# Minys233/GCN-BMP

Measured on NVIDIA B200. Metric: drug pairs/sec (fwd+bwd, GGNN+co-attention), higher is better.
Workload: dtype bf16

## Files before the change

gcn-bmp_b200/csrc/coattn_tc.cu:

```cuda
#include "tc_common.cuh"

namespace bmp {
namespace ctc {
using namespace tc;

constexpr int EPW = 16, NE = 32 * EPW, NT = NE + 64;
constexpr int CLD = 68;
constexpr int PLD = 65;
constexpr int MAXHD = 15;
constexpr int STAGES = 2;

#define EPI_SYNC() asm volatile("bar.sync 1, %0;" ::"n"(NE) : "memory")
#define CTS(i) do { if (a.dbg && blockIdx.x == 0 && tid == 0 && it == 1) a.dbg[i] = clock64(); } while (0)

struct Args {
    int mb, n1, n2, O, head, act, pool;
    const float *atoms_1, *atoms_2, *b, *wa_1, *wa_2, *W_j, *b_j, *lt_2, *V2;
    const uint8_t *img1, *img2, *img1x;
    float *c1, *c2;
    const float *dc1, *dc2;
    float *R, *P1, *P2, *DL1, *DL2, *d_a1, *d_a2;
    float *d_W, *d_lt_1, *d_lt_2, *d_V1, *d_V2, *d_b, *d_wa_1, *d_wa_2;
    long long *dbg;
};

template <int H, bool BWD>
struct Cfg {
    static constexpr int KP = H / 64;
    static constexpr int W1_TILE = (H + 32) * 128;
    static constexpr int WH_TILE = H * 128;
    static constexpr int OFF_XP = 0;
    static constexpr int OFF_QP = OFF_XP + KP * PANEL_BYTES;
    static constexpr int OFF_W = OFF_QP + PANEL_BYTES;
    static constexpr int OFF_SP = OFF_W + STAGES * W1_TILE;
    static constexpr int OFF_DP = OFF_SP + (BWD ? KP * PANEL_BYTES : 0);
    static constexpr int OFF_F = OFF_DP + (BWD ? 2 * PANEL_BYTES : 0);
    static constexpr int TMEM_COLS = BWD ? 512 : 256;
    static constexpr uint32_t COL_D1 = 0, COL_D2 = 192, COL_R = 0, COL_A1 = 0, COL_S = 256, COL_A2 = 256, COL_X1 = 160, COL_X2 = 176, COL_DW = 384;
};

__host__ __device__ inline int f32_floats(int H, int hd, bool bwd) {
    hd = hd <= 8 ? 8 : 16;
    int n = AT * CLD + 2 * AT * PLD + 4;
    n += 4 * hd * AT;
    n += 4 * AT + 2 * H;
    n += 4 * AT + 16 * AT;
    if (bwd) n += 2 * H + 2 * hd * AT + 2 * 16 + 4;
    return (n + 3) & ~3;
}
template <int H, bool BWD>
__host__ __device__ inline size_t smem_bytes(int hd) {
    return (size_t)Cfg<H, BWD>::OFF_F + (size_t)f32_floats(H, hd, BWD) * 4 + 256 + 1024;
}

__device__ __forceinline__ float warp_sum(float v) {
    for (int o = 16; o; o >>= 1) v += __shfl_xor_sync(0xffffffffu, v, o);
    return v;
}
__device__ __forceinline__ float warp_max(float v) {
    for (int o = 16; o; o >>= 1) v = fmaxf(v, __shfl_xor_sync(0xffffffffu, v, o));
    return v;
}
__device__ __forceinline__ float bf16_at(const uint8_t *panels, int row, int col) {
    return __bfloat162float(*reinterpret_cast<const __nv_bfloat16 *>(panels + (col >> 6) * PANEL_BYTES + sw128(row, col & 63)));
}
__device__ __forceinline__ uint4 pack8(const float *v) {
    return make_uint4(pack_bf16(v[0], v[1]), pack_bf16(v[2], v[3]), pack_bf16(v[4], v[5]), pack_bf16(v[6], v[7]));
}

template <int H, bool BWD, int HP>
__global__ void __launch_bounds__(NT, 1) coattn_tc_kernel(const Args a) {
    using C = Cfg<H, BWD>;
    constexpr int HS = HP, HQ = HP / 4;
    constexpr int KP = C::KP;
    extern __shared__ uint8_t smem_raw[];
    uint8_t *smem = (uint8_t *)(((uintptr_t)smem_raw + 1023) & ~(uintptr_t)1023);
    const uint32_t sbase = s32(smem);
    const uint32_t s_xp = sbase + C::OFF_XP, s_qp = sbase + C::OFF_QP, s_w = sbase + C::OFF_W, s_sp = sbase + C::OFF_SP,
                   s_dp = sbase + C::OFF_DP;
    uint8_t *XP = smem + C::OFF_XP, *QP = smem + C::OFF_QP, *SP = smem + C::OFF_SP, *DP = smem + C::OFF_DP;
    const int hd = a.head, N1 = a.n1, N2 = a.n2, O = a.O;
    const bool pool = a.pool != 0;
    float *fp = reinterpret_cast<float *>(smem + C::OFF_F);
    float *Cs = fp; fp += AT * CLD;
    float *L1t = fp; fp += AT * PLD;
    float *L2p = fp; fp += AT * PLD + 4;
    float *lt1 = fp; fp += HS * AT;
    float *lt2 = fp; fp += HS * AT;
    float *H1 = fp; fp += HS * AT;
    float *H2 = fp; fp += HS * AT;
    float *attn1 = fp; fp += AT;
    float *attn2 = fp; fp += AT;
    float *v1 = fp; fp += AT;
    float *v2 = fp; fp += AT;
    float *p1 = fp; fp += H;
    float *p2 = fp; fp += H;
    float *st4 = fp; fp += 4 * AT;
    float *part = fp; fp += 16 * AT;
    float *dp1 = fp, *dp2 = fp + H, *dpre1 = fp + 2 * H, *dpre2 = dpre1 + HS * AT;
    float *gwa1 = dpre2 + HS * AT, *gwa2 = gwa1 + 16, *gb = gwa2 + 16;
    const int f32n = f32_floats(H, hd, BWD);
    const uint32_t s_bar = sbase + C::OFF_F + f32n * 4;
    auto BAR = [&](int i) { return s_bar + 8u * i; };
    constexpr int B_FULL = 0, B_EMPTY = 2, B_XRDY = 4, B_G1 = 5, B_S = 6, B_QRDY = 7, B_G2 = 8, B_DRDY = 9, B_R = 10,
                  B_A2 = 11, B_RRDY = 12, B_A1 = 13, NBAR = 14;
    uint32_t *tmem_slot = reinterpret_cast<uint32_t *>(smem + C::OFF_F + f32n * 4 + 8 * NBAR + 8);

    const int tid = threadIdx.x, warp = tid >> 5, lane = tid & 31;
    if (tid == 0) {
        for (int s = 0; s < STAGES; ++s) { mbar_init(BAR(B_FULL + s), 1); mbar_init(BAR(B_EMPTY + s), 1); }
        mbar_init(BAR(B_XRDY), EPW);
        mbar_init(BAR(B_G1), 1);
        mbar_init(BAR(B_S), 1);
        mbar_init(BAR(B_QRDY), EPW);
        mbar_init(BAR(B_G2), 1);
        mbar_init(BAR(B_DRDY), EPW);
        mbar_init(BAR(B_R), 1);
        mbar_init(BAR(B_A2), 1);
        mbar_init(BAR(B_RRDY), EPW);
        mbar_init(BAR(B_A1), 1);
        fence_mbar_init();
    }
    if (warp == EPW + 1) {
        asm volatile("tcgen05.alloc.cta_group::1.sync.aligned.shared::cta.b32 [%0], %1;" ::"r"(s32(tmem_slot)), "r"(C::TMEM_COLS));
        asm volatile("tcgen05.relinquish_alloc_permit.cta_group::1.sync.aligned;");
    }
    tc_fence_before();
    __syncthreads();
    tc_fence_after();
    const uint32_t tmem = *tmem_slot;

    if (warp == EPW) {
        if (lane == 0) {
            uint32_t stage = 0, phase = 0;
            auto put = [&](const uint8_t *src, uint32_t bytes) {
                mbar_wait(BAR(B_EMPTY + stage), phase ^ 1);
                mbar_expect_tx(BAR(B_FULL + stage), bytes);
                tma_bulk_g2s(s_w + stage * C::W1_TILE, src, bytes, BAR(B_FULL + stage));
                if (++stage == STAGES) { stage = 0; phase ^= 1; }
            };
            for (int pair = blockIdx.x; pair < a.mb; pair += gridDim.x) {
                for (int kt = 0; kt < KP; ++kt) put(a.img1 + (size_t)kt * C::W1_TILE, C::W1_TILE);
                if (BWD) {
                    for (int kt = 0; kt < KP; ++kt) put(a.img2 + (size_t)kt * C::WH_TILE, C::WH_TILE);
                    for (int kt = 0; kt < KP; ++kt) put(a.img1 + (size_t)kt * C::W1_TILE, C::WH_TILE);
                    put(a.img1x, C::WH_TILE);
                }
            }
        }
    } else if (warp == EPW + 1) {
        if (lane == 0) {
            constexpr uint32_t ID_G1 = idesc2(H + 32, 0, 0), ID_H = idesc2(H, 0, 0), ID_64 = idesc2(64, 0, 0), ID_HMN = idesc2(H, 0, 1),
                               ID_WMN = idesc2(H, 1, 1), ID_X = idesc2(16, 1, 1);
            uint32_t stage = 0, phase = 0, it = 0;
            auto mma_wtile = [&](uint32_t a_addr, uint32_t dcol, uint32_t id, bool first, int ksteps) {
                mbar_wait(BAR(B_FULL + stage), phase);
                tc_fence_after();
                const uint32_t b_addr = s_w + stage * C::W1_TILE;
                for (int k = 0; k < ksteps; ++k)
                    tc_mma(tmem + dcol, desc_kmajor(a_addr + k * 32), desc_kmajor(b_addr + k * 32), id, (first && k == 0) ? 0u : 1u);
                tc_commit(BAR(B_EMPTY + stage));
                if (++stage == STAGES) { stage = 0; phase ^= 1; }
            };
            for (int pair = blockIdx.x; pair < a.mb; pair += gridDim.x, ++it) {
                const uint32_t par = it & 1;
                mbar_wait(BAR(B_XRDY), par);
                tc_fence_after();
                for (int kp = 0; kp < KP; ++kp) mma_wtile(s_xp + kp * PANEL_BYTES, C::COL_D1, ID_G1, kp == 0, 4);
                tc_commit(BAR(B_G1));
                if (BWD) {
                    for (int kp = 0; kp < KP; ++kp) mma_wtile(s_xp + kp * PANEL_BYTES, C::COL_S, ID_H, kp == 0, 4);
                    tc_commit(BAR(B_S));
                }
                mbar_wait(BAR(B_QRDY), par);
                tc_fence_after();
                for (int kp = 0; kp < KP; ++kp)
#pragma unroll
                    for (int k = 0; k < 4; ++k)
                        tc_mma(tmem + C::COL_D2, desc_kmajor(s_xp + kp * PANEL_BYTES + k * 32), desc_kmajor(s_qp + kp * 8192 + k * 32), ID_64,
                               (kp == 0 && k == 0) ? 0u : 1u);
                tc_commit(BAR(B_G2));
                if (BWD) {
                    const uint32_t acc = it ? 1u : 0u;
                    mbar_wait(BAR(B_DRDY), par);
                    tc_fence_after();
#pragma unroll
                    for (int k = 0; k < 4; ++k)
                        tc_mma(tmem + C::COL_R, desc_kmajor(s_dp + k * 32), desc_mnmajor(s_xp + 64 * 128 + k * 16 * 128), ID_HMN, k ? 1u : 0u);
                    tc_commit(BAR(B_R));
#pragma unroll
                    for (int k = 0; k < 5; ++k)
                        tc_mma(tmem + C::COL_A2, desc_kmajor(k < 4 ? s_dp + k * 32 : s_dp + PANEL_BYTES), desc_mnmajor(s_sp + k * 16 * 128), ID_HMN,
                               k ? 1u : 0u);
#pragma unroll
                    for (int k = 0; k < 4; ++k)
                        tc_mma(tmem + C::COL_X2, desc_mnmajor(s_xp + 64 * 128 + k * 16 * 128), desc_mnmajor(s_dp + PANEL_BYTES + 64 * 128 + k * 16 * 128),
                               ID_X, (acc || k) ? 1u : 0u);
                    tc_commit(BAR(B_A2));
                    mbar_wait(BAR(B_RRDY), par);
                    tc_fence_after();
                    for (int kp = 0; kp < KP; ++kp) mma_wtile(s_sp + kp * PANEL_BYTES, C::COL_A1, ID_H, kp == 0, 4);
                    mma_wtile(s_qp, C::COL_A1, ID_H, false, 1);
#pragma unroll
                    for (int k = 0; k < 4; ++k) {
                        tc_mma(tmem + C::COL_DW, desc_mnmajor(s_xp + k * 16 * 128), desc_mnmajor(s_sp + k * 16 * 128), ID_WMN, (acc || k) ? 1u : 0u);
                        tc_mma(tmem + C::COL_X1, desc_mnmajor(s_xp + k * 16 * 128), desc_mnmajor(s_qp + k * 16 * 128), ID_X, (acc || k) ? 1u : 0u);
                    }
                    tc_commit(BAR(B_A1));
                }
            }
        }
    } else {
        const int q = warp & 3, cg = warp >> 2;
        const int row = 32 * q + lane;
        const uint32_t t_lane = tmem + ((uint32_t)(32 * q) << 16);
        uint32_t it = 0;
        if (BWD) {
            for (int i = tid; i < 36; i += NE) gwa1[i] = 0.f;
            for (int idx = tid; idx < 16 * (H / 8); idx += NE) {
                const int e = idx / (H / 8), c8 = idx % (H / 8);
                float v[8];
#pragma unroll
                for (int x = 0; x < 8; ++x) {
                    const int k = c8 * 8 + x;
                    v[x] = e < hd ? a.lt_2[(long)e * H + k] : (e == 15 ? a.V2[k] : 0.f);
                }
                *reinterpret_cast<uint4 *>(SP + (c8 >> 3) * PANEL_BYTES + sw128(64 + e, (c8 & 7) * 8)) = pack8(v);
            }
            for (int idx = tid; idx < 128 * 8; idx += NE)
                *reinterpret_cast<uint4 *>(DP + PANEL_BYTES + idx * 16) = make_uint4(0, 0, 0, 0);
        }
        for (int pair = blockIdx.x; pair < a.mb; pair += gridDim.x, ++it) {
            const uint32_t par = it & 1;
            const long r1 = (long)pair * N1, r2 = (long)pair * N2;
            EPI_SYNC();
            CTS(0);
            {
                constexpr int PER = 128 * (H / 8) / NE;
                float4 x0[PER], x1[PER];
#pragma unroll
                for (int u = 0; u < PER; ++u) {
                    const int idx = tid + u * NE, r = idx / (H / 8), c8 = idx % (H / 8), n = r & 63;
                    const bool live = r < 64 ? n < N1 : n < N2;
                    x0[u] = x1[u] = make_float4(0.f, 0.f, 0.f, 0.f);
                    if (live) {
                        const float4 *src = reinterpret_cast<const float4 *>((r < 64 ? a.atoms_1 + (r1 + n) * H : a.atoms_2 + (r2 + n) * H) + c8 * 8);
                        x0[u] = __ldg(src);
                        x1[u] = __ldg(src + 1);
                    }
                }
#pragma unroll
                for (int u = 0; u < PER; ++u) {
                    const int idx = tid + u * NE, r = idx / (H / 8), c8 = idx % (H / 8);
                    *reinterpret_cast<uint4 *>(XP + (c8 >> 3) * PANEL_BYTES + sw128(r, (c8 & 7) * 8)) =
                        make_uint4(pack_bf16(x0[u].x, x0[u].y), pack_bf16(x0[u].z, x0[u].w), pack_bf16(x1[u].x, x1[u].y), pack_bf16(x1[u].z, x1[u].w));
                }
            }
            warp_arrive(BAR(B_XRDY), lane);
            CTS(1);
            if (pair + (int)gridDim.x < a.mb) {
                const long np = pair + gridDim.x;
                const char *b1 = reinterpret_cast<const char *>(a.atoms_1 + np * N1 * H), *b2 = reinterpret_cast<const char *>(a.atoms_2 + np * N2 * H);
                for (int off = tid * 128; off < N1 * H * 4; off += NE * 128) asm volatile("prefetch.global.L2 [%0];" ::"l"(b1 + off));
                for (int off = tid * 128; off < N2 * H * 4; off += NE * 128) asm volatile("prefetch.global.L2 [%0];" ::"l"(b2 + off));
            }
            mbar_wait(BAR(B_G1), par);
            tc_fence_after();
            CTS(2);
            if (q >= 2 && cg * 32 < H) {
                uint32_t v[32];
                tc_ld32(t_lane + C::COL_D1 + cg * 32, v);
                tc_wait_ld();
                const int i = row - 64;
#pragma unroll
                for (int g = 0; g < 4; ++g) {
                    const int kk = cg * 32 + 8 * g;
                    float f[8];
#pragma unroll
                    for (int x = 0; x < 8; ++x) f[x] = __uint_as_float(v[8 * g + x]);
                    *reinterpret_cast<uint4 *>(QP + (kk >> 6) * 8192 + sw128(i, kk & 63)) = pack8(f);
                }
            }
            if (cg == (H == 128 ? 0 : 3)) {
                uint32_t w[16];
                tc_ld16(t_lane + C::COL_D1 + H + (q >= 2 ? 16 : 0), w);
                tc_wait_ld();
                const int n = row & 63;
                float *lt = (q >= 2 ? lt2 : lt1) + n * HS;
#pragma unroll
                for (int d4 = 0; d4 < HQ; ++d4)
                    *reinterpret_cast<float4 *>(lt + 4 * d4) = make_float4(__uint_as_float(w[4 * d4]), __uint_as_float(w[4 * d4 + 1]), __uint_as_float(w[4 * d4 + 2]),
                                                                           4 * d4 + 3 == 15 ? 0.f : __uint_as_float(w[4 * d4 + 3]));
                (q >= 2 ? v2 : v1)[n] = __uint_as_float(w[15]);
            }
            if (BWD) {
                mbar_wait(BAR(B_S), par);
                tc_fence_after();
                if (q < 2 && cg * 32 < H) {
                    uint32_t v[32];
                    tc_ld32(t_lane + C::COL_S + cg * 32, v);
                    tc_wait_ld();
#pragma unroll
                    for (int g = 0; g < 4; ++g) {
                        const int kk = cg * 32 + 8 * g;
                        float f[8];
#pragma unroll
                        for (int x = 0; x < 8; ++x) f[x] = __uint_as_float(v[8 * g + x]);
                        *reinterpret_cast<uint4 *>(SP + (kk >> 6) * PANEL_BYTES + sw128(row, kk & 63)) = pack8(f);
                    }
                }
            }
            warp_arrive(BAR(B_QRDY), lane);
            EPI_SYNC();
            CTS(3);
            mbar_wait(BAR(B_G2), par);
            tc_fence_after();
            CTS(4);
            if (q < 2) {
                uint32_t w[16];
                tc_ld16(t_lane + C::COL_D2 + cg * 16, w);
                tc_wait_ld();
                const float base = v1[row] + a.b[0];
#pragma unroll
                for (int x = 0; x < 16; x += 4) {
                    const float4 vv = *reinterpret_cast<const float4 *>(v2 + cg * 16 + x);
                    float4 o;
                    o.x = act_fast(a.act, __uint_as_float(w[x]) + base + vv.x);
                    o.y = act_fast(a.act, __uint_as_float(w[x + 1]) + base + vv.y);
                    o.z = act_fast(a.act, __uint_as_float(w[x + 2]) + base + vv.z);
                    o.w = act_fast(a.act, __uint_as_float(w[x + 3]) + base + vv.w);
                    *reinterpret_cast<float4 *>(Cs + row * CLD + cg * 16 + x) = o;
                }
            }
            tc_fence_before();
            EPI_SYNC();
            CTS(5);
            if (pool) {
                if (tid < AT) {
                    float sm = 0.f;
                    for (int j = 0; j < N1; ++j) sm += Cs[j * CLD + tid];
                    attn2[tid] = sm / (float)N1;
                }
                for (int j = warp; j < AT; j += EPW) {
                    const float sm = warp_sum((lane < N2 ? Cs[j * CLD + lane] : 0.f) + (lane + 32 < N2 ? Cs[j * CLD + lane + 32] : 0.f));
                    if (lane == 0) attn1[j] = sm / (float)N2;
                }
            } else {
            float *m2 = st4, *is2 = st4 + AT, *m1 = st4 + 2 * AT, *is1 = st4 + 3 * AT;
            {
                const int i = tid & 63, pt = tid >> 6;
                float m = -INFINITY, s = 0.f;
                if (i < N2) {
                    float c[8];
#pragma unroll
                    for (int x = 0; x < 8; ++x) c[x] = (8 * pt + x < N1) ? Cs[(8 * pt + x) * CLD + i] : -INFINITY;
#pragma unroll
                    for (int x = 0; x < 8; ++x) m = fmaxf(m, c[x]);
#pragma unroll
                    for (int x = 0; x < 8; ++x) s += c[x] > -INFINITY ? __expf(c[x] - m) : 0.f;
                }
                part[pt * AT + i] = m;
                part[8 * AT + pt * AT + i] = s;
                {
                    float x0[4], x1[4], mx[4], sm[4];
#pragma unroll
                    for (int k = 0; k < 4; ++k) {
                        const int j = warp + EPW * k;
                        x0[k] = (j < N1 && lane < N2) ? Cs[j * CLD + lane] : -INFINITY;
                        x1[k] = (j < N1 && lane + 32 < N2) ? Cs[j * CLD + lane + 32] : -INFINITY;
                        mx[k] = fmaxf(x0[k], x1[k]);
                    }
#pragma unroll
                    for (int o = 16; o; o >>= 1)
#pragma unroll
                        for (int k = 0; k < 4; ++k) mx[k] = fmaxf(mx[k], __shfl_xor_sync(0xffffffffu, mx[k], o));
#pragma unroll
                    for (int k = 0; k < 4; ++k)
                        sm[k] = (x0[k] > -INFINITY ? __expf(x0[k] - mx[k]) : 0.f) + (x1[k] > -INFINITY ? __expf(x1[k] - mx[k]) : 0.f);
#pragma unroll
                    for (int o = 16; o; o >>= 1)
#pragma unroll
                        for (int k = 0; k < 4; ++k) sm[k] += __shfl_xor_sync(0xffffffffu, sm[k], o);
                    if (lane < 4) {
                        const float mm = lane == 0 ? mx[0] : (lane == 1 ? mx[1] : (lane == 2 ? mx[2] : mx[3]));
                        const float ss = lane == 0 ? sm[0] : (lane == 1 ? sm[1] : (lane == 2 ? sm[2] : sm[3]));
                        m2[warp + EPW * lane] = mm;
                        is2[warp + EPW * lane] = ss > 0.f ? 1.f / ss : 0.f;
                    }
                }
            }
            EPI_SYNC();
            if (tid < AT) {
                float m = -INFINITY, s = 0.f;
#pragma unroll
                for (int pt = 0; pt < 8; ++pt) m = fmaxf(m, part[pt * AT + tid]);
#pragma unroll
                for (int pt = 0; pt < 8; ++pt) {
                    const float pm = part[pt * AT + tid];
                    s += pm > -INFINITY ? part[8 * AT + pt * AT + tid] * __expf(pm - m) : 0.f;
                }
                m1[tid] = m;
                is1[tid] = s > 0.f ? 1.f / s : 0.f;
            }
            EPI_SYNC();
            for (int idx = tid; idx < AT * AT; idx += NE) {
                const int j = idx >> 6, i = idx & 63;
                const bool live = j < N1 && i < N2;
                const float c = Cs[j * CLD + i];
                L2p[j * PLD + i] = live ? __expf(c - m2[j]) * is2[j] : 0.f;
                L1t[i * PLD + j] = live ? __expf(c - m1[i]) * is1[i] : 0.f;
            }
            EPI_SYNC();
            CTS(6);
            {
                const int which = tid >> 8, n = (tid >> 2) & 63, pt = tid & 3;
                const float *Lw = which ? L2p : L1t, *other = which ? lt1 : lt2;
                float acc[HP];
#pragma unroll
                for (int d = 0; d < HP; ++d) acc[d] = 0.f;
#pragma unroll 4
                for (int mm = 0; mm < 16; ++mm) {
                    const int m = 4 * mm + pt;
                    const float l = Lw[m * PLD + n];
#pragma unroll
                    for (int d4 = 0; d4 < HQ; ++d4) {
                        const float4 r4 = *reinterpret_cast<const float4 *>(other + m * HS + 4 * d4);
                        acc[4 * d4] = fmaf(l, r4.x, acc[4 * d4]); acc[4 * d4 + 1] = fmaf(l, r4.y, acc[4 * d4 + 1]);
                        acc[4 * d4 + 2] = fmaf(l, r4.z, acc[4 * d4 + 2]); acc[4 * d4 + 3] = fmaf(l, r4.w, acc[4 * d4 + 3]);
                    }
                }
#pragma unroll
                for (int d = 0; d < HP; ++d) {
                    acc[d] += __shfl_xor_sync(0xffffffffu, acc[d], 1);
                    acc[d] += __shfl_xor_sync(0xffffffffu, acc[d], 2);
                }
                const float *self = (which ? lt2 : lt1) + n * HS;
                float *Hk = (which ? H2 : H1) + n * HS;
#pragma unroll
                for (int d4 = 0; d4 < HQ; ++d4) {
                    const float v = pt == 0 ? acc[4 * d4] : (pt == 1 ? acc[4 * d4 + 1] : (pt == 2 ? acc[4 * d4 + 2] : acc[4 * d4 + 3]));
                    Hk[4 * d4 + pt] = tanh_fast(self[4 * d4 + pt] + v);
                }
            }
            EPI_SYNC();
            CTS(7);
            if (tid < 2 * AT) {
                const int n = tid & 63;
                const float *Hk = (tid < AT ? H1 : H2) + n * HS, *wa = tid < AT ? a.wa_1 : a.wa_2;
                float sc = 0.f;
#pragma unroll
                for (int d = 0; d < HP; ++d) sc += d < hd ? __ldg(wa + d) * Hk[d] : 0.f;
                (tid < AT ? attn1 : attn2)[n] = sc;
            }
            }
            EPI_SYNC();
            if (warp < 2) {
                float *x = warp ? attn2 : attn1;
                const int n = warp ? N2 : N1;
                const float x0 = lane < n ? x[lane] : -INFINITY, x1 = lane + 32 < n ? x[lane + 32] : -INFINITY;
                const float m = warp_max(fmaxf(x0, x1));
                const float e0 = lane < n ? __expf(x0 - m) : 0.f, e1 = lane + 32 < n ? __expf(x1 - m) : 0.f;
                const float s = warp_sum(e0 + e1);
                x[lane] = e0 / s;
                x[lane + 32] = e1 / s;
            }
            EPI_SYNC();
            CTS(8);
            if (tid < 2 * H) {
                const int which = tid >= H, h = which ? tid - H : tid;
                const float *at = which ? attn2 : attn1;
                const int n = which ? N2 : N1;
                float s = 0.f;
                for (int r = 0; r < n; ++r) s += at[r] * bf16_at(XP, 64 * which + r, h);
                (which ? p2 : p1)[h] = s;
            }
            EPI_SYNC();
            CTS(9);
            if (!BWD) {
                for (int r = tid >> 2; r < 2 * O; r += NE / 4) {
                    const int which = r >= O, o = which ? r - O : r, pt = tid & 3;
                    const float *p = which ? p2 : p1;
                    const float4 *w = reinterpret_cast<const float4 *>(a.W_j + (long)o * H);
                    float4 ww[H / 16];
#pragma unroll
                    for (int u = 0; u < H / 16; ++u) ww[u] = __ldg(w + 4 * u + pt);
                    float s0 = 0.f, s1 = 0.f;
#pragma unroll
                    for (int u = 0; u < H / 16; ++u) {
                        const float4 pp = *reinterpret_cast<const float4 *>(p + 4 * (4 * u + pt));
                        s0 = fmaf(ww[u].x, pp.x, fmaf(ww[u].y, pp.y, s0));
                        s1 = fmaf(ww[u].z, pp.z, fmaf(ww[u].w, pp.w, s1));
                    }
                    float sum = s0 + s1;
                    sum += __shfl_xor_sync(0xffffffffu, sum, 1);
                    sum += __shfl_xor_sync(0xffffffffu, sum, 2);
                    if (pt == 0) (which ? a.c2 : a.c1)[(long)pair * O + o] = sum + a.b_j[o];
                }
                CTS(10);
                continue;
            }
            float *t1 = st4, *t2 = st4 + AT, *cs = st4 + 2 * AT, *rsum = st4 + 3 * AT;
            {
                const int oh = tid >> 8, e = tid & 255;
                const int which = e >= H, h = which ? e - H : e;
                float s0 = 0.f, s1 = 0.f, s2 = 0.f, s3 = 0.f;
                if (e < 2 * H) {
                    if (oh == 0) (which ? a.P2 : a.P1)[(long)pair * H + h] = (which ? p2 : p1)[h];
                    const float *dc = (which ? a.dc2 : a.dc1) + (long)pair * O;
                    const int ob = ((O + 1) / 2 + 7) & ~7, o_end = oh ? O : (ob < O ? ob : O);
                    int o = oh ? (ob < O ? ob : O) : 0;
                    for (; o + 8 <= o_end; o += 8) {
                        float w[8];
#pragma unroll
                        for (int x = 0; x < 8; ++x) w[x] = __ldg(a.W_j + (long)(o + x) * H + h);
                        const float4 d0 = __ldg(reinterpret_cast<const float4 *>(dc + o)), d1 = __ldg(reinterpret_cast<const float4 *>(dc + o) + 1);
                        s0 = fmaf(w[0], d0.x, s0); s1 = fmaf(w[1], d0.y, s1); s2 = fmaf(w[2], d0.z, s2); s3 = fmaf(w[3], d0.w, s3);
                        s0 = fmaf(w[4], d1.x, s0); s1 = fmaf(w[5], d1.y, s1); s2 = fmaf(w[6], d1.z, s2); s3 = fmaf(w[7], d1.w, s3);
                    }
                    for (; o < o_end; ++o) s0 = fmaf(__ldg(a.W_j + (long)o * H + h), __ldg(dc + o), s0);
                }
                if (oh == 1 && e < 2 * H) part[e] = (s0 + s1) + (s2 + s3);
                EPI_SYNC();
                if (oh == 0 && e < 2 * H) (which ? dp2 : dp1)[h] = (s0 + s1) + (s2 + s3) + part[e];
            }
            EPI_SYNC();
            CTS(10);
            {
                const int which = tid >> 8, n = (tid >> 2) & 63, hp = tid & 3;
                const float *dp = which ? dp2 : dp1;
                float s = 0.f;
                for (int c8 = hp; c8 < H / 8; c8 += 4) {
                    const uint4 u = *reinterpret_cast<const uint4 *>(XP + (c8 >> 3) * PANEL_BYTES + sw128(64 * which + n, (c8 & 7) * 8));
                    const __nv_bfloat162 *b2 = reinterpret_cast<const __nv_bfloat162 *>(&u);
#pragma unroll
                    for (int x = 0; x < 4; ++x) {
                        const float2 f = __bfloat1622float2(b2[x]);
                        s += f.x * dp[c8 * 8 + 2 * x] + f.y * dp[c8 * 8 + 2 * x + 1];
                    }
                }
                s += __shfl_xor_sync(0xffffffffu, s, 1);
                s += __shfl_xor_sync(0xffffffffu, s, 2);
                if (hp == 0) (which ? t2 : t1)[n] = s;
            }
            EPI_SYNC();
            if (warp < 2) {
                const float *at = warp ? attn2 : attn1;
                float *da = warp ? t2 : t1;
                const int n = warp ? N2 : N1;
                const float x0 = lane < n ? at[lane] * da[lane] : 0.f, x1 = lane + 32 < n ? at[lane + 32] * da[lane + 32] : 0.f;
                const float dot = warp_sum(x0 + x1);
                da[lane] = lane < n ? at[lane] * (da[lane] - dot) : 0.f;
                da[lane + 32] = lane + 32 < n ? at[lane + 32] * (da[lane + 32] - dot) : 0.f;
            }
            EPI_SYNC();
            CTS(11);
            if (pool) {
                for (int idx = tid; idx < 2 * AT * HP; idx += NE) (idx < AT * HP ? H1 : H2 - AT * HP)[idx] = 0.f;
                for (int idx = tid; idx < AT * AT; idx += NE) {
                    const int j = idx >> 6, i = idx & 63;
                    const float c = Cs[j * CLD + i];
                    const float g = (j < N1 && i < N2) ? t1[j] / (float)N2 + t2[i] / (float)N1 : 0.f;
                    Cs[j * CLD + i] = g * act_bwd(a.act, c, c);
                }
                EPI_SYNC();
            } else {
            for (int idx = tid; idx < 2 * AT * HQ; idx += NE) {
                const int which = idx / (AT * HQ), r = idx % (AT * HQ), n = r / HQ, d4 = r % HQ;
                const float4 hv = *reinterpret_cast<const float4 *>((which ? H2 : H1) + n * HS + 4 * d4);
                const float *wa = which ? a.wa_2 : a.wa_1;
                const float ds = (which ? t2 : t1)[n];
                float4 o;
                o.x = 4 * d4 + 0 < hd ? ds * __ldg(wa + 4 * d4 + 0) * (1.f - hv.x * hv.x) : 0.f;
                o.y = 4 * d4 + 1 < hd ? ds * __ldg(wa + 4 * d4 + 1) * (1.f - hv.y * hv.y) : 0.f;
                o.z = 4 * d4 + 2 < hd ? ds * __ldg(wa + 4 * d4 + 2) * (1.f - hv.z * hv.z) : 0.f;
                o.w = 4 * d4 + 3 < hd ? ds * __ldg(wa + 4 * d4 + 3) * (1.f - hv.w * hv.w) : 0.f;
                *reinterpret_cast<float4 *>((which ? dpre2 : dpre1) + n * HS + 4 * d4) = o;
            }
            for (int r = warp; r < 2 * hd; r += EPW) {
                const int which = r >= hd, d = which ? r - hd : r;
                const float *Hk = (which ? H2 : H1) + d, *ds = which ? t2 : t1;
                const float sw = warp_sum(ds[lane] * Hk[lane * HS] + ds[lane + 32] * Hk[(lane + 32) * HS]);
                if (lane == 0) (which ? gwa2 : gwa1)[d] += sw;
            }
            EPI_SYNC();
            CTS(12);
            {
                const int out = tid >> 2, pt = tid & 3, which = out >= AT, n = out & 63;
                const float *Lw = which ? L2p : L1t;
                const float *other = which ? dpre2 : dpre1;
                float own[HP];
#pragma unroll
                for (int d4 = 0; d4 < HQ; ++d4) {
                    const float4 r4 = *reinterpret_cast<const float4 *>((which ? lt1 : lt2) + n * HS + 4 * d4);
                    own[4 * d4] = r4.x; own[4 * d4 + 1] = r4.y; own[4 * d4 + 2] = r4.z; own[4 * d4 + 3] = r4.w;
                }
                float u = 0.f;
#pragma unroll 4
                for (int mm = 0; mm < 16; ++mm) {
                    const int m = 4 * mm + pt;
                    float dl = 0.f;
#pragma unroll
                    for (int d4 = 0; d4 < HQ; ++d4) {
                        const float4 r4 = *reinterpret_cast<const float4 *>(other + m * HS + 4 * d4);
                        dl = fmaf(r4.x, own[4 * d4], fmaf(r4.y, own[4 * d4 + 1], fmaf(r4.z, own[4 * d4 + 2], fmaf(r4.w, own[4 * d4 + 3], dl))));
                    }
                    u = fmaf(Lw[n * PLD + m], dl, u);
                }
                u += __shfl_xor_sync(0xffffffffu, u, 1);
                u += __shfl_xor_sync(0xffffffffu, u, 2);
                if (pt == 0) part[out] = u;
            }
            {
                const int which = tid >> 8, n = (tid >> 2) & 63, pt = tid & 3;
                const float *Lw = which ? L1t : L2p, *other = which ? dpre1 : dpre2;
                float acc[HP];
#pragma unroll
                for (int d = 0; d < HP; ++d) acc[d] = 0.f;
#pragma unroll 4
                for (int mm = 0; mm < 16; ++mm) {
                    const int m = 4 * mm + pt;
                    const float l = Lw[n * PLD + m];
#pragma unroll
                    for (int d4 = 0; d4 < HQ; ++d4) {
                        const float4 r4 = *reinterpret_cast<const float4 *>(other + m * HS + 4 * d4);
                        acc[4 * d4] = fmaf(l, r4.x, acc[4 * d4]); acc[4 * d4 + 1] = fmaf(l, r4.y, acc[4 * d4 + 1]);
                        acc[4 * d4 + 2] = fmaf(l, r4.z, acc[4 * d4 + 2]); acc[4 * d4 + 3] = fmaf(l, r4.w, acc[4 * d4 + 3]);
                    }
                }
#pragma unroll
                for (int d = 0; d < HP; ++d) {
                    acc[d] += __shfl_xor_sync(0xffffffffu, acc[d], 1);
                    acc[d] += __shfl_xor_sync(0xffffffffu, acc[d], 2);
                }
                const float *self = (which ? dpre2 : dpre1) + n * HS;
                float *dst = (which ? H2 : H1) + n * HS;
#pragma unroll
                for (int d4 = 0; d4 < HQ; ++d4) {
                    const float v = pt == 0 ? acc[4 * d4] : (pt == 1 ? acc[4 * d4 + 1] : (pt == 2 ? acc[4 * d4 + 2] : acc[4 * d4 + 3]));
                    dst[4 * d4 + pt] = self[4 * d4 + pt] + v;
                }
            }
            EPI_SYNC();
            CTS(13);
            {
                const int i = tid & 63;
                float l2[HP], p2[HP];
#pragma unroll
                for (int d4 = 0; d4 < HQ; ++d4) {
                    const float4 x4 = *reinterpret_cast<const float4 *>(lt2 + i * HS + 4 * d4), y4 = *reinterpret_cast<const float4 *>(dpre2 + i * HS + 4 * d4);
                    l2[4 * d4] = x4.x; l2[4 * d4 + 1] = x4.y; l2[4 * d4 + 2] = x4.z; l2[4 * d4 + 3] = x4.w;
                    p2[4 * d4] = y4.x; p2[4 * d4 + 1] = y4.y; p2[4 * d4 + 2] = y4.z; p2[4 * d4 + 3] = y4.w;
                }
                const float u1i = part[i];
#pragma unroll 2
                for (int u8 = 0; u8 < AT * AT / NE; ++u8) {
                    const int j = (tid >> 6) + u8 * (NE / 64);
                    float dl1 = 0.f, dl2 = 0.f;
#pragma unroll
                    for (int d4 = 0; d4 < HQ; ++d4) {
                        const float4 x4 = *reinterpret_cast<const float4 *>(dpre1 + j * HS + 4 * d4), y4 = *reinterpret_cast<const float4 *>(lt1 + j * HS + 4 * d4);
                        dl1 = fmaf(x4.x, l2[4 * d4], fmaf(x4.y, l2[4 * d4 + 1], fmaf(x4.z, l2[4 * d4 + 2], fmaf(x4.w, l2[4 * d4 + 3], dl1))));
                        dl2 = fmaf(y4.x, p2[4 * d4], fmaf(y4.y, p2[4 * d4 + 1], fmaf(y4.z, p2[4 * d4 + 2], fmaf(y4.w, p2[4 * d4 + 3], dl2))));
                    }
                    const float c = Cs[j * CLD + i];
                    const float g = L1t[i * PLD + j] * (dl1 - u1i) + L2p[j * PLD + i] * (dl2 - part[AT + j]);
                    Cs[j * CLD + i] = g * act_bwd(a.act, c, c);
                }
            }
            EPI_SYNC();
            CTS(14);
            }
            if (tid < AT) {
                float s = 0.f;
                for (int j = 0; j < AT; ++j) s += Cs[j * CLD + tid];
                rsum[tid] = s;
            }
            for (int j = warp; j < AT; j += EPW) {
                const float s = warp_sum(Cs[j * CLD + lane] + Cs[j * CLD + lane + 32]);
                if (lane == 0) cs[j] = s;
            }
            EPI_SYNC();
            CTS(15);
            if (warp == EPW - 1) {
                const float s = warp_sum(rsum[lane] + rsum[lane + 32]);
                if (lane == 0) gb[0] += s;
            }
            for (int idx = tid; idx < 2 * AT * 8; idx += NE) {
                float v[8];
                if (idx < AT * 8) {
                    const int j = idx >> 3, c8 = idx & 7;
                    const float4 x0 = *reinterpret_cast<const float4 *>(Cs + j * CLD + c8 * 8), x1 = *reinterpret_cast<const float4 *>(Cs + j * CLD + c8 * 8 + 4);
                    v[0] = x0.x; v[1] = x0.y; v[2] = x0.z; v[3] = x0.w; v[4] = x1.x; v[5] = x1.y; v[6] = x1.z; v[7] = x1.w;
                    *reinterpret_cast<uint4 *>(DP + sw128(j, c8 * 8)) = pack8(v);
                } else {
                    const int i = idx & 63, c8 = (idx - AT * 8) >> 6;
#pragma unroll
                    for (int x = 0; x < 8; ++x) v[x] = Cs[(c8 * 8 + x) * CLD + i];
                    *reinterpret_cast<uint4 *>(DP + sw128(64 + i, c8 * 8)) = pack8(v);
                }
            }
            if (tid < 2 * AT) {
                const int which = tid < AT, n = tid & 63;
                const float *dl = (which ? H2 : H1) + n * HS;
                float v[16];
#pragma unroll
                for (int d = 0; d < 16; ++d) v[d] = d < HP ? dl[d] : 0.f;
                v[15] = which ? rsum[n] : cs[n];
                uint8_t *dst = which ? DP + PANEL_BYTES : QP;
                const int r = which ? 64 + n : n;
                *reinterpret_cast<uint4 *>(dst + sw128(r, 0)) = pack8(v);
                *reinterpret_cast<uint4 *>(dst + sw128(r, 8)) = pack8(v + 8);
            }
            warp_arrive(BAR(B_DRDY), lane);
            CTS(16);
            mbar_wait(BAR(B_R), par);
            mbar_wait(BAR(B_A2), par);
            tc_fence_after();
            CTS(17);
            float *stg = reinterpret_cast<float *>(DP + warp * 2048);
            if (cg * 32 < H) {
                uint32_t v[32];
                if (q < 2) {
                    tc_ld32(t_lane + C::COL_R + cg * 32, v);
                    tc_wait_ld();
#pragma unroll
                    for (int g = 0; g < 4; ++g) {
                        const int kk = cg * 32 + 8 * g;
                        float f[8];
#pragma unroll
                        for (int x = 0; x < 8; ++x) f[x] = __uint_as_float(v[8 * g + x]);
                        *reinterpret_cast<uint4 *>(SP + (kk >> 6) * PANEL_BYTES + sw128(row, kk & 63)) = pack8(f);
                    }
                } else {
                    tc_ld32(t_lane + C::COL_A2 + cg * 32, v);
                    tc_wait_ld();
                    const float at = attn2[row - 64];
                    float f[32];
#pragma unroll
                    for (int x = 0; x < 32; x += 4) {
                        const float4 d4 = *reinterpret_cast<const float4 *>(dp2 + cg * 32 + x);
                        f[x] = fmaf(at, d4.x, __uint_as_float(v[x])); f[x + 1] = fmaf(at, d4.y, __uint_as_float(v[x + 1]));
                        f[x + 2] = fmaf(at, d4.z, __uint_as_float(v[x + 2])); f[x + 3] = fmaf(at, d4.w, __uint_as_float(v[x + 3]));
                    }
#pragma unroll
                    for (int h2 = 0; h2 < 2; ++h2)
                        warp_store_rows<16>(stg, f + 16 * h2, lane, [&](int r) -> float * {
                            const int i = 32 * (q - 2) + r;
                            return i < N2 ? a.d_a2 + (r2 + i) * H + cg * 32 + 16 * h2 : nullptr;
                        });
                }
            }
            warp_arrive(BAR(B_RRDY), lane);
            CTS(18);
            mbar_wait(BAR(B_A1), par);
            tc_fence_after();
            CTS(19);
            if (q < 2 && cg * 32 < H) {
                uint32_t v[32];
                tc_ld32(t_lane + C::COL_A1 + cg * 32, v);
                tc_wait_ld();
                const float at = attn1[row];
                float f[32];
#pragma unroll
                for (int x = 0; x < 32; x += 4) {
                    const float4 d4 = *reinterpret_cast<const float4 *>(dp1 + cg * 32 + x);
                    f[x] = fmaf(at, d4.x, __uint_as_float(v[x])); f[x + 1] = fmaf(at, d4.y, __uint_as_float(v[x + 1]));
                    f[x + 2] = fmaf(at, d4.z, __uint_as_float(v[x + 2])); f[x + 3] = fmaf(at, d4.w, __uint_as_float(v[x + 3]));
                }
#pragma unroll
                for (int h2 = 0; h2 < 2; ++h2)
                    warp_store_rows<16>(stg, f + 16 * h2, lane, [&](int r) -> float * {
                        const int j = 32 * q + r;
                        return j < N1 ? a.d_a1 + (r1 + j) * H + cg * 32 + 16 * h2 : nullptr;
                    });
            }
            CTS(20);
            CTS(21);
            tc_fence_before();
        }
        if (BWD && it > 0) {
            tc_fence_after();
            if (row < H && cg * 32 < H && a.d_W) {
                uint32_t v[32];
                tc_ld32(t_lane + C::COL_DW + cg * 32, v);
                tc_wait_ld();
                float *dst = a.d_W + (long)row * H + cg * 32;
#pragma unroll
                for (int x = 0; x < 32; x += 4)
                    atomicAdd(reinterpret_cast<float4 *>(dst + x),
                              make_float4(__uint_as_float(v[x]), __uint_as_float(v[x + 1]), __uint_as_float(v[x + 2]), __uint_as_float(v[x + 3])));
            }
            if (row < H && cg >= 2) {
                const int k2 = cg - 2;
                uint32_t w[16];
                tc_ld16(t_lane + (k2 ? C::COL_X2 : C::COL_X1), w);
                tc_wait_ld();
                float *dlt = k2 ? a.d_lt_2 : a.d_lt_1, *dV = k2 ? a.d_V2 : a.d_V1;
#pragma unroll
                for (int d = 0; d < MAXHD; ++d)
                    if (d < hd && dlt) atomicAdd(dlt + (long)d * H + row, __uint_as_float(w[d]));
                if (dV) atomicAdd(dV + row, __uint_as_float(w[15]));
            }
            tc_fence_before();
            EPI_SYNC();
            if (tid < hd) {
                if (a.d_wa_1) atomicAdd(a.d_wa_1 + tid, gwa1[tid]);
                if (a.d_wa_2) atomicAdd(a.d_wa_2 + tid, gwa2[tid]);
            }
            if (tid == 0 && a.d_b) atomicAdd(a.d_b, gb[0]);
        }
    }
    tc_fence_before();
    __syncthreads();
    if (warp == EPW + 1) {
        tc_fence_after();
        asm volatile("tcgen05.dealloc.cta_group::1.sync.aligned.b32 %0, %1;" ::"r"(tmem), "r"(C::TMEM_COLS));
    }
}

struct PackArgs {
    int H, head;
    const float *W, *V1, *V2, *lt_1, *lt_2;
    uint8_t *img1, *img2, *img1x;
};
__global__ void pack_coattn_kernel(const PackArgs p) {
    const int H = p.H, KP = H / 64, hd = p.head;
    const long n1 = (long)KP * (H + 32) * 64, n2 = (long)KP * H * 64, n3 = (long)H * 64;
    for (long idx = (long)blockIdx.x * blockDim.x + threadIdx.x; idx < n1 + n2 + n3; idx += (long)gridDim.x * blockDim.x) {
        float w = 0.f;
        uint8_t *dst;
        int n, kk;
        if (idx < n1) {
            kk = idx & 63; n = (idx >> 6) % (H + 32);
            const int kt = (int)(idx / (64L * (H + 32))), K = kt * 64 + kk;
            if (n < H) w = p.W[(long)n * H + K];
            else {
                const int e = n - H, which = e >> 4, d = e & 15;
                if (d < hd) w = (which ? p.lt_2 : p.lt_1)[(long)d * H + K];
                else if (d == 15) w = (which ? p.V2 : p.V1)[K];
            }
            dst = p.img1 + (size_t)kt * (H + 32) * 128;
        } else if (idx < n1 + n2) {
            const long r = idx - n1;
            kk = r & 63; n = (r >> 6) % H;
            const int kt = (int)(r / (64L * H));
            w = p.W[(long)(kt * 64 + kk) * H + n];
            dst = p.img2 + (size_t)kt * H * 128;
        } else {
            const long r = idx - n1 - n2;
            kk = r & 63; n = (int)(r >> 6);
            if (kk < hd) w = p.lt_1[(long)kk * H + n];
            else if (kk == 15) w = p.V1[n];
            dst = p.img1x;
        }
        const uint32_t off = (uint32_t)n * 128u + ((((uint32_t)(kk >> 3) ^ ((uint32_t)n & 7u)) << 4) | (((uint32_t)kk & 7u) << 1));
        *reinterpret_cast<__nv_bfloat16 *>(dst + off) = __float2bfloat16_rn(w);
    }
}

static size_t img_bytes(int H) { return (size_t)(H / 64) * (H + 32) * 128 + (size_t)(H / 64) * H * 128 + (size_t)H * 128; }

}
}

using namespace bmp;

static long long *g_ctc_dbg = nullptr;
extern "C" void bmp_debug_set_buffer_ctc(void *p) { g_ctc_dbg = (long long *)p; }

extern "C" size_t bmp_coattn_tc_workspace_bytes(int hidden) {
    if (hidden != 64 && hidden != 128) return 0;
    return ctc::img_bytes(hidden) + 1024;
}

bool bmp_coattn_tc_supported(int H, int head, int variant, bool bwd) {
    if (H != 64 && H != 128) return false;
    if (variant == BMP_COATTN_FINE ? (head < 1 || head > ctc::MAXHD) : variant != BMP_COATTN_POOL) return false;
    if (variant == BMP_COATTN_POOL) head = 0;
    const size_t need = H == 64 ? (bwd ? ctc::smem_bytes<64, true>(head) : ctc::smem_bytes<64, false>(head))
                                : (bwd ? ctc::smem_bytes<128, true>(head) : ctc::smem_bytes<128, false>(head));
    return need <= 227 * 1024;
}

template <int H, bool BWD, int HP>
static int launch_ctc_hp(const ctc::Args &k, int head, cudaStream_t st) {
    int dev = 0, sms = 148;
    cudaGetDevice(&dev);
    cudaDeviceGetAttribute(&sms, cudaDevAttrMultiProcessorCount, dev);
    const int grid = k.mb < sms ? k.mb : sms;
    const size_t smem = ctc::smem_bytes<H, BWD>(head);
    cudaFuncSetAttribute(ctc::coattn_tc_kernel<H, BWD, HP>, cudaFuncAttributeMaxDynamicSharedMemorySize, (int)smem);
    ProfScope prof(BWD ? BMP_PROF_COATTN_BWD : BMP_PROF_COATTN_FWD, st);
    ctc::coattn_tc_kernel<H, BWD, HP><<<grid, ctc::NT, smem, st>>>(k);
    count_launch();
    return check_launch("coattn_tc_kernel");
}

template <int H, bool BWD>
static int launch_ctc(const ctc::Args &k, int head, cudaStream_t st) {
    return head <= 8 ? launch_ctc_hp<H, BWD, 8>(k, head, st) : launch_ctc_hp<H, BWD, 16>(k, head, st);
}

static int ctc_prepare(ctc::Args &k, int mb, int n1, int n2, int H, int O, int head, int act, const float *a1, const float *a2,
                       const float *W, const float *V1, const float *V2, const float *b, const float *lt1, const float *lt2,
                       const float *wa1, const float *wa2, const float *Wj, const float *bj, void *ws, size_t ws_bytes, bool images_ready,
                       cudaStream_t st) {
    if (!ws || ws_bytes < bmp_coattn_tc_workspace_bytes(H)) {
        set_error("BMP_MODE_BF16 co-attention: tc_workspace of >= %zu bytes required", bmp_coattn_tc_workspace_bytes(H));
        return BMP_EINVAL;
    }
    uint8_t *base = (uint8_t *)(((uintptr_t)ws + 255) & ~(uintptr_t)255);
    ctc::PackArgs p;
    p.H = H; p.head = head; p.W = W; p.V1 = V1; p.V2 = V2; p.lt_1 = lt1; p.lt_2 = lt2;
    p.img1 = base;
    p.img2 = p.img1 + (size_t)(H / 64) * (H + 32) * 128;
    p.img1x = p.img2 + (size_t)(H / 64) * H * 128;
    if (!images_ready) {
        ctc::pack_coattn_kernel<<<32, 256, 0, st>>>(p);
        count_launch();
        int rc = check_launch("pack_coattn_kernel");
        if (rc) return rc;
    }
    k = ctc::Args{};
    k.mb = mb; k.n1 = n1; k.n2 = n2; k.O = O; k.head = head; k.act = act;
    k.atoms_1 = a1; k.atoms_2 = a2; k.b = b; k.wa_1 = wa1; k.wa_2 = wa2; k.W_j = Wj; k.b_j = bj; k.lt_2 = lt2; k.V2 = V2;
    k.img1 = p.img1; k.img2 = p.img2; k.img1x = p.img1x;
    k.dbg = g_ctc_dbg;
    return BMP_OK;
}

int bmp_coattn_forward_tc(const bmp_coattn_fwd_t *a, void *stream) {
    cudaStream_t st = (cudaStream_t)stream;
    ctc::Args k;
    const int head = a->variant == BMP_COATTN_POOL ? 0 : a->head;
    int rc = ctc_prepare(k, a->mb, a->n1, a->n2, a->hidden, a->out_dim, head, a->act, a->atoms_1, a->atoms_2, a->W, a->V1, a->V2, a->b,
                         a->lt_1, a->lt_2, a->wa_1, a->wa_2, a->W_j, a->b_j, a->tc_workspace, a->tc_workspace_bytes, a->tc_images_ready != 0, st);
    if (rc) return rc;
    k.c1 = a->compact_1; k.c2 = a->compact_2;
    k.pool = a->variant == BMP_COATTN_POOL;
    return a->hidden == 64 ? launch_ctc<64, false>(k, head, st) : launch_ctc<128, false>(k, head, st);
}

int bmp_coattn_backward_tc(const bmp_coattn_bwd_t *a, void *stream) {
    cudaStream_t st = (cudaStream_t)stream;
    ctc::Args k;
    const int head = a->variant == BMP_COATTN_POOL ? 0 : a->head;
    int rc = ctc_prepare(k, a->mb, a->n1, a->n2, a->hidden, a->out_dim, head, a->act, a->atoms_1, a->atoms_2, a->W, a->V1, a->V2, a->b,
                         a->lt_1, a->lt_2, a->wa_1, a->wa_2, a->W_j, a->b_j, a->tc_workspace, a->tc_workspace_bytes, a->tc_images_ready != 0, st);
    if (rc) return rc;
    k.dc1 = a->d_compact_1; k.dc2 = a->d_compact_2; k.R = a->R; k.P1 = a->P1; k.P2 = a->P2; k.DL1 = a->DL1; k.DL2 = a->DL2;
    k.d_a1 = a->d_atoms_1; k.d_a2 = a->d_atoms_2;
    k.d_W = a->d_W; k.d_lt_1 = a->d_lt_1; k.d_lt_2 = a->d_lt_2;
    k.d_V1 = a->d_V1; k.d_V2 = a->d_V2; k.d_b = a->d_b; k.d_wa_1 = a->d_wa_1; k.d_wa_2 = a->d_wa_2;
    k.pool = a->variant == BMP_COATTN_POOL;
    return a->hidden == 64 ? launch_ctc<64, true>(k, head, st) : launch_ctc<128, true>(k, head, st);
}
```

gcn-bmp_b200/csrc/common.cuh:

```cuda
#pragma once
#include <cuda_runtime.h>
#include <stdint.h>
#include <initializer_list>
#include "../../include/gcnbmp.h"

namespace bmp {

constexpr int AT = 64;
constexpr int NTHREADS = 256;
constexpr int KT = 32;
constexpr int XLD = KT + 4;
constexpr int XLDT = 64 + 4;
constexpr int STAGE_FLOATS = 2 * 64 * XLD;

void set_error(const char *fmt, ...);
void count_launch(int n = 1);
int check_launch(const char *what);
bool aligned16(std::initializer_list<const void *> ps);
struct ProfScope {
    int kind;
    cudaStream_t st;
    void *slot;
    ProfScope(int kind, cudaStream_t st);
    ~ProfScope();
};
inline bool same_gru(const bmp_gru_t &x, const bmp_gru_t &y) {
    return x.W_r == y.W_r && x.b_Wr == y.b_Wr && x.U_r == y.U_r && x.b_Ur == y.b_Ur && x.W_z == y.W_z && x.b_Wz == y.b_Wz &&
           x.U_z == y.U_z && x.b_Uz == y.b_Uz && x.W == y.W && x.b_W == y.b_W && x.U == y.U && x.b_U == y.b_U;
}

__device__ __forceinline__ void cp_async16(void *smem, const void *gmem) {
    unsigned s = (unsigned)__cvta_generic_to_shared(smem);
    asm volatile("cp.async.cg.shared.global [%0], [%1], 16;\n" ::"r"(s), "l"(gmem));
}
__device__ __forceinline__ void cp_async_commit() { asm volatile("cp.async.commit_group;\n" ::); }
template <int N>
__device__ __forceinline__ void cp_async_wait() { asm volatile("cp.async.wait_group %0;\n" ::"n"(N)); }

__device__ __forceinline__ float sigmoidf_(float x) { return 1.f / (1.f + expf(-x)); }

__device__ __forceinline__ float act_fwd(int act, float x) {
    switch (act) {
        case BMP_ACT_TANH: return tanhf(x);
        case BMP_ACT_RELU: return x > 0.f ? x : 0.f;
        case BMP_ACT_SIGMOID: return sigmoidf_(x);
        default: return x;
    }
}
__device__ __forceinline__ float act_bwd(int act, float x, float y) {
    switch (act) {
        case BMP_ACT_TANH: return 1.f - y * y;
        case BMP_ACT_RELU: return x > 0.f ? 1.f : 0.f;
        case BMP_ACT_SIGMOID: return y * (1.f - y);
        default: return 1.f;
    }
}

__device__ __forceinline__ void zero_acc(float (&acc)[4][4]) {
#pragma unroll
    for (int a = 0; a < 4; ++a)
#pragma unroll
        for (int b = 0; b < 4; ++b) acc[a][b] = 0.f;
}

template <bool TRANS>
__device__ __forceinline__ void stage_tile(float *buf, const float *__restrict__ Xg, long ldx,
                                           int o_base, int o_lim, int k0, int K) {
    const int tid = threadIdx.x;
#pragma unroll
    for (int it = 0; it < 2; ++it) {
        int idx = tid + it * NTHREADS;
        if (!TRANS) {
            int row = idx >> 3, kq = (idx & 7) * 4;
            float *dst = buf + row * XLD + kq;
            if (o_base + row < o_lim && k0 + kq < K)
                cp_async16(dst, Xg + (long)(o_base + row) * ldx + k0 + kq);
            else
                *reinterpret_cast<float4 *>(dst) = make_float4(0.f, 0.f, 0.f, 0.f);
        } else {
            int krow = idx >> 4, oq = (idx & 15) * 4;
            float *dst = buf + krow * XLDT + oq;
            if (k0 + krow < K && o_base + oq < o_lim)
                cp_async16(dst, Xg + (long)(k0 + krow) * ldx + o_base + oq);
            else
                *reinterpret_cast<float4 *>(dst) = make_float4(0.f, 0.f, 0.f, 0.f);
        }
    }
}

template <bool TRANS>
__device__ __forceinline__ void gemm64_g(float (&acc)[4][4], const float *__restrict__ Xg, long ldx,
                                         int o_base, int o_lim, int K, const float *Ys, float *stage) {
    const int tx = threadIdx.x & 15, ty = threadIdx.x >> 4;
    const int o0 = ty * 4, i0 = tx * 4;
    const int nchunks = (K + KT - 1) / KT;
    constexpr int BUF = 64 * XLD;
    stage_tile<TRANS>(stage, Xg, ldx, o_base, o_lim, 0, K);
    cp_async_commit();
    for (int c = 0; c < nchunks; ++c) {
        float *cur = stage + (c & 1) * BUF;
        if (c + 1 < nchunks) {
            stage_tile<TRANS>(stage + ((c + 1) & 1) * BUF, Xg, ldx, o_base, o_lim, (c + 1) * KT, K);
            cp_async_commit();
            cp_async_wait<1>();
        } else {
            cp_async_wait<0>();
        }
        __syncthreads();
        const int k0 = c * KT;
        const int kmax = min(KT, K - k0);
        const float *Yk = Ys + (long)k0 * AT + i0;
        if (!TRANS) {
            for (int kk = 0; kk < kmax; kk += 4) {
                float4 x[4], y[4];
#pragma unroll
                for (int a = 0; a < 4; ++a) x[a] = *reinterpret_cast<const float4 *>(cur + (o0 + a) * XLD + kk);
#pragma unroll
                for (int q = 0; q < 4; ++q) y[q] = *reinterpret_cast<const float4 *>(Yk + (kk + q) * AT);
#pragma unroll
                for (int a = 0; a < 4; ++a) {
                    acc[a][0] += x[a].x * y[0].x + x[a].y * y[1].x + x[a].z * y[2].x + x[a].w * y[3].x;
                    acc[a][1] += x[a].x * y[0].y + x[a].y * y[1].y + x[a].z * y[2].y + x[a].w * y[3].y;
                    acc[a][2] += x[a].x * y[0].z + x[a].y * y[1].z + x[a].z * y[2].z + x[a].w * y[3].z;
                    acc[a][3] += x[a].x * y[0].w + x[a].y * y[1].w + x[a].z * y[2].w + x[a].w * y[3].w;
                }
            }
        } else {
#pragma unroll 4
            for (int kk = 0; kk < kmax; ++kk) {
                float4 x = *reinterpret_cast<const float4 *>(cur + kk * XLDT + o0);
                float4 y = *reinterpret_cast<const float4 *>(Yk + kk * AT);
                acc[0][0] += x.x * y.x; acc[0][1] += x.x * y.y; acc[0][2] += x.x * y.z; acc[0][3] += x.x * y.w;
                acc[1][0] += x.y * y.x; acc[1][1] += x.y * y.y; acc[1][2] += x.y * y.z; acc[1][3] += x.y * y.w;
                acc[2][0] += x.z * y.x; acc[2][1] += x.z * y.y; acc[2][2] += x.z * y.z; acc[2][3] += x.z * y.w;
                acc[3][0] += x.w * y.x; acc[3][1] += x.w * y.y; acc[3][2] += x.w * y.z; acc[3][3] += x.w * y.w;
            }
        }
        __syncthreads();
    }
}

__device__ __forceinline__ void gemm64_s(float (&acc)[4][4], const float *Xs, int ldx, int o_base, int K,
                                         const float *Ys) {
    const int tx = threadIdx.x & 15, ty = threadIdx.x >> 4;
    const int o0 = o_base + ty * 4, i0 = tx * 4;
    for (int kk = 0; kk < K; kk += 4) {
        float4 x[4], y[4];
#pragma unroll
        for (int a = 0; a < 4; ++a) x[a] = *reinterpret_cast<const float4 *>(Xs + (o0 + a) * ldx + kk);
#pragma unroll
        for (int q = 0; q < 4; ++q) y[q] = *reinterpret_cast<const float4 *>(Ys + (kk + q) * AT + i0);
#pragma unroll
        for (int a = 0; a < 4; ++a) {
            acc[a][0] += x[a].x * y[0].x + x[a].y * y[1].x + x[a].z * y[2].x + x[a].w * y[3].x;
            acc[a][1] += x[a].x * y[0].y + x[a].y * y[1].y + x[a].z * y[2].y + x[a].w * y[3].y;
            acc[a][2] += x[a].x * y[0].z + x[a].y * y[1].z + x[a].z * y[2].z + x[a].w * y[3].z;
            acc[a][3] += x[a].x * y[0].w + x[a].y * y[1].w + x[a].z * y[2].w + x[a].w * y[3].w;
        }
    }
}

__device__ __forceinline__ void load_cm(float *dst, const float *__restrict__ src, int n, int C) {
    const int nq = C >> 2;
    for (int idx = threadIdx.x; idx < nq * AT; idx += NTHREADS) {
        int i = idx & (AT - 1), cq = idx >> 6;
        float4 v = make_float4(0.f, 0.f, 0.f, 0.f);
        if (i < n) v = *reinterpret_cast<const float4 *>(src + (long)i * C + cq * 4);
        float *d = dst + (cq * 4) * AT + i;
        d[0] = v.x; d[AT] = v.y; d[2 * AT] = v.z; d[3 * AT] = v.w;
    }
}
__device__ __forceinline__ void load_embed_cm(float *dst, const int32_t *__restrict__ ids,
                                              const float *__restrict__ W, int n, int C, int n_types) {
    const int nq = C >> 2;
    for (int idx = threadIdx.x; idx < nq * AT; idx += NTHREADS) {
        int i = idx & (AT - 1), cq = idx >> 6;
        float4 v = make_float4(0.f, 0.f, 0.f, 0.f);
        if (i < n) {
            int id = ids[i];
            id = id < 0 ? 0 : (id >= n_types ? n_types - 1 : id);
            v = *reinterpret_cast<const float4 *>(W + (long)id * C + cq * 4);
        }
        float *d = dst + (cq * 4) * AT + i;
        d[0] = v.x; d[AT] = v.y; d[2 * AT] = v.z; d[3 * AT] = v.w;
    }
}
__device__ __forceinline__ void store_cm(float *__restrict__ dst, long ld, const float *src, int n, int C) {
    const int nq = C >> 2;
    for (int idx = threadIdx.x; idx < nq * AT; idx += NTHREADS) {
        int i = idx & (AT - 1), cq = idx >> 6;
        if (i < n) {
            const float *s = src + (cq * 4) * AT + i;
            *reinterpret_cast<float4 *>(dst + (long)i * ld + cq * 4) = make_float4(s[0], s[AT], s[2 * AT], s[3 * AT]);
        }
    }
}
__device__ __forceinline__ void tile_store_g(float *__restrict__ g, long ld, int o_base, int o_lim, int n,
                                             const float (&v)[4][4]) {
    const int tx = threadIdx.x & 15, ty = threadIdx.x >> 4;
    const int o0 = o_base + ty * 4, i0 = tx * 4;
    if (o0 >= o_lim) return;
#pragma unroll
    for (int b = 0; b < 4; ++b)
        if (i0 + b < n)
            *reinterpret_cast<float4 *>(g + (long)(i0 + b) * ld + o0) = make_float4(v[0][b], v[1][b], v[2][b], v[3][b]);
}
__device__ __forceinline__ void tile_load_g(const float *__restrict__ g, long ld, int o_base, int o_lim, int n,
                                            float (&v)[4][4]) {
    const int tx = threadIdx.x & 15, ty = threadIdx.x >> 4;
    const int o0 = o_base + ty * 4, i0 = tx * 4;
#pragma unroll
    for (int b = 0; b < 4; ++b) {
        float4 t = make_float4(0.f, 0.f, 0.f, 0.f);
        if (o0 < o_lim && i0 + b < n) t = *reinterpret_cast<const float4 *>(g + (long)(i0 + b) * ld + o0);
        v[0][b] = t.x; v[1][b] = t.y; v[2][b] = t.z; v[3][b] = t.w;
    }
}
__device__ __forceinline__ void tile_store_s(float *s, int o_base, const float (&v)[4][4]) {
    const int tx = threadIdx.x & 15, ty = threadIdx.x >> 4;
    const int o0 = o_base + ty * 4, i0 = tx * 4;
#pragma unroll
    for (int a = 0; a < 4; ++a)
        *reinterpret_cast<float4 *>(s + (o0 + a) * AT + i0) = make_float4(v[a][0], v[a][1], v[a][2], v[a][3]);
}
__device__ __forceinline__ void tile_load_s(const float *s, int o_base, float (&v)[4][4]) {
    const int tx = threadIdx.x & 15, ty = threadIdx.x >> 4;
    const int o0 = o_base + ty * 4, i0 = tx * 4;
#pragma unroll
    for (int a = 0; a < 4; ++a) {
        float4 t = *reinterpret_cast<const float4 *>(s + (o0 + a) * AT + i0);
        v[a][0] = t.x; v[a][1] = t.y; v[a][2] = t.z; v[a][3] = t.w;
    }
}

template <bool TRANSPOSE>
__device__ __forceinline__ void load_adj(float *dst, const float *__restrict__ adj, int n,
                                         const float *colscale = nullptr) {
    if (TRANSPOSE) {
        for (int idx = threadIdx.x; idx < 16 * AT; idx += NTHREADS) {
            int i = idx & (AT - 1), jq = (idx >> 6) * 4;
            float v[4] = {0.f, 0.f, 0.f, 0.f};
            if (i < n) {
#pragma unroll
                for (int q = 0; q < 4; ++q)
                    if (jq + q < n) {
                        v[q] = adj[(long)i * n + jq + q];
                        if (colscale) v[q] *= colscale[jq + q];
                    }
            }
#pragma unroll
            for (int q = 0; q < 4; ++q) dst[(jq + q) * AT + i] = v[q];
        }
    } else {
        for (int idx = threadIdx.x; idx < AT * AT; idx += NTHREADS) {
            int i = idx >> 6, j = idx & (AT - 1);
            float v = 0.f;
            if (i < n && j < n) {
                v = adj[(long)i * n + j];
                if (colscale) v *= colscale[j];
            }
            dst[i * AT + j] = v;
        }
    }
}

}
```

gcn-bmp_b200/csrc/gemm.cu:

```cuda
#include "common.cuh"

namespace bmp {

constexpr int RT = 32;
constexpr int WLD = 64 + 4;

__global__ void __launch_bounds__(NTHREADS) wgrad_kernel(const float *__restrict__ A, int lda,
                                                         const float *__restrict__ B, int ldb,
                                                         float *__restrict__ C, int ldc,
                                                         long rows, int M, int N, int tilesN, long rows_per_cta,
                                                         int vec) {
    __shared__ __align__(16) float As[2][RT][WLD];
    __shared__ __align__(16) float Bs[2][RT][WLD];
    const int tid = threadIdx.x;
    const int tm = (blockIdx.x / tilesN) * 64, tn = (blockIdx.x % tilesN) * 64;
    const long r_begin = (long)blockIdx.y * rows_per_cta;
    const long r_end = min(rows, r_begin + rows_per_cta);
    if (r_begin >= r_end) return;
    const int tx = tid & 15, ty = tid >> 4;
    const int m0 = ty * 4, n0 = tx * 4;
    float acc[4][4];
    zero_acc(acc);

    auto stage = [&](int buf, long r0) {
#pragma unroll
        for (int it = 0; it < 2; ++it) {
            int idx = tid + it * NTHREADS;
            int rr = idx >> 4, cq = (idx & 15) * 4;
            long r = r0 + rr;
            float *da = &As[buf][rr][cq], *db = &Bs[buf][rr][cq];
            if (vec) {
                if (r < r_end && tm + cq < M) cp_async16(da, A + r * lda + tm + cq);
                else *reinterpret_cast<float4 *>(da) = make_float4(0.f, 0.f, 0.f, 0.f);
                if (r < r_end && tn + cq < N) cp_async16(db, B + r * ldb + tn + cq);
                else *reinterpret_cast<float4 *>(db) = make_float4(0.f, 0.f, 0.f, 0.f);
            } else {
#pragma unroll
                for (int q = 0; q < 4; ++q) {
                    da[q] = (r < r_end && tm + cq + q < M) ? A[r * lda + tm + cq + q] : 0.f;
                    db[q] = (r < r_end && tn + cq + q < N) ? B[r * ldb + tn + cq + q] : 0.f;
                }
            }
        }
    };
    const long nchunks = (r_end - r_begin + RT - 1) / RT;
    stage(0, r_begin);
    cp_async_commit();
    for (long c = 0; c < nchunks; ++c) {
        const int cur = c & 1;
        if (c + 1 < nchunks) {
            stage(cur ^ 1, r_begin + (c + 1) * RT);
            cp_async_commit();
            cp_async_wait<1>();
        } else {
            cp_async_wait<0>();
        }
        __syncthreads();
#pragma unroll 8
        for (int kk = 0; kk < RT; ++kk) {
            float4 x = *reinterpret_cast<const float4 *>(&As[cur][kk][m0]);
            float4 y = *reinterpret_cast<const float4 *>(&Bs[cur][kk][n0]);
            acc[0][0] += x.x * y.x; acc[0][1] += x.x * y.y; acc[0][2] += x.x * y.z; acc[0][3] += x.x * y.w;
            acc[1][0] += x.y * y.x; acc[1][1] += x.y * y.y; acc[1][2] += x.y * y.z; acc[1][3] += x.y * y.w;
            acc[2][0] += x.z * y.x; acc[2][1] += x.z * y.y; acc[2][2] += x.z * y.z; acc[2][3] += x.z * y.w;
            acc[3][0] += x.w * y.x; acc[3][1] += x.w * y.y; acc[3][2] += x.w * y.z; acc[3][3] += x.w * y.w;
        }
        __syncthreads();
    }
#pragma unroll
    for (int a = 0; a < 4; ++a)
#pragma unroll
        for (int b = 0; b < 4; ++b)
            if (tm + m0 + a < M && tn + n0 + b < N) atomicAdd(C + (long)(tm + m0 + a) * ldc + tn + n0 + b, acc[a][b]);
}

__global__ void __launch_bounds__(NTHREADS) colsum_kernel(const float *__restrict__ B, int ldb,
                                                          float *__restrict__ out, int ostride, long rows, int N,
                                                          long rows_per_cta) {
    __shared__ float red[4][64];
    const int col = blockIdx.x * 64 + (threadIdx.x & 63), rg = threadIdx.x >> 6;
    const long r_begin = (long)blockIdx.y * rows_per_cta;
    const long r_end = min(rows, r_begin + rows_per_cta);
    float s = 0.f;
    if (col < N)
        for (long r = r_begin + rg; r < r_end; r += 4) s += B[r * ldb + col];
    red[rg][threadIdx.x & 63] = s;
    __syncthreads();
    if (rg == 0 && col < N) {
        s = red[0][threadIdx.x] + red[1][threadIdx.x] + red[2][threadIdx.x] + red[3][threadIdx.x];
        atomicAdd(out + (long)col * ostride, s);
    }
}

template <int MODE>
__global__ void __launch_bounds__(NTHREADS) linear_kernel(const float *__restrict__ X, const float *__restrict__ W,
                                                          const float *__restrict__ bias, float *__restrict__ Y,
                                                          long rows, int in_dim, int out_dim, int act) {
    __shared__ __align__(16) float Xs[64][XLD];
    __shared__ __align__(16) float Ws[64 * XLD];
    const int tid = threadIdx.x, tx = tid & 15, ty = tid >> 4;
    const long r0 = (long)blockIdx.x * 64;
    const int c0 = blockIdx.y * 64;
    const int Kred = MODE == 0 ? in_dim : out_dim;
    const int Nout = MODE == 0 ? out_dim : in_dim;
    const int ldx = Kred, ldw = in_dim;
    float acc[4][4];
    zero_acc(acc);
    for (int k0 = 0; k0 < Kred; k0 += KT) {
        for (int idx = tid; idx < 64 * KT; idx += NTHREADS) {
            int rr = idx / KT, kk = idx % KT;
            long r = r0 + rr;
            Xs[rr][kk] = (r < rows && k0 + kk < Kred) ? X[r * ldx + k0 + kk] : 0.f;
        }
        if (MODE == 0) {
            for (int idx = tid; idx < 64 * KT; idx += NTHREADS) {
                int oo = idx / KT, kk = idx % KT;
                Ws[oo * XLD + kk] = (c0 + oo < out_dim && k0 + kk < in_dim) ? W[(long)(c0 + oo) * ldw + k0 + kk] : 0.f;
            }
        } else {
            for (int idx = tid; idx < KT * 64; idx += NTHREADS) {
                int oo = idx / 64, kk = idx % 64;
                Ws[oo * WLD + kk] = (k0 + oo < out_dim && c0 + kk < in_dim) ? W[(long)(k0 + oo) * ldw + c0 + kk] : 0.f;
            }
        }
        __syncthreads();
        if (MODE == 0) {
#pragma unroll
            for (int kk = 0; kk < KT; kk += 4) {
                float4 x[4], w[4];
#pragma unroll
                for (int a = 0; a < 4; ++a) x[a] = *reinterpret_cast<const float4 *>(&Xs[tx + 16 * a][kk]);
#pragma unroll
                for (int b = 0; b < 4; ++b) w[b] = *reinterpret_cast<const float4 *>(&Ws[(ty * 4 + b) * XLD + kk]);
#pragma unroll
                for (int a = 0; a < 4; ++a)
#pragma unroll
                    for (int b = 0; b < 4; ++b)
                        acc[a][b] += x[a].x * w[b].x + x[a].y * w[b].y + x[a].z * w[b].z + x[a].w * w[b].w;
            }
        } else {
#pragma unroll
            for (int kk = 0; kk < KT; kk += 4) {
                float4 x[4], w[4];
#pragma unroll
                for (int a = 0; a < 4; ++a) x[a] = *reinterpret_cast<const float4 *>(&Xs[tx + 16 * a][kk]);
#pragma unroll
                for (int q = 0; q < 4; ++q) w[q] = *reinterpret_cast<const float4 *>(&Ws[(kk + q) * WLD + ty * 4]);
#pragma unroll
                for (int a = 0; a < 4; ++a) {
                    acc[a][0] += x[a].x * w[0].x + x[a].y * w[1].x + x[a].z * w[2].x + x[a].w * w[3].x;
                    acc[a][1] += x[a].x * w[0].y + x[a].y * w[1].y + x[a].z * w[2].y + x[a].w * w[3].y;
                    acc[a][2] += x[a].x * w[0].z + x[a].y * w[1].z + x[a].z * w[2].z + x[a].w * w[3].z;
                    acc[a][3] += x[a].x * w[0].w + x[a].y * w[1].w + x[a].z * w[2].w + x[a].w * w[3].w;
                }
            }
        }
        __syncthreads();
    }
#pragma unroll
    for (int a = 0; a < 4; ++a) {
        long r = r0 + tx + 16 * a;
        if (r >= rows) continue;
#pragma unroll
        for (int b = 0; b < 4; ++b) {
            int c = c0 + ty * 4 + b;
            if (c >= Nout) continue;
            float v = acc[a][b];
            if (MODE == 0) {
                if (bias) v += bias[c];
                v = act_fwd(act, v);
            }
            Y[r * Nout + c] = v;
        }
    }
}

__global__ void act_bwd_kernel(float *__restrict__ dy, const float *__restrict__ y, long n, int act) {
    long i = (long)blockIdx.x * blockDim.x + threadIdx.x;
    if (i >= n) return;
    float yy = y[i], d = 1.f;
    if (act == BMP_ACT_TANH) d = 1.f - yy * yy;
    else if (act == BMP_ACT_RELU) d = yy > 0.f ? 1.f : 0.f;
    else if (act == BMP_ACT_SIGMOID) d = yy * (1.f - yy);
    dy[i] *= d;
}

static int sm_count() {
    static int sms = 0;
    if (!sms) {
        int dev = 0;
        cudaGetDevice(&dev);
        cudaDeviceGetAttribute(&sms, cudaDevAttrMultiProcessorCount, dev);
        if (sms <= 0) sms = 148;
    }
    return sms;
}

}

using namespace bmp;

extern "C" int bmp_wgrad(const float *A, int lda, const float *B, int ldb, float *C, int ldc,
                         int64_t rows, int M, int N, void *stream) {
    if (!A || !B || !C) { set_error("bmp_wgrad: null pointer"); return BMP_EINVAL; }
    if (rows <= 0 || M <= 0 || N <= 0) return BMP_OK;
    const int vec = !((lda & 3) || (ldb & 3) || (M & 3) || (N & 3) || ((uintptr_t)A & 15) || ((uintptr_t)B & 15));
    const int tilesM = (M + 63) / 64, tilesN = (N + 63) / 64;
    const int tiles = tilesM * tilesN;
    long split = (4L * sm_count() + tiles - 1) / tiles;
    long max_split = (rows + 4 * RT - 1) / (4 * RT);
    if (split > max_split) split = max_split;
    if (split < 1) split = 1;
    if (split > 65535) split = 65535;
    long rpc = (rows + split - 1) / split;
    rpc = (rpc + RT - 1) / RT * RT;
    split = (rows + rpc - 1) / rpc;
    dim3 grid(tiles, (unsigned)split);
    wgrad_kernel<<<grid, NTHREADS, 0, (cudaStream_t)stream>>>(A, lda, B, ldb, C, ldc, rows, M, N, tilesN, rpc, vec);
    count_launch();
    return check_launch("wgrad_kernel");
}

extern "C" int bmp_colsum(const float *B, int ldb, float *out, int out_stride, int64_t rows, int N, void *stream) {
    if (!B || !out) { set_error("bmp_colsum: null pointer"); return BMP_EINVAL; }
    if (rows <= 0 || N <= 0) return BMP_OK;
    const int tiles = (N + 63) / 64;
    long split = (2L * sm_count() + tiles - 1) / tiles;
    long max_split = (rows + 255) / 256;
    if (split > max_split) split = max_split;
    if (split < 1) split = 1;
    if (split > 65535) split = 65535;
    long rpc = (rows + split - 1) / split;
    split = (rows + rpc - 1) / rpc;
    dim3 grid(tiles, (unsigned)split);
    colsum_kernel<<<grid, NTHREADS, 0, (cudaStream_t)stream>>>(B, ldb, out, out_stride, rows, N, rpc);
    count_launch();
    return check_launch("colsum_kernel");
}

extern "C" int bmp_linear_forward(const float *x, const float *W, const float *b, float *y,
                                  int rows, int in_dim, int out_dim, int act, void *stream) {
    if (!x || !W || !y) { set_error("bmp_linear_forward: null pointer"); return BMP_EINVAL; }
    if (rows <= 0) return BMP_OK;
    if (in_dim <= 0 || out_dim <= 0) { set_error("bmp_linear_forward: bad dims"); return BMP_ESHAPE; }
    dim3 grid((rows + 63) / 64, (out_dim + 63) / 64);
    linear_kernel<0><<<grid, NTHREADS, 0, (cudaStream_t)stream>>>(x, W, b, y, rows, in_dim, out_dim, act);
    count_launch();
    return check_launch("linear_kernel<0>");
}

extern "C" int bmp_linear_backward(const float *x, const float *W, const float *y, float *dy,
                                   float *dx, float *dW, float *db,
                                   int rows, int in_dim, int out_dim, int act, void *stream) {
    if (!x || !W || !dy) { set_error("bmp_linear_backward: null pointer"); return BMP_EINVAL; }
    if (rows <= 0) return BMP_OK;
    cudaStream_t st = (cudaStream_t)stream;
    int rc;
    if (act != BMP_ACT_IDENTITY) {
        if (!y) { set_error("bmp_linear_backward: y needed for a non-identity activation"); return BMP_EINVAL; }
        long n = (long)rows * out_dim;
        act_bwd_kernel<<<(unsigned)((n + 255) / 256), 256, 0, st>>>(dy, y, n, act);
        count_launch();
        if ((rc = check_launch("act_bwd_kernel"))) return rc;
    }
    if (dx) {
        dim3 grid((rows + 63) / 64, (in_dim + 63) / 64);
        linear_kernel<1><<<grid, NTHREADS, 0, st>>>(dy, W, nullptr, dx, rows, in_dim, out_dim, 0);
        count_launch();
        if ((rc = check_launch("linear_kernel<1>"))) return rc;
    }
    if (dW) {
        if ((rc = bmp_wgrad(dy, out_dim, x, in_dim, dW, in_dim, rows, out_dim, in_dim, stream))) return rc;
    }
    if (db && (rc = bmp_colsum(dy, out_dim, db, 1, rows, out_dim, stream))) return rc;
    return BMP_OK;
}
```

gcn-bmp_b200/csrc/pair.cu:

```cuda
#include <cstring>
#include "common.cuh"

using namespace bmp;

namespace {

struct Carve {
    uint8_t *p;
    size_t used;
    explicit Carve(void *base) : p((uint8_t *)(((uintptr_t)base + 1023) & ~(uintptr_t)1023)), used(1024) {}
    template <class T>
    T *take(size_t n) {
        const size_t bytes = (n * sizeof(T) + 1023) & ~(size_t)1023;
        T *r = p ? reinterpret_cast<T *>(p) : nullptr;
        if (p) p += bytes;
        used += bytes;
        return r;
    }
};

struct Enc {
    float *Hs, *Ms, *Gs, *RSs, *Ps, *dHs;
    float *out2, *dout2;
    uint8_t *stash2;
    float *R, *DL;
};

struct Plan {
    Enc e[2];
    void *x3_ws, *tc_fwd, *tc_bwd, *co_ws;
    size_t x3_bytes, tc_bytes, co_bytes;
    float *c1, *c2, *dc1, *dc2, *P1, *P2, *corr, *dcorr, *dlogits;
    size_t total;
};

Plan make_plan(void *base, int mb, int n1, int n2, int H, int O, int head, int K, int T, int mode) {
    Plan pl;
    memset(&pl, 0, sizeof(pl));
    Carve c(base);
    const int N[2] = {n1, n2};
    const bool bf16 = mode == BMP_MODE_BF16;
    for (int s = 0; s < 2; ++s) {
        const size_t R = (size_t)mb * N[s], RH = R * H;
        Enc &e = pl.e[s];
        if (bf16) {
            e.out2 = c.take<float>(2 * RH);
            e.dout2 = c.take<float>(2 * RH);
            e.stash2 = c.take<uint8_t>(bmp_ggnn_stash2_bytes(mb, H, T));
        } else {
            e.Hs = c.take<float>((size_t)(T + 1) * RH);
            e.Ms = c.take<float>((size_t)T * RH);
            e.Gs = c.take<float>((size_t)T * 3 * RH);
            e.RSs = c.take<float>((size_t)T * RH);
            e.Ps = c.take<float>((size_t)T * 4 * RH);
            e.dHs = c.take<float>((size_t)(T + 1) * RH);
        }
        e.R = c.take<float>(RH);
        e.DL = c.take<float>(R * (size_t)(head > 0 ? head : 1));
    }
    if (bf16) {
        pl.tc_bytes = bmp_ggnn_tc_workspace_bytes(H, T);
        pl.tc_fwd = c.take<uint8_t>(pl.tc_bytes);
        pl.tc_bwd = c.take<uint8_t>(pl.tc_bytes);
        pl.co_bytes = bmp_coattn_tc_workspace_bytes(H);
        pl.co_ws = c.take<uint8_t>(pl.co_bytes ? pl.co_bytes : 16);
    } else {
        const size_t b1 = bmp_ggnn_x3_workspace_bytes(mb, n1, H, 4, T, 0), b2 = bmp_ggnn_x3_workspace_bytes(mb, n2, H, 4, T, 0);
        pl.x3_bytes = (b1 && b2) ? (b1 > b2 ? b1 : b2) : 0;
        pl.x3_ws = pl.x3_bytes ? c.take<uint8_t>(pl.x3_bytes) : nullptr;
    }
    pl.c1 = c.take<float>((size_t)mb * O); pl.c2 = c.take<float>((size_t)mb * O);
    pl.dc1 = c.take<float>((size_t)mb * O); pl.dc2 = c.take<float>((size_t)mb * O);
    pl.P1 = c.take<float>((size_t)mb * H); pl.P2 = c.take<float>((size_t)mb * H);
    pl.corr = c.take<float>((size_t)mb * O); pl.dcorr = c.take<float>((size_t)mb * O);
    pl.dlogits = c.take<float>((size_t)mb * K);
    pl.total = c.used;
    return pl;
}

bool shape_bad(int mb, int n1, int n2, int H, int O, int head, int K, int T) {
    return mb <= 0 || n1 <= 0 || n2 <= 0 || H <= 0 || O <= 0 || head < 0 || K <= 0 || T <= 0 || T > BMP_MAX_STEPS;
}

}

extern "C" size_t bmp_pair_workspace_bytes(int mb, int n1, int n2, int hidden, int out_dim, int head, int n_classes, int n_steps, int mode) {
    if (shape_bad(mb, n1, n2, hidden, out_dim, head, n_classes, n_steps)) return 0;
    if (mode == BMP_MODE_BF16 && bmp_ggnn_stash2_bytes(mb, hidden, n_steps) == 0) return 0;
    return make_plan(nullptr, mb, n1, n2, hidden, out_dim, head, n_classes, n_steps, mode).total;
}

extern "C" int bmp_pair_forward_backward(const bmp_pair_t *a, void *stream) {
    if (!a || !a->atoms_1 || !a->atoms_2 || !a->adj_1 || !a->adj_2 || !a->labels || !a->embed_W || !a->out_W || !a->logits || !a->loss ||
        !a->workspace) {
        set_error("bmp_pair_forward_backward: null argument");
        return BMP_EINVAL;
    }
    const int mb = a->mb, H = a->hidden, O = a->out_dim, K = a->n_classes, T = a->n_steps, head = a->head;
    if (shape_bad(mb, a->n1, a->n2, H, O, head, K, T)) { set_error("bmp_pair_forward_backward: bad shape"); return BMP_ESHAPE; }
    const size_t need = bmp_pair_workspace_bytes(mb, a->n1, a->n2, H, O, head, K, T, a->mode);
    if (need == 0 || a->workspace_bytes < need) {
        set_error("bmp_pair_forward_backward: workspace of %zu bytes, %zu needed", a->workspace_bytes, need);
        return BMP_EINVAL;
    }
    if (!(a->count > 0.f)) { set_error("bmp_pair_forward_backward: count must be positive"); return BMP_EINVAL; }
    const bool bf16 = a->mode == BMP_MODE_BF16;
    cudaStream_t st = (cudaStream_t)stream;
    Plan pl = make_plan(a->workspace, mb, a->n1, a->n2, H, O, head, K, T, a->mode);
    const int N[2] = {a->n1, a->n2};
    const int32_t *atoms[2] = {a->atoms_1, a->atoms_2};
    const void *adj[2] = {a->adj_1, a->adj_2};
    if (a->adj_u8 && !bf16) { set_error("bmp_pair_forward_backward: a byte / bit-packed adjacency needs BMP_MODE_BF16"); return BMP_EINVAL; }
    const float *hT[2];
    float *d_hT[2];
    int rc;

    for (int s = 0; s < 2; ++s) {
        const size_t RH = (size_t)mb * N[s] * H;
        Enc &e = pl.e[s];
        bmp_ggnn_fwd_t f;
        memset(&f, 0, sizeof(f));
        f.mb = mb; f.n_atoms = N[s]; f.hidden = H; f.n_edge = 4; f.n_steps = T; f.n_atom_types = a->n_atom_types; f.mode = a->mode;
        f.atoms = atoms[s]; f.embed_W = a->embed_W; f.adj = reinterpret_cast<const float *>(adj[s]); f.adj_u8 = a->adj_u8;
        for (int t = 0; t < T; ++t) { f.msg_W[t] = a->msg_W[t]; f.msg_b[t] = a->msg_b[t]; f.gru[t] = a->gru[t]; f.stateful[t] = a->stateful[t]; }
        if (bf16) {
            f.h0_out = e.out2; f.h_out = e.out2 + RH; f.stash2 = e.stash2;
            f.tc_workspace = pl.tc_fwd; f.tc_workspace_bytes = pl.tc_bytes; f.tc_images_ready = s;
            hT[s] = e.out2 + RH; d_hT[s] = e.dout2 + RH;
        } else {
            f.Hs = e.Hs; f.Ms = e.Ms; f.Gs = e.Gs; f.RSs = e.RSs;
            f.tc_workspace = pl.x3_ws; f.tc_workspace_bytes = pl.x3_bytes; f.tc_images_ready = s;
            hT[s] = e.Hs + (size_t)T * RH; d_hT[s] = e.dHs + (size_t)T * RH;
        }
        if ((rc = bmp_ggnn_forward(&f, stream))) return rc;
    }
    bmp_coattn_fwd_t cf;
    memset(&cf, 0, sizeof(cf));
    cf.mb = mb; cf.n1 = a->n1; cf.n2 = a->n2; cf.hidden = H; cf.out_dim = O; cf.head = head; cf.variant = a->coattn_variant; cf.act = a->coattn_act;
    cf.atoms_1 = hT[0]; cf.atoms_2 = hT[1];
    cf.W = a->W; cf.V1 = a->V1; cf.V2 = a->V2; cf.b = a->b; cf.lt_1 = a->lt_1; cf.lt_2 = a->lt_2; cf.wa_1 = a->wa_1; cf.wa_2 = a->wa_2;
    cf.W_j = a->W_j; cf.b_j = a->b_j;
    cf.compact_1 = pl.c1; cf.compact_2 = pl.c2;
    cf.mode = a->mode; cf.tc_workspace = pl.co_ws; cf.tc_workspace_bytes = pl.co_bytes;
    if ((rc = bmp_coattn_forward(&cf, stream))) return rc;
    if ((rc = bmp_hole_corr_forward(pl.c1, pl.c2, pl.corr, mb, O, stream))) return rc;
    if ((rc = bmp_linear_forward(pl.corr, a->out_W, a->out_b, a->logits, mb, O, K, BMP_ACT_IDENTITY, stream))) return rc;
    if ((rc = bmp_sigmoid_ce(a->logits, a->labels, a->loss, pl.dlogits, mb * K, a->count, stream))) return rc;
    if ((rc = bmp_linear_backward(pl.corr, a->out_W, a->logits, pl.dlogits, pl.dcorr, a->d_out_W, a->d_out_b, mb, O, K, BMP_ACT_IDENTITY, stream)))
        return rc;
    if ((rc = bmp_hole_corr_backward(pl.c1, pl.c2, pl.dcorr, pl.dc1, pl.dc2, mb, O, stream))) return rc;
    for (int s = 0; s < 2; ++s) {
        const size_t RH = (size_t)mb * N[s] * H;
        if (bf16) cudaMemsetAsync(pl.e[s].dout2, 0, RH * sizeof(float), st);
        else cudaMemsetAsync(pl.e[s].dHs, 0, (size_t)T * RH * sizeof(float), st);
    }
    bmp_coattn_bwd_t cb;
    memset(&cb, 0, sizeof(cb));
    cb.mb = mb; cb.n1 = a->n1; cb.n2 = a->n2; cb.hidden = H; cb.out_dim = O; cb.head = head; cb.variant = a->coattn_variant; cb.act = a->coattn_act;
    cb.atoms_1 = hT[0]; cb.atoms_2 = hT[1];
    cb.W = a->W; cb.V1 = a->V1; cb.V2 = a->V2; cb.b = a->b; cb.lt_1 = a->lt_1; cb.lt_2 = a->lt_2; cb.wa_1 = a->wa_1; cb.wa_2 = a->wa_2;
    cb.W_j = a->W_j; cb.b_j = a->b_j;
    cb.d_compact_1 = pl.dc1; cb.d_compact_2 = pl.dc2;
    cb.R = pl.e[0].R; cb.P1 = pl.P1; cb.P2 = pl.P2; cb.DL1 = pl.e[0].DL; cb.DL2 = pl.e[1].DL;
    cb.d_atoms_1 = d_hT[0]; cb.d_atoms_2 = d_hT[1];
    cb.d_W = a->d_W; cb.d_V1 = a->d_V1; cb.d_V2 = a->d_V2; cb.d_b = a->d_b; cb.d_lt_1 = a->d_lt_1; cb.d_lt_2 = a->d_lt_2;
    cb.d_wa_1 = a->d_wa_1; cb.d_wa_2 = a->d_wa_2; cb.d_W_j = a->d_W_j; cb.d_b_j = a->d_b_j;
    cb.mode = a->mode; cb.tc_workspace = pl.co_ws; cb.tc_workspace_bytes = pl.co_bytes; cb.tc_images_ready = 1;
    if ((rc = bmp_coattn_backward(&cb, stream))) return rc;
    for (int s = 0; s < 2; ++s) {
        Enc &e = pl.e[s];
        bmp_ggnn_bwd_t g;
        memset(&g, 0, sizeof(g));
        g.mb = mb; g.n_atoms = N[s]; g.hidden = H; g.n_edge = 4; g.n_steps = T; g.mode = a->mode;
        g.adj = reinterpret_cast<const float *>(adj[s]); g.adj_u8 = a->adj_u8;
        for (int t = 0; t < T; ++t) {
            g.msg_W[t] = a->msg_W[t]; g.gru[t] = a->gru[t]; g.stateful[t] = a->stateful[t];
            g.d_msg_W[t] = a->d_msg_W[t]; g.d_msg_b[t] = a->d_msg_b[t]; g.d_gru[t] = a->d_gru[t];
        }
        if (bf16) {
            g.stash2 = e.stash2; g.dHs = e.dout2;
            g.tc_workspace = pl.tc_bwd; g.tc_workspace_bytes = pl.tc_bytes; g.tc_images_ready = s;
        } else {
            g.Hs = e.Hs; g.Ms = e.Ms; g.RSs = e.RSs; g.Gs = e.Gs; g.Ps = e.Ps; g.dHs = e.dHs;
            g.tc_workspace = pl.x3_ws; g.tc_workspace_bytes = pl.x3_bytes; g.tc_images_ready = 1;
        }
        if ((rc = bmp_ggnn_backward(&g, stream))) return rc;
        if (a->d_embed_W &&
            (rc = bmp_embed_backward(atoms[s], bf16 ? e.dout2 : e.dHs, a->d_embed_W, mb * N[s], H, a->n_atom_types, stream)))
            return rc;
    }
    return BMP_OK;
}
```

gcn-bmp_b200/gcnbmp/_capi.py:

```python
import ctypes as C
import os

_HERE = os.path.dirname(os.path.abspath(__file__))
LIB_PATH = os.path.join(_HERE, "libgcnbmp.so")

MAX_STEPS = 16
OK, EINVAL, ESHAPE, EARCH, ECUDA = 0, -1, -2, -3, -4
ACT = {"identity": 0, "tanh": 1, "relu": 2, "sigmoid": 3}
READOUT_R1, READOUT_R2, READOUT_SUM = 1, 2, 3
COATTN_FINE, COATTN_POOL = 0, 1
PAIR_SYM, PAIR_PROD, PAIR_CONCAT = 0, 1, 2
MODE_F32, MODE_BF16 = 0, 1

fp = C.c_void_p
_A = lambda: fp * MAX_STEPS


class GRU(C.Structure):
    _fields_ = [(n, fp) for n in ("W_r", "b_Wr", "U_r", "b_Ur", "W_z", "b_Wz", "U_z", "b_Uz", "W", "b_W", "U", "b_U")]


class GgnnFwd(C.Structure):
    _fields_ = [(n, C.c_int) for n in ("mb", "n_atoms", "hidden", "n_edge", "n_steps", "n_atom_types", "mode")] + [
        ("atoms", fp), ("h_in", fp), ("embed_W", fp), ("adj", fp), ("state_in", fp),
        ("msg_W", _A()), ("msg_b", _A()), ("gru", GRU * MAX_STEPS), ("stateful", C.c_int * MAX_STEPS),
        ("h_out", fp), ("h0_out", fp), ("Hs", fp), ("Ms", fp), ("Gs", fp), ("RSs", fp),
        ("tc_workspace", fp), ("tc_workspace_bytes", C.c_size_t), ("stash2", fp), ("tc_images_ready", C.c_int), ("adj_u8", C.c_int),
        ("mol_index", fp)]


class GgnnBwd(C.Structure):
    _fields_ = [(n, C.c_int) for n in ("mb", "n_atoms", "hidden", "n_edge", "n_steps", "mode")] + [
        ("adj", fp), ("state_in", fp), ("msg_W", _A()), ("gru", GRU * MAX_STEPS),
        ("stateful", C.c_int * MAX_STEPS), ("Hs", fp), ("Ms", fp), ("RSs", fp), ("Gs", fp), ("Ps", fp), ("dHs", fp),
        ("d_msg_W", _A()), ("d_msg_b", _A()), ("d_gru", GRU * MAX_STEPS), ("d_state_in", fp),
        ("tc_workspace", fp), ("tc_workspace_bytes", C.c_size_t), ("stash2", fp), ("tc_images_ready", C.c_int), ("adj_u8", C.c_int),
        ("mol_index", fp)]


class Pair(C.Structure):
    _fields_ = [(n, C.c_int) for n in ("mb", "n1", "n2", "hidden", "out_dim", "head", "n_classes", "n_steps", "n_atom_types", "mode",
                                       "coattn_variant", "coattn_act")] + [
        ("atoms_1", fp), ("atoms_2", fp), ("adj_1", fp), ("adj_2", fp), ("labels", fp), ("count", C.c_float), ("embed_W", fp),
        ("msg_W", _A()), ("msg_b", _A()), ("gru", GRU * MAX_STEPS), ("stateful", C.c_int * MAX_STEPS)] + [
        (n, fp) for n in ("W", "V1", "V2", "b", "lt_1", "lt_2", "wa_1", "wa_2", "W_j", "b_j", "out_W", "out_b", "d_embed_W")] + [
        ("d_msg_W", _A()), ("d_msg_b", _A()), ("d_gru", GRU * MAX_STEPS)] + [
        (n, fp) for n in ("d_W", "d_V1", "d_V2", "d_b", "d_lt_1", "d_lt_2", "d_wa_1", "d_wa_2", "d_W_j", "d_b_j", "d_out_W", "d_out_b",
                          "logits", "loss", "workspace")] + [("workspace_bytes", C.c_size_t), ("adj_u8", C.c_int)]


class Bimpm(C.Structure):
    _fields_ = [(n, C.c_int) for n in ("mb", "n1", "n2", "hidden", "head")] + [
        ("atoms_1", fp), ("atoms_2", fp), ("max_pooling_W", fp), ("att_mean_W", fp), ("att_max_W", fp),
        ("out_1", fp), ("out_2", fp), ("d_out_1", fp), ("d_out_2", fp), ("d_atoms_1", fp), ("d_atoms_2", fp),
        ("d_max_pooling_W", fp), ("d_att_mean_W", fp), ("d_att_max_W", fp), ("workspace", fp), ("workspace_bytes", C.c_size_t)]


class RelgcnFwd(C.Structure):
    _fields_ = [(n, C.c_int) for n in ("mb", "n_atoms", "n_edge", "n_layers", "n_atom_types", "scale_adj", "act")] + [
        ("ch", C.c_int * (MAX_STEPS + 1)), ("atoms", fp), ("h_in", fp), ("embed_W", fp), ("adj", fp),
        ("self_W", _A()), ("self_b", _A()), ("edge_W", _A()), ("edge_b", _A()), ("h_out", fp), ("Hs", fp),
        ("mode", C.c_int), ("tc_workspace", fp), ("tc_workspace_bytes", C.c_size_t), ("stash2", fp), ("tc_images_ready", C.c_int), ("adj_u8", C.c_int)]


class RelgcnBwd(C.Structure):
    _fields_ = [(n, C.c_int) for n in ("mb", "n_atoms", "n_edge", "n_layers", "scale_adj", "act")] + [
        ("ch", C.c_int * (MAX_STEPS + 1)), ("adj", fp), ("self_W", _A()), ("edge_W", _A()), ("Hs", fp),
        ("d_h_out", fp), ("Ds", fp), ("Ps", fp), ("d_h0", fp),
        ("d_self_W", _A()), ("d_self_b", _A()), ("d_edge_W", _A()), ("d_edge_b", _A()),
        ("mode", C.c_int), ("tc_workspace", fp), ("tc_workspace_bytes", C.c_size_t), ("stash2", fp), ("tc_images_ready", C.c_int), ("adj_u8", C.c_int)]


class ReadoutFwd(C.Structure):
    _fields_ = [(n, C.c_int) for n in ("mb", "n_atoms", "hidden", "out_dim", "variant", "act", "act_agg")] + [
        (n, fp) for n in ("h", "h0", "is_real_node", "W_i", "b_i", "W_j", "b_j", "g")] + [
        ("mode", C.c_int), ("tc_workspace", fp), ("tc_workspace_bytes", C.c_size_t), ("tc_images_ready", C.c_int)]


class ReadoutBwd(C.Structure):
    _fields_ = [(n, C.c_int) for n in ("mb", "n_atoms", "hidden", "out_dim", "variant", "act", "act_agg")] + [
        (n, fp) for n in ("h", "h0", "is_real_node", "W_i", "b_i", "W_j", "b_j", "g", "dg",
                          "DU", "DV", "dh", "dh0", "d_W_i", "d_b_i", "d_W_j", "d_b_j")] + [
        ("mode", C.c_int), ("tc_workspace", fp), ("tc_workspace_bytes", C.c_size_t), ("tc_images_ready", C.c_int)]


_CO_PARAMS = ("W", "V1", "V2", "b", "lt_1", "lt_2", "wa_1", "wa_2", "W_j", "b_j")


class CoattnFwd(C.Structure):
    _fields_ = [(n, C.c_int) for n in ("mb", "n1", "n2", "hidden", "out_dim", "head", "variant", "act")] + [
        (n, fp) for n in ("atoms_1", "atoms_2") + _CO_PARAMS + ("compact_1", "compact_2")] + [
        ("mode", C.c_int), ("tc_workspace", fp), ("tc_workspace_bytes", C.c_size_t), ("tc_images_ready", C.c_int)]


class CoattnBwd(C.Structure):
    _fields_ = [(n, C.c_int) for n in ("mb", "n1", "n2", "hidden", "out_dim", "head", "variant", "act")] + [
        (n, fp) for n in ("atoms_1", "atoms_2") + _CO_PARAMS + ("d_compact_1", "d_compact_2", "R", "P1", "P2",
                                                             "DL1", "DL2", "d_atoms_1", "d_atoms_2")
        + tuple("d_" + p for p in _CO_PARAMS)] + [
        ("mode", C.c_int), ("tc_workspace", fp), ("tc_workspace_bytes", C.c_size_t), ("tc_images_ready", C.c_int)]


def _load():
    if not os.path.exists(LIB_PATH):
        raise ImportError(
            "gcnbmp: %s is missing -- build it with `python gcn-bmp_b200/build.py` "
            "(there is no CPU fallback)" % LIB_PATH)
    lib = C.CDLL(LIB_PATH)
    i, i64, f, vp = C.c_int, C.c_int64, C.c_float, C.c_void_p
    sig = {
        "bmp_ggnn_forward": [C.POINTER(GgnnFwd), vp],
        "bmp_ggnn_backward": [C.POINTER(GgnnBwd), vp],
        "bmp_embed_backward": [fp, fp, fp, i, i, i, vp],
        "bmp_relgcn_forward": [C.POINTER(RelgcnFwd), vp],
        "bmp_relgcn_backward": [C.POINTER(RelgcnBwd), vp],
        "bmp_rescale_adj": [fp, fp, i, i, i, vp],
        "bmp_readout_forward": [C.POINTER(ReadoutFwd), vp],
        "bmp_readout_backward": [C.POINTER(ReadoutBwd), vp],
        "bmp_coattn_forward": [C.POINTER(CoattnFwd), vp],
        "bmp_coattn_backward": [C.POINTER(CoattnBwd), vp],
        "bmp_hole_corr_forward": [fp, fp, fp, i, i, vp],
        "bmp_hole_corr_backward": [fp, fp, fp, fp, fp, i, i, vp],
        "bmp_linear_forward": [fp, fp, fp, fp, i, i, i, i, vp],
        "bmp_linear_backward": [fp, fp, fp, fp, fp, fp, fp, i, i, i, i, vp],
        "bmp_wgrad": [fp, i, fp, i, fp, i, i64, i, i, vp],
        "bmp_wgrad_tc": [fp, i, fp, i, fp, i, i64, i, i, fp, i, vp],
        "bmp_wgrad_tc3": [fp, i, fp, i, fp, i, i64, i, i, fp, i, vp],
        "bmp_colsum": [fp, i, fp, i, i64, i, vp],
        "bmp_sigmoid_ce": [fp, fp, fp, fp, i, f, vp],
        "bmp_adam_step": [fp, fp, fp, fp, i, f, f, f, f, f, i, vp],
        "bmp_pair_features_forward": [fp, fp, fp, i, i, i, vp],
        "bmp_pair_features_backward": [fp, fp, fp, fp, fp, i, i, i, vp],
        "bmp_bilinear_forward": [fp, fp, fp, fp, fp, fp, fp, fp, i, i, i, i, vp],
        "bmp_bilinear_backward": [fp] * 14 + [i, i, i, i, vp],
        "bmp_grad_hooks": [fp, fp, i, f, f, f, fp, vp],
        "bmp_atoms_bcast_add_act_forward": [fp, fp, fp, i, i, i, i, vp],
        "bmp_atoms_bcast_add_act_backward": [fp, fp, fp, fp, i, i, i, i, vp],
        "bmp_atoms_softmax_forward": [fp, fp, i, i, i, vp],
        "bmp_atoms_softmax_backward": [fp, fp, fp, i, i, i, vp],
        "bmp_atoms_pool_forward": [fp, i, fp, fp, i, i, i, vp],
        "bmp_atoms_pool_backward": [fp, i, fp, fp, fp, fp, i, i, i, vp],
        "bmp_gin_aggregate": [fp, fp, fp, i, i, i, i, i, vp],
        "bmp_nfp_gather": [fp, fp, fp, i, i, i, i, i, vp],
        "bmp_bimpm_forward": [C.POINTER(Bimpm), vp],
        "bmp_bimpm_backward": [C.POINTER(Bimpm), vp],
        "bmp_embed_forward": [fp, fp, fp, i, i, i, vp],
    }
    for name, args in sig.items():
        fn = getattr(lib, name)
        fn.argtypes, fn.restype = args, C.c_int
    lib.bmp_ggnn_tc_workspace_bytes.argtypes, lib.bmp_ggnn_tc_workspace_bytes.restype = [i, i], C.c_size_t
    lib.bmp_ggnn_stash2_bytes.argtypes, lib.bmp_ggnn_stash2_bytes.restype = [i, i, i], C.c_size_t
    lib.bmp_ggnn_x3_workspace_bytes.argtypes, lib.bmp_ggnn_x3_workspace_bytes.restype = [i, i, i, i, i, i], C.c_size_t
    lib.bmp_pair_workspace_bytes.argtypes, lib.bmp_pair_workspace_bytes.restype = [i] * 9, C.c_size_t
    lib.bmp_pair_forward_backward.argtypes, lib.bmp_pair_forward_backward.restype = [C.c_void_p, vp], C.c_int
    lib.bmp_readout_tc_workspace_bytes.argtypes, lib.bmp_readout_tc_workspace_bytes.restype = [i, i], C.c_size_t
    lib.bmp_readout_x3_workspace_bytes.argtypes, lib.bmp_readout_x3_workspace_bytes.restype = [i] * 6, C.c_size_t
    lib.bmp_coattn_tc_workspace_bytes.argtypes, lib.bmp_coattn_tc_workspace_bytes.restype = [i], C.c_size_t
    lib.bmp_relgcn_tc_workspace_bytes.argtypes, lib.bmp_relgcn_tc_workspace_bytes.restype = [i, i], C.c_size_t
    lib.bmp_bimpm_workspace_bytes.argtypes, lib.bmp_bimpm_workspace_bytes.restype = [i, i, i, i, i], C.c_size_t
    lib.bmp_last_error.restype = C.c_char_p
    lib.bmp_version.restype = C.c_int
    lib.bmp_device_check.restype = C.c_int
    lib.bmp_launch_count.restype = C.c_uint64
    lib.bmp_reset_launch_count.restype = None
    lib.bmp_profile_enable.argtypes, lib.bmp_profile_enable.restype = [i], None
    lib.bmp_profile_read.argtypes, lib.bmp_profile_read.restype = [C.POINTER(C.c_double), C.POINTER(C.c_longlong), i], C.c_int
    return lib


lib = _load()
EXPORTS = ["bmp_ggnn_forward", "bmp_ggnn_backward", "bmp_embed_backward", "bmp_relgcn_forward",
           "bmp_relgcn_backward", "bmp_relgcn_tc_workspace_bytes", "bmp_rescale_adj", "bmp_readout_forward", "bmp_readout_backward", "bmp_readout_tc_workspace_bytes", "bmp_coattn_forward",
           "bmp_coattn_backward", "bmp_coattn_tc_workspace_bytes", "bmp_hole_corr_forward", "bmp_hole_corr_backward", "bmp_linear_forward",
           "bmp_linear_backward", "bmp_ggnn_tc_workspace_bytes", "bmp_ggnn_stash2_bytes", "bmp_ggnn_x3_workspace_bytes", "bmp_pair_workspace_bytes", "bmp_pair_forward_backward", "bmp_readout_x3_workspace_bytes", "bmp_wgrad", "bmp_wgrad_tc", "bmp_wgrad_tc3", "bmp_colsum", "bmp_sigmoid_ce", "bmp_adam_step",
           "bmp_pair_features_forward", "bmp_pair_features_backward", "bmp_bilinear_forward", "bmp_bilinear_backward", "bmp_grad_hooks",
           "bmp_atoms_bcast_add_act_forward", "bmp_atoms_bcast_add_act_backward", "bmp_atoms_softmax_forward", "bmp_atoms_softmax_backward",
           "bmp_atoms_pool_forward", "bmp_atoms_pool_backward", "bmp_gin_aggregate", "bmp_nfp_gather", "bmp_embed_forward", "bmp_bimpm_forward", "bmp_bimpm_backward", "bmp_bimpm_workspace_bytes",
           "bmp_last_error", "bmp_version", "bmp_device_check", "bmp_launch_count", "bmp_reset_launch_count",
           "bmp_profile_enable", "bmp_profile_read"]


class BmpError(RuntimeError):
    def __init__(self, code, msg):
        RuntimeError.__init__(self, "gcnbmp error %d: %s" % (code, msg))
        self.code = code


def check(rc):
    if rc != 0:
        msg = lib.bmp_last_error().decode("utf-8", "replace")
        if rc == ESHAPE:
            raise ValueError("gcnbmp: %s" % msg)
        raise BmpError(rc, msg)


def launch_count():
    return int(lib.bmp_launch_count())


def reset_launch_count():
    lib.bmp_reset_launch_count()


PROF_KINDS = ("ggnn_fwd", "ggnn_bwd", "wgrad", "coattn_fwd", "coattn_bwd", "readout")


def profile_enable(on=True):
    lib.bmp_profile_enable(1 if on else 0)


def profile_read():
    n = len(PROF_KINDS)
    ms, cnt = (C.c_double * n)(), (C.c_longlong * n)()
    check(lib.bmp_profile_read(ms, cnt, n))
    return {k: (float(ms[j]), int(cnt[j])) for j, k in enumerate(PROF_KINDS)}
```

gcn-bmp_b200/gcnbmp/functional.py:

```python
import ctypes as C

import torch

from . import _capi as K


def _p(t):
    return None if t is None else C.c_void_p(t.data_ptr())


def _stream():
    return C.c_void_p(torch.cuda.current_stream().cuda_stream)


def adj_format(t):
    if t.dtype in (torch.uint8, torch.bool):
        n, w = t.shape[-2], t.shape[-1]
        return 2 if (t.dtype == torch.uint8 and w == (n + 7) // 8 and w != n) else 1
    return 0


def pack_adjacency(adj):
    if isinstance(adj, torch.Tensor):
        n = adj.shape[-1]
        w = (n + 7) // 8
        b = (adj != 0).to(torch.uint8)
        if w * 8 != n:
            b = torch.nn.functional.pad(b, (0, w * 8 - n))
        b = b.reshape(b.shape[:-1] + (w, 8))
        weights = (1 << torch.arange(8, device=b.device, dtype=torch.int32))
        return (b.to(torch.int32) * weights).sum(dim=-1).to(torch.uint8)
    import numpy as np
    return np.packbits(np.asarray(adj) != 0, axis=-1, bitorder="little")


def unpack_adjacency(bits, n_atoms=None):
    n = bits.shape[-2] if n_atoms is None else n_atoms
    sh = torch.arange(8, device=bits.device, dtype=torch.int32)
    x = ((bits.to(torch.int32).unsqueeze(-1) >> sh) & 1).reshape(bits.shape[:-1] + (bits.shape[-1] * 8,))
    return x[..., :n].to(torch.float32).contiguous()


def _adj(t, mode):
    fmt = adj_format(t)
    if fmt == 2 and mode != K.MODE_BF16:
        return unpack_adjacency(t), 0
    if mode == K.MODE_BF16 and fmt:
        t = t.contiguous()
        return (t.view(torch.uint8) if t.dtype == torch.bool else t), fmt
    return _f32(t), 0


def _f32(t):
    if t is None:
        return None
    if t.dtype != torch.float32 or not t.is_contiguous():
        t = t.contiguous().float()
    return t


def _need_cuda(*ts):
    for t in ts:
        if t is not None and not t.is_cuda:
            raise RuntimeError("gcnbmp: tensors must live on a CUDA device (no CPU fallback)")


def act_code(a):
    if a is None:
        return K.ACT["identity"]
    name = a if isinstance(a, str) else getattr(a, "__name__", str(a))
    if name not in K.ACT:
        raise ValueError("gcnbmp: unsupported activation %r" % (a,))
    return K.ACT[name]


GRU_FIELDS = ("W_r", "b_Wr", "U_r", "b_Ur", "W_z", "b_Wz", "U_z", "b_Uz", "W", "b_W", "U", "b_U")


def _fill_gru(dst, tensors):
    for name, t in zip(GRU_FIELDS, tensors):
        setattr(dst, name, _p(t))


_WEIGHT_CACHE = False
_PARAM_EPOCH = 0
_IMAGES = {}


def set_weight_cache(flag):
    global _WEIGHT_CACHE
    _WEIGHT_CACHE = bool(flag)
    if not flag:
        _IMAGES.clear()


def params_changed():
    global _PARAM_EPOCH
    _PARAM_EPOCH += 1
    _IMAGES.clear()


def _tc_images(kind, nbytes, dev, params):
    if not _WEIGHT_CACHE:
        return torch.empty((nbytes,), device=dev, dtype=torch.uint8), 0
    key = (kind, nbytes, str(dev)) + tuple(p.data_ptr() if p is not None else 0 for p in params)
    ent = _IMAGES.get(key)
    if ent is not None and ent[1] == _PARAM_EPOCH:
        return ent[0], 1
    ws = torch.empty((nbytes,), device=dev, dtype=torch.uint8)
    _IMAGES[key] = (ws, _PARAM_EPOCH, tuple(params))
    return ws, 0


F32_TENSOR_CORES = True


def _x3_workspace(a, mb, N, H, E, T, dev, params, inference):
    if not F32_TENSOR_CORES:
        return None
    nbytes = int(K.lib.bmp_ggnn_x3_workspace_bytes(mb, N, H, E, T, int(inference)))
    if nbytes == 0:
        return None
    ws, a.tc_images_ready = _tc_images("ggnn_x3", nbytes, dev, params)
    a.tc_workspace, a.tc_workspace_bytes = _p(ws), nbytes
    return ws


_GRAD_SINK = False


def set_grad_sink(flag):
    global _GRAD_SINK
    _GRAD_SINK = bool(flag)


def _grad_targets(params):
    bufs, rets = [], []
    for p in params:
        if p is None:
            bufs.append(None)
            rets.append(None)
        elif (_GRAD_SINK and p.is_leaf and p.requires_grad and p.grad is not None and p.grad.dtype == torch.float32
              and p.grad.is_contiguous() and p.grad.shape == p.shape):
            bufs.append(p.grad)
            rets.append(None)
        else:
            z = torch.zeros_like(p)
            bufs.append(z)
            rets.append(z)
    return bufs, rets


class GGNNEncode(torch.autograd.Function):

    @staticmethod
    def forward(ctx, x, adj, state_in, plan, n_msg, n_gru, mode, want_stash, keep_steps, mol_index, *params):
        _need_cuda(x, adj)
        if mol_index is not None and (mode != K.MODE_BF16 or x.dtype not in (torch.int32, torch.int64)):
            x, adj, mol_index = x.index_select(0, mol_index.long()), adj.index_select(0, mol_index.long()), None
        adj, adj_u8 = _adj(adj, mode)
        mb, E, N, _ = adj.shape
        if mol_index is not None:
            mol_index = mol_index.to(torch.int32).contiguous()
            mb = mol_index.shape[0]
        embed_W = params[0]
        msg = [(params[1 + 2 * i], params[2 + 2 * i]) for i in range(n_msg)]
        base = 1 + 2 * n_msg
        gru = [params[base + 12 * i: base + 12 * (i + 1)] for i in range(n_gru)]
        H = msg[0][0].shape[1]
        T = len(plan)
        a = K.GgnnFwd()
        a.mb, a.n_atoms, a.hidden, a.n_edge, a.n_steps, a.mode = mb, N, H, E, T, mode
        is_ids = x.dtype in (torch.int32, torch.int64)
        if is_ids:
            x = x.to(torch.int32).contiguous()
            a.atoms, a.embed_W, a.n_atom_types = _p(x), _p(embed_W), embed_W.shape[0]
        else:
            x = _f32(x)
            a.h_in = _p(x)
        state_in = _f32(state_in)
        a.adj, a.state_in, a.adj_u8, a.mol_index = _p(adj), _p(state_in), adj_u8, _p(mol_index)
        for t, (mi, gi, st) in enumerate(plan):
            a.msg_W[t], a.msg_b[t] = _p(msg[mi][0]), _p(msg[mi][1])
            _fill_gru(a.gru[t], gru[gi])
            a.stateful[t] = int(st)
        dev = adj.device
        rows = mb * N
        if mode == K.MODE_BF16:
            nbytes = int(K.lib.bmp_ggnn_tc_workspace_bytes(H, T))
            if nbytes == 0:
                raise ValueError("gcnbmp: BMP_MODE_BF16 supports hidden 64, 128 or (forward only) 256 (got %d)" % H)
            if want_stash and H == 256:
                raise ValueError("gcnbmp: BMP_MODE_BF16 at hidden 256 is forward-only (call under torch.no_grad(), "
                                 "or train in MODE_F32)")
            ws, a.tc_images_ready = _tc_images("ggnn_fwd", nbytes, dev, params)
            a.tc_workspace, a.tc_workspace_bytes = _p(ws), nbytes
        if want_stash and mode == K.MODE_BF16 and not keep_steps:
            out = torch.empty((2, mb, N, H), device=dev, dtype=torch.float32)
            stash2 = torch.empty((int(K.lib.bmp_ggnn_stash2_bytes(mb, H, T)),), device=dev, dtype=torch.uint8)
            a.h0_out, a.h_out, a.stash2 = _p(out[0]), _p(out[1]), _p(stash2)
            K.check(K.lib.bmp_ggnn_forward(C.byref(a), _stream()))
            ctx.save_for_backward(x, adj, state_in, stash2, None, None, None, *params)
            ctx.mol_index = mol_index
            ctx.meta = (plan, n_msg, n_gru, mode, is_ids, (mb, N, H))
            return out
        x3ws = None
        if mode == K.MODE_F32 and state_in is None and mol_index is None and not adj_u8:
            x3ws = _x3_workspace(a, mb, N, H, E, T, dev, params, not want_stash)
        if want_stash:
            Hs = torch.empty((T + 1, mb, N, H), device=dev, dtype=torch.float32)
            Ms = torch.empty((T, rows, H), device=dev, dtype=torch.float32)
            Gs = torch.empty((T, rows, 3 * H), device=dev, dtype=torch.float32)
            RSs = torch.empty((T, rows, H), device=dev, dtype=torch.float32)
            a.Hs, a.Ms, a.Gs, a.RSs = _p(Hs), _p(Ms), _p(Gs), _p(RSs)
            K.check(K.lib.bmp_ggnn_forward(C.byref(a), _stream()))
            ctx.save_for_backward(x, adj, state_in, Hs, Ms, Gs, RSs, *params)
            ctx.mol_index = mol_index
            ctx.meta = (plan, n_msg, n_gru, mode, is_ids, None)
            ctx.x3 = x3ws is not None
            return Hs
        out = torch.empty((2, mb, N, H), device=dev, dtype=torch.float32)
        a.h0_out, a.h_out = _p(out[0]), _p(out[1])
        K.check(K.lib.bmp_ggnn_forward(C.byref(a), _stream()))
        return out

    @staticmethod
    def backward(ctx, dHs):
        x, adj, state_in, Hs, Ms, Gs, RSs = ctx.saved_tensors[:7]
        params = ctx.saved_tensors[7:]
        plan, n_msg, n_gru, mode, is_ids, v2shape = ctx.meta
        T = len(plan)
        E = adj.shape[1]
        stash2 = None
        if v2shape is not None:
            stash2, Hs = Hs, None
            mb, N, H = v2shape
        else:
            _, mb, N, H = Hs.shape
        rows = mb * N
        dHs = dHs.contiguous().clone()
        grads, rets = _grad_targets(params)
        Ps = torch.empty((T, rows, E * H), device=adj.device, dtype=torch.float32) if stash2 is None else None
        a = K.GgnnBwd()
        a.mb, a.n_atoms, a.hidden, a.n_edge, a.n_steps, a.mode = mb, N, H, E, T, mode
        mol_index = ctx.mol_index
        a.adj, a.state_in, a.adj_u8, a.mol_index = _p(adj), _p(state_in), adj_format(adj), _p(mol_index)
        base = 1 + 2 * n_msg
        for t, (mi, gi, st) in enumerate(plan):
            a.msg_W[t] = _p(params[1 + 2 * mi])
            _fill_gru(a.gru[t], params[base + 12 * gi: base + 12 * (gi + 1)])
            a.stateful[t] = int(st)
            a.d_msg_W[t], a.d_msg_b[t] = _p(grads[1 + 2 * mi]), _p(grads[2 + 2 * mi])
            _fill_gru(a.d_gru[t], grads[base + 12 * gi: base + 12 * (gi + 1)])
        a.Hs, a.Ms, a.RSs, a.Gs, a.Ps, a.dHs = _p(Hs), _p(Ms), _p(RSs), _p(Gs), _p(Ps), _p(dHs)
        a.stash2 = _p(stash2)
        d_state = torch.zeros_like(state_in) if state_in is not None else None
        a.d_state_in = _p(d_state)
        if mode == K.MODE_BF16:
            nbytes = int(K.lib.bmp_ggnn_tc_workspace_bytes(H, T))
            ws, a.tc_images_ready = _tc_images("ggnn_bwd", nbytes, adj.device, params)
            a.tc_workspace, a.tc_workspace_bytes = _p(ws), nbytes
        if mode == K.MODE_F32 and getattr(ctx, "x3", False):
            _x3_workspace(a, mb, N, H, E, T, adj.device, params, False)
        K.check(K.lib.bmp_ggnn_backward(C.byref(a), _stream()))
        dx = None
        if is_ids:
            ids = x if mol_index is None else x.index_select(0, mol_index.long()).contiguous()
            K.check(K.lib.bmp_embed_backward(_p(ids), _p(dHs[0]), _p(grads[0]), rows, H, grads[0].shape[0], _stream()))
        else:
            dx = dHs[0]
            rets[0] = None
        return (dx, None, d_state, None, None, None, None, None, None, None) + tuple(rets)


class RelGCNEncode(torch.autograd.Function):

    @staticmethod
    def forward(ctx, x, adj, ch, scale_adj, act, want_stash, mode, *params):
        _need_cuda(x, adj)
        adj, adj_u8 = _adj(adj, mode)
        mb, E, N, _ = adj.shape
        L = len(ch) - 1
        tc = mode == K.MODE_BF16 and int(K.lib.bmp_relgcn_tc_workspace_bytes(ch[0], L)) > 0 and len(set(ch)) == 1 and E == 4
        if mode == K.MODE_BF16 and not tc:
            raise ValueError("gcnbmp: BMP_MODE_BF16 RelGCN needs one channel count in {64,128} for all layers and 4 bond types "
                             "(got %r, %d bond types)" % (tuple(ch), E))
        a = K.RelgcnFwd()
        a.mb, a.n_atoms, a.n_edge, a.n_layers, a.scale_adj, a.act = mb, N, E, L, int(bool(scale_adj)), act
        for l, c in enumerate(ch):
            a.ch[l] = c
        is_ids = x.dtype in (torch.int32, torch.int64)
        if is_ids:
            x = x.to(torch.int32).contiguous()
            a.atoms, a.embed_W, a.n_atom_types = _p(x), _p(params[0]), params[0].shape[0]
        else:
            x = _f32(x)
            a.h_in = _p(x)
        a.adj, a.adj_u8 = _p(adj), adj_u8
        for l in range(L):
            Ws, bs, We, be = params[1 + 4 * l: 5 + 4 * l]
            a.self_W[l], a.self_b[l], a.edge_W[l], a.edge_b[l] = _p(Ws), _p(bs), _p(We), _p(be)
        rows = mb * N
        h_out = torch.empty((mb, N, ch[-1]), device=adj.device, dtype=torch.float32)
        a.h_out = _p(h_out)
        Hs = None
        if tc:
            nbytes = int(K.lib.bmp_relgcn_tc_workspace_bytes(ch[0], L))
            ws, a.tc_images_ready = _tc_images("relgcn_fwd", nbytes, adj.device, params)
            a.mode, a.tc_workspace, a.tc_workspace_bytes = K.MODE_BF16, _p(ws), nbytes
            if want_stash:
                Hs = torch.empty((int(K.lib.bmp_ggnn_stash2_bytes(mb, ch[0], L)),), device=adj.device, dtype=torch.uint8)
                a.stash2 = _p(Hs)
        elif want_stash:
            Hs = torch.empty((rows * sum(ch),), device=adj.device, dtype=torch.float32)
            a.Hs = _p(Hs)
        K.check(K.lib.bmp_relgcn_forward(C.byref(a), _stream()))
        if want_stash:
            ctx.save_for_backward(x, adj, Hs, *params)
            ctx.meta = (tuple(ch), int(bool(scale_adj)), act, is_ids, tc)
        return h_out

    @staticmethod
    def backward(ctx, d_out):
        x, adj, Hs = ctx.saved_tensors[:3]
        params = ctx.saved_tensors[3:]
        ch, scale_adj, act, is_ids, tc = ctx.meta
        mb, E, N, _ = adj.shape
        L = len(ch) - 1
        rows = mb * N
        dev = adj.device
        d_out = _f32(d_out)
        grads, rets = _grad_targets(params)
        Ds = Ps = None
        if not tc:
            Ds = torch.empty((rows * sum(ch[1:]),), device=dev, dtype=torch.float32)
            Ps = torch.empty((rows * E * sum(ch[1:]),), device=dev, dtype=torch.float32)
        d_h0 = torch.empty((mb, N, ch[0]), device=dev, dtype=torch.float32)
        a = K.RelgcnBwd()
        if tc:
            nbytes = int(K.lib.bmp_relgcn_tc_workspace_bytes(ch[0], L))
            ws, a.tc_images_ready = _tc_images("relgcn_bwd", nbytes, dev, params)
            a.mode, a.tc_workspace, a.tc_workspace_bytes, a.stash2 = K.MODE_BF16, _p(ws), nbytes, _p(Hs)
            Hs = None
        a.mb, a.n_atoms, a.n_edge, a.n_layers, a.scale_adj, a.act = mb, N, E, L, scale_adj, act
        for l, c in enumerate(ch):
            a.ch[l] = c
        a.adj, a.Hs, a.d_h_out, a.Ds, a.Ps, a.d_h0 = _p(adj), _p(Hs), _p(d_out), _p(Ds), _p(Ps), _p(d_h0)
        a.adj_u8 = adj_format(adj)
        for l in range(L):
            Ws, bs, We, be = params[1 + 4 * l: 5 + 4 * l]
            a.self_W[l], a.edge_W[l] = _p(Ws), _p(We)
            gWs, gbs, gWe, gbe = grads[1 + 4 * l: 5 + 4 * l]
            a.d_self_W[l], a.d_self_b[l], a.d_edge_W[l], a.d_edge_b[l] = _p(gWs), _p(gbs), _p(gWe), _p(gbe)
        K.check(K.lib.bmp_relgcn_backward(C.byref(a), _stream()))
        dx = None
        if is_ids:
            K.check(K.lib.bmp_embed_backward(_p(x), _p(d_h0), _p(grads[0]), rows, ch[0], grads[0].shape[0], _stream()))
        else:
            dx = d_h0
            rets[0] = None
        return (dx, None, None, None, None, None, None) + tuple(rets)


def _readout_ws(a, mode, H, O, variant, dev, params):
    a.mode = K.MODE_F32
    if mode == K.MODE_BF16 and variant != K.READOUT_SUM:
        nbytes = int(K.lib.bmp_readout_tc_workspace_bytes(H, O))
        if nbytes:
            ws, a.tc_images_ready = _tc_images("readout", nbytes, dev, params)
            a.mode, a.tc_workspace, a.tc_workspace_bytes = K.MODE_BF16, _p(ws), nbytes
            return ws
    if mode == K.MODE_F32 and F32_TENSOR_CORES and variant != K.READOUT_SUM and isinstance(a, K.ReadoutFwd):
        nbytes = int(K.lib.bmp_readout_x3_workspace_bytes(a.mb, a.n_atoms, H, O, variant, int(bool(a.h0))))
        if nbytes:
            ws, a.tc_images_ready = _tc_images("readout_x3", nbytes, dev, params)
            a.tc_workspace, a.tc_workspace_bytes = _p(ws), nbytes
            return ws
    return None


MAX_KERNEL_ATOMS = 64
_TORCH_ACT = {0: (lambda x: x), 1: torch.tanh, 2: torch.relu, 3: torch.sigmoid}


def _readout_large(h, h0, mask, variant, act, act_agg, W_i, b_i, W_j, b_j):
    if variant == K.READOUT_SUM:
        return h.sum(dim=1)
    h1 = torch.cat((h, h0), dim=2) if h0 is not None else h
    gi = torch.sigmoid(torch.nn.functional.linear(h1, W_i, b_i))
    gj = _TORCH_ACT[act](torch.nn.functional.linear(h1 if variant == K.READOUT_R1 else h, W_j, b_j))
    g = gi * gj
    if mask is not None:
        g = g * mask.reshape(mask.shape[0], mask.shape[1], 1)
    return _TORCH_ACT[act_agg](g.sum(dim=1))


def readout(h, h0, mask, variant, act, act_agg, W_i, b_i, W_j, b_j, mode=0):
    kcat = h.shape[2] * (2 if h0 is not None else 1)
    too_wide = variant != K.READOUT_SUM and torch.is_grad_enabled() and kcat + 2 * W_i.shape[0] > 836
    if h.shape[1] > MAX_KERNEL_ATOMS or too_wide:
        return _readout_large(_f32(h), _f32(h0), _f32(mask), variant, act, act_agg, W_i, b_i, W_j, b_j)
    return Readout.apply(h, h0, mask, variant, act, act_agg, W_i, b_i, W_j, b_j, mode)


def _coattention_large(a1, a2, variant, act, W, V1, V2, b, lt_1, lt_2, wa_1, wa_2, W_j, b_j):
    H = a1.shape[2]
    C = torch.matmul(a2, torch.matmul(a1, W.reshape(H, H)).transpose(1, 2))
    C = C + torch.matmul(a1, V1.reshape(H, 1)).transpose(1, 2) + torch.matmul(a2, V2.reshape(H, 1)) + b.reshape(1, 1, 1)
    C = _TORCH_ACT[act](C)
    if variant == K.COATTN_POOL:
        attn_1 = torch.softmax(C.mean(dim=1), dim=1)
        attn_2 = torch.softmax(C.mean(dim=2), dim=1)
    else:
        L_2 = torch.softmax(C, dim=1)
        L_1 = torch.softmax(C.transpose(1, 2), dim=1)
        l1, l2 = torch.matmul(a1, lt_1.t()), torch.matmul(a2, lt_2.t())
        H_1 = torch.tanh(l1 + torch.matmul(L_1, l2))
        H_2 = torch.tanh(l2 + torch.matmul(L_2, l1))
        attn_1 = torch.softmax(torch.matmul(H_1, wa_1.t()), dim=1)[:, :, 0]
        attn_2 = torch.softmax(torch.matmul(H_2, wa_2.t()), dim=1)[:, :, 0]
    j1 = torch.nn.functional.linear(a1, W_j, b_j)
    j2 = torch.nn.functional.linear(a2, W_j, b_j)
    return (attn_1.unsqueeze(2) * j1).sum(dim=1), (attn_2.unsqueeze(2) * j2).sum(dim=1)


def coattention(atoms_1, atoms_2, variant, act, W, V1, V2, b, lt_1, lt_2, wa_1, wa_2, W_j, b_j, mode=0):
    if max(atoms_1.shape[1], atoms_2.shape[1]) > MAX_KERNEL_ATOMS or atoms_1.shape[2] > 192:
        return _coattention_large(_f32(atoms_1), _f32(atoms_2), variant, act, W, V1, V2, b, lt_1, lt_2, wa_1, wa_2, W_j, b_j)
    return Coattention.apply(atoms_1, atoms_2, variant, act, W, V1, V2, b, lt_1, lt_2, wa_1, wa_2, W_j, b_j, mode)


class Readout(torch.autograd.Function):

    @staticmethod
    def forward(ctx, h, h0, mask, variant, act, act_agg, W_i, b_i, W_j, b_j, mode=0):
        _need_cuda(h)
        h, h0, mask = _f32(h), _f32(h0), _f32(mask)
        mb, N, H = h.shape
        O = H if variant == K.READOUT_SUM else W_i.shape[0]
        g = torch.empty((mb, O), device=h.device, dtype=torch.float32)
        a = K.ReadoutFwd()
        a.mb, a.n_atoms, a.hidden, a.out_dim, a.variant, a.act, a.act_agg = mb, N, H, O, variant, act, act_agg
        a.h, a.h0, a.is_real_node = _p(h), _p(h0), _p(mask)
        a.W_i, a.b_i, a.W_j, a.b_j, a.g = _p(W_i), _p(b_i), _p(W_j), _p(b_j), _p(g)
        ws = _readout_ws(a, mode, H, O, variant, h.device, (W_i, W_j))
        K.check(K.lib.bmp_readout_forward(C.byref(a), _stream()))
        ctx.save_for_backward(h, h0, mask, W_i, b_i, W_j, b_j, g)
        ctx.meta = (variant, act, act_agg, mode)
        return g

    @staticmethod
    def backward(ctx, dg):
        h, h0, mask, W_i, b_i, W_j, b_j, g = ctx.saved_tensors
        variant, act, act_agg, mode = ctx.meta
        mb, N, H = h.shape
        O = g.shape[1]
        dev = h.device
        dg = _f32(dg)
        z = lambda t: torch.zeros_like(t) if t is not None else None
        dh, dh0 = torch.zeros_like(h), z(h0)
        (gWi, gbi, gWj, gbj), rets = _grad_targets([W_i, b_i, W_j, b_j])
        a = K.ReadoutBwd()
        a.mb, a.n_atoms, a.hidden, a.out_dim, a.variant, a.act, a.act_agg = mb, N, H, O, variant, act, act_agg
        a.h, a.h0, a.is_real_node = _p(h), _p(h0), _p(mask)
        a.W_i, a.b_i, a.W_j, a.b_j, a.g, a.dg = _p(W_i), _p(b_i), _p(W_j), _p(b_j), _p(g), _p(dg)
        if variant != K.READOUT_SUM:
            DU = torch.empty((mb * N, O), device=dev, dtype=torch.float32)
            DV = torch.empty((mb * N, O), device=dev, dtype=torch.float32)
            a.DU, a.DV = _p(DU), _p(DV)
        a.dh, a.dh0 = _p(dh), _p(dh0)
        a.d_W_i, a.d_b_i, a.d_W_j, a.d_b_j = _p(gWi), _p(gbi), _p(gWj), _p(gbj)
        ws = _readout_ws(a, mode, H, O, variant, dev, (W_i, W_j))
        K.check(K.lib.bmp_readout_backward(C.byref(a), _stream()))
        return (dh, dh0, None, None, None, None) + tuple(rets) + (None,)


def _coattn_workspace(a, mode, H, dev, params):
    if mode != K.MODE_BF16:
        return None
    n = int(K.lib.bmp_coattn_tc_workspace_bytes(H))
    if not n:
        return None
    ws, a.tc_images_ready = _tc_images("coattn", n, dev, params)
    a.tc_workspace, a.tc_workspace_bytes = _p(ws), n
    return ws


class Coattention(torch.autograd.Function):

    @staticmethod
    def forward(ctx, atoms_1, atoms_2, variant, act, W, V1, V2, b, lt_1, lt_2, wa_1, wa_2, W_j, b_j, mode=0):
        _need_cuda(atoms_1, atoms_2)
        atoms_1, atoms_2 = _f32(atoms_1), _f32(atoms_2)
        mb, n1, H = atoms_1.shape
        n2 = atoms_2.shape[1]
        O = W_j.shape[0]
        head = lt_1.shape[0] if lt_1 is not None else 0
        c1 = torch.empty((mb, O), device=atoms_1.device, dtype=torch.float32)
        c2 = torch.empty_like(c1)
        a = K.CoattnFwd()
        a.mb, a.n1, a.n2, a.hidden, a.out_dim, a.head, a.variant, a.act = mb, n1, n2, H, O, head, variant, act
        a.atoms_1, a.atoms_2 = _p(atoms_1), _p(atoms_2)
        ps = (W, V1, V2, b, lt_1, lt_2, wa_1, wa_2, W_j, b_j)
        for n, t in zip(K._CO_PARAMS, ps):
            setattr(a, n, _p(t))
        a.compact_1, a.compact_2 = _p(c1), _p(c2)
        a.mode = mode
        ws = _coattn_workspace(a, mode, H, atoms_1.device, ps)
        K.check(K.lib.bmp_coattn_forward(C.byref(a), _stream()))
        ctx.save_for_backward(atoms_1, atoms_2, *ps)
        ctx.meta = (variant, act, head, mode)
        return c1, c2

    @staticmethod
    def backward(ctx, dc1, dc2):
        atoms_1, atoms_2 = ctx.saved_tensors[:2]
        ps = ctx.saved_tensors[2:]
        variant, act, head, mode = ctx.meta
        mb, n1, H = atoms_1.shape
        n2 = atoms_2.shape[1]
        O = ps[8].shape[0]
        dev = atoms_1.device
        dc1, dc2 = _f32(dc1), _f32(dc2)
        grads, rets = _grad_targets(ps)
        da1, da2 = torch.empty_like(atoms_1), torch.empty_like(atoms_2)
        e = lambda *s: torch.empty(s, device=dev, dtype=torch.float32)
        R, P1, P2 = e(mb * n1, H), e(mb, H), e(mb, H)
        DL1 = e(mb * n1, head) if head else None
        DL2 = e(mb * n2, head) if head else None
        a = K.CoattnBwd()
        a.mb, a.n1, a.n2, a.hidden, a.out_dim, a.head, a.variant, a.act = mb, n1, n2, H, O, head, variant, act
        a.atoms_1, a.atoms_2 = _p(atoms_1), _p(atoms_2)
        for n, t, g in zip(K._CO_PARAMS, ps, grads):
            setattr(a, n, _p(t))
            setattr(a, "d_" + n, _p(g))
        a.d_compact_1, a.d_compact_2 = _p(dc1), _p(dc2)
        a.R, a.P1, a.P2, a.DL1, a.DL2 = _p(R), _p(P1), _p(P2), _p(DL1), _p(DL2)
        a.d_atoms_1, a.d_atoms_2 = _p(da1), _p(da2)
        a.mode = mode
        ws = _coattn_workspace(a, mode, H, dev, ps)
        K.check(K.lib.bmp_coattn_backward(C.byref(a), _stream()))
        return (da1, da2, None, None) + tuple(rets) + (None,)


class HoleCorr(torch.autograd.Function):

    @staticmethod
    def forward(ctx, left, right):
        _need_cuda(left, right)
        left, right = _f32(left), _f32(right)
        mb, D = left.shape
        out = torch.empty_like(left)
        K.check(K.lib.bmp_hole_corr_forward(_p(left), _p(right), _p(out), mb, D, _stream()))
        ctx.save_for_backward(left, right)
        return out

    @staticmethod
    def backward(ctx, d_out):
        left, right = ctx.saved_tensors
        mb, D = left.shape
        d_out = _f32(d_out)
        dl, dr = torch.empty_like(left), torch.empty_like(right)
        K.check(K.lib.bmp_hole_corr_backward(_p(left), _p(right), _p(d_out), _p(dl), _p(dr), mb, D, _stream()))
        return dl, dr


class PairFeatures(torch.autograd.Function):

    @staticmethod
    def forward(ctx, left, right, kind):
        _need_cuda(left, right)
        left, right = _f32(left), _f32(right)
        if left.shape != right.shape or left.dim() != 2:
            raise ValueError("gcnbmp: pair features need two (mb, D) arrays of one shape, got %s and %s" % (tuple(left.shape), tuple(right.shape)))
        mb, D = left.shape
        out = torch.empty((mb, D if kind == K.PAIR_PROD else 2 * D), device=left.device, dtype=torch.float32)
        K.check(K.lib.bmp_pair_features_forward(_p(left), _p(right), _p(out), mb, D, kind, _stream()))
        ctx.save_for_backward(left, right)
        ctx.kind = kind
        return out

    @staticmethod
    def backward(ctx, d_out):
        left, right = ctx.saved_tensors
        mb, D = left.shape
        d_out = _f32(d_out)
        dl, dr = torch.empty_like(left), torch.empty_like(right)
        K.check(K.lib.bmp_pair_features_backward(_p(left), _p(right), _p(d_out), _p(dl), _p(dr), mb, D, ctx.kind, _stream()))
        return dl, dr, None


class Bilinear(torch.autograd.Function):

    @staticmethod
    def forward(ctx, e1, e2, W, V1, V2, b):
        _need_cuda(e1, e2)
        e1, e2 = _f32(e1), _f32(e2)
        mb, L = e1.shape
        R, Ko = W.shape[1], W.shape[2]
        if e2.shape != (mb, R) or W.shape[0] != L:
            raise ValueError("gcnbmp: Bilinear shapes e1 %s e2 %s W %s" % (tuple(e1.shape), tuple(e2.shape), tuple(W.shape)))
        u = torch.empty((mb, R * Ko), device=e1.device, dtype=torch.float32)
        y = torch.empty((mb, Ko), device=e1.device, dtype=torch.float32)
        K.check(K.lib.bmp_bilinear_forward(_p(e1), _p(e2), _p(W), _p(V1), _p(V2), _p(b), _p(u), _p(y), mb, L, R, Ko, _stream()))
        ctx.save_for_backward(e1, e2, W, V1, V2, b, u)
        return y

    @staticmethod
    def backward(ctx, dy):
        e1, e2, W, V1, V2, b, u = ctx.saved_tensors
        mb, L = e1.shape
        R, Ko = W.shape[1], W.shape[2]
        dy = _f32(dy)
        du = torch.empty_like(u)
        de1, de2 = torch.empty_like(e1), torch.empty_like(e2)
        (dW, dV1, dV2, db), rets = _grad_targets([W, V1, V2, b])
        K.check(K.lib.bmp_bilinear_backward(_p(e1), _p(e2), _p(W), _p(V1), _p(V2), _p(u), _p(dy), _p(du), _p(de1), _p(de2),
                                            _p(dW), _p(dV1), _p(dV2), _p(db), mb, L, R, Ko, _stream()))
        return (de1, de2) + tuple(rets)


class AtomsBcastAddAct(torch.autograd.Function):

    @staticmethod
    def forward(ctx, x, v, n_atoms, act):
        t = x if x is not None else v
        _need_cuda(t)
        x, v = _f32(x), _f32(v)
        if x is not None:
            mb, n_atoms, ch = x.shape
        else:
            mb, ch = v.shape
        if v is not None and tuple(v.shape) != (mb, ch):
            raise ValueError("gcnbmp: broadcast vector %s does not match atoms %s" % (tuple(v.shape), (mb, n_atoms, ch)))
        y = torch.empty((mb, n_atoms, ch), device=t.device, dtype=torch.float32)
        K.check(K.lib.bmp_atoms_bcast_add_act_forward(_p(x), _p(v), _p(y), mb, n_atoms, ch, act, _stream()))
        ctx.save_for_backward(y)
        ctx.meta = (x is not None, v is not None, act)
        return y

    @staticmethod
    def backward(ctx, dy):
        (y,) = ctx.saved_tensors
        has_x, has_v, act = ctx.meta
        mb, n, ch = y.shape
        dy = _f32(dy)
        dx = torch.empty_like(y) if has_x else None
        dv = torch.empty((mb, ch), device=y.device, dtype=torch.float32) if has_v else None
        K.check(K.lib.bmp_atoms_bcast_add_act_backward(_p(y), _p(dy), _p(dx), _p(dv), mb, n, ch, act, _stream()))
        return dx, dv, None, None


class AtomsSoftmax(torch.autograd.Function):

    @staticmethod
    def forward(ctx, x):
        _need_cuda(x)
        x = _f32(x)
        mb, n, ch = x.shape
        y = torch.empty_like(x)
        K.check(K.lib.bmp_atoms_softmax_forward(_p(x), _p(y), mb, n, ch, _stream()))
        ctx.save_for_backward(y)
        return y

    @staticmethod
    def backward(ctx, dy):
        (y,) = ctx.saved_tensors
        mb, n, ch = y.shape
        dx = torch.empty_like(y)
        K.check(K.lib.bmp_atoms_softmax_backward(_p(y), _p(_f32(dy)), _p(dx), mb, n, ch, _stream()))
        return dx


class AtomsPool(torch.autograd.Function):

    @staticmethod
    def forward(ctx, attn, z):
        _need_cuda(attn, z)
        attn, z = _f32(attn), _f32(z)
        mb, n, ch = z.shape
        if attn.shape[:2] != z.shape[:2] or attn.shape[2] not in (1, ch):
            raise ValueError("gcnbmp: attention %s does not pool atoms %s" % (tuple(attn.shape), tuple(z.shape)))
        out = torch.empty((mb, ch), device=z.device, dtype=torch.float32)
        K.check(K.lib.bmp_atoms_pool_forward(_p(attn), attn.shape[2], _p(z), _p(out), mb, n, ch, _stream()))
        ctx.save_for_backward(attn, z)
        return out

    @staticmethod
    def backward(ctx, d_out):
        attn, z = ctx.saved_tensors
        mb, n, ch = z.shape
        da, dz = torch.empty_like(attn), torch.empty_like(z)
        K.check(K.lib.bmp_atoms_pool_backward(_p(attn), attn.shape[2], _p(z), _p(_f32(d_out)), _p(da), _p(dz), mb, n, ch, _stream()))
        return da, dz


class GINAggregate(torch.autograd.Function):

    @staticmethod
    def forward(ctx, h, adj):
        _need_cuda(h, adj)
        h, adj = _f32(h), _f32(adj)
        mb, E, N, _ = adj.shape
        H = h.shape[2]
        out = torch.empty_like(h)
        K.check(K.lib.bmp_gin_aggregate(_p(adj), _p(h), _p(out), mb, E, N, H, 0, _stream()))
        ctx.save_for_backward(adj)
        return out

    @staticmethod
    def backward(ctx, d_out):
        (adj,) = ctx.saved_tensors
        mb, E, N, _ = adj.shape
        d_out = _f32(d_out)
        dh = torch.empty_like(d_out)
        K.check(K.lib.bmp_gin_aggregate(_p(adj), _p(d_out), _p(dh), mb, E, N, d_out.shape[2], 1, _stream()))
        return dh, None


class BiMPMMatch(torch.autograd.Function):

    @staticmethod
    def _args(a1, a2, Wm, Wa, Wx):
        mb, N1, H = a1.shape
        a = K.Bimpm()
        a.mb, a.n1, a.n2, a.hidden, a.head = mb, N1, a2.shape[1], H, Wm.shape[0]
        a.atoms_1, a.atoms_2 = _p(a1), _p(a2)
        a.max_pooling_W, a.att_mean_W, a.att_max_W = _p(Wm), _p(Wa), _p(Wx)
        n = int(K.lib.bmp_bimpm_workspace_bytes(mb, N1, a2.shape[1], H, Wm.shape[0]))
        ws = torch.empty((max(n, 4),), device=a1.device, dtype=torch.uint8)
        a.workspace, a.workspace_bytes = _p(ws), n
        return a, ws

    @staticmethod
    def forward(ctx, a1, a2, Wm, Wa, Wx):
        _need_cuda(a1, a2)
        a1, a2, Wm, Wa, Wx = _f32(a1), _f32(a2), _f32(Wm), _f32(Wa), _f32(Wx)
        if a1.shape[0] != a2.shape[0] or a1.shape[2] != a2.shape[2] or tuple(Wm.shape) != tuple(Wa.shape) != tuple(Wx.shape):
            raise ValueError("gcnbmp: BiMPM shapes %s %s %s" % (tuple(a1.shape), tuple(a2.shape), tuple(Wm.shape)))
        a, ws = BiMPMMatch._args(a1, a2, Wm, Wa, Wx)
        o1 = torch.empty((a.mb, 3 * a.head), device=a1.device, dtype=torch.float32)
        o2 = torch.empty_like(o1)
        a.out_1, a.out_2 = _p(o1), _p(o2)
        K.check(K.lib.bmp_bimpm_forward(C.byref(a), _stream()))
        ctx.save_for_backward(a1, a2, Wm, Wa, Wx)
        return o1, o2

    @staticmethod
    def backward(ctx, g1, g2):
        a1, a2, Wm, Wa, Wx = ctx.saved_tensors
        a, ws = BiMPMMatch._args(a1, a2, Wm, Wa, Wx)
        g1 = _f32(g1) if g1 is not None else torch.zeros((a.mb, 3 * a.head), device=a1.device)
        g2 = _f32(g2) if g2 is not None else torch.zeros((a.mb, 3 * a.head), device=a1.device)
        d1, d2 = torch.empty_like(a1), torch.empty_like(a2)
        (gm, ga, gx), rets = _grad_targets([Wm, Wa, Wx])
        a.d_out_1, a.d_out_2, a.d_atoms_1, a.d_atoms_2 = _p(g1), _p(g2), _p(d1), _p(d2)
        a.d_max_pooling_W, a.d_att_mean_W, a.d_att_max_W = _p(gm), _p(ga), _p(gx)
        K.check(K.lib.bmp_bimpm_backward(C.byref(a), _stream()))
        return (d1, d2) + tuple(rets)


class EmbedID(torch.autograd.Function):

    @staticmethod
    def forward(ctx, ids, W):
        _need_cuda(ids, W)
        ids = ids.to(torch.int32).contiguous()
        W = _f32(W)
        out = torch.empty(tuple(ids.shape) + (W.shape[1],), device=W.device, dtype=torch.float32)
        K.check(K.lib.bmp_embed_forward(_p(ids), _p(W), _p(out), ids.numel(), W.shape[1], W.shape[0], _stream()))
        ctx.save_for_backward(ids, W)
        return out

    @staticmethod
    def backward(ctx, d_out):
        ids, W = ctx.saved_tensors
        (gW,), rets = _grad_targets([W])
        K.check(K.lib.bmp_embed_backward(_p(ids), _p(_f32(d_out)), _p(gW), ids.numel(), W.shape[1], W.shape[0], _stream()))
        return None, rets[0]


class NFPGather(torch.autograd.Function):

    @staticmethod
    def forward(ctx, h, adj, n_degree):
        _need_cuda(h, adj)
        h, adj = _f32(h), _f32(adj)
        mb, N, C = h.shape
        if tuple(adj.shape) != (mb, N, N):
            raise ValueError("gcnbmp: NFP takes the (mb, N, N) adjacency of its preprocessor, got %s" % (tuple(adj.shape),))
        X = torch.empty((mb, N, n_degree * C), device=h.device, dtype=torch.float32)
        K.check(K.lib.bmp_nfp_gather(_p(adj), _p(h), _p(X), mb, N, C, n_degree, 0, _stream()))
        ctx.save_for_backward(adj)
        ctx.meta = (C, n_degree)
        return X

    @staticmethod
    def backward(ctx, dX):
        (adj,) = ctx.saved_tensors
        C, D = ctx.meta
        mb, N, _ = adj.shape
        dh = torch.empty((mb, N, C), device=adj.device, dtype=torch.float32)
        K.check(K.lib.bmp_nfp_gather(_p(adj), _p(_f32(dX)), _p(dh), mb, N, C, D, 1, _stream()))
        return dh, None, None


class Linear(torch.autograd.Function):

    @staticmethod
    def forward(ctx, x, W, b, act):
        _need_cuda(x)
        x = _f32(x)
        rows, in_dim = x.shape
        out_dim = W.shape[0]
        y = torch.empty((rows, out_dim), device=x.device, dtype=torch.float32)
        K.check(K.lib.bmp_linear_forward(_p(x), _p(W), _p(b), _p(y), rows, in_dim, out_dim, act, _stream()))
        ctx.save_for_backward(x, W, b, y)
        ctx.act = act
        return y

    @staticmethod
    def backward(ctx, dy):
        x, W, b, y = ctx.saved_tensors
        rows, in_dim = x.shape
        out_dim = W.shape[0]
        dy = dy.contiguous().float().clone()
        dx = torch.empty_like(x)
        (dW, db), rets = _grad_targets([W, b])
        K.check(K.lib.bmp_linear_backward(_p(x), _p(W), _p(y), _p(dy), _p(dx), _p(dW), _p(db),
                                          rows, in_dim, out_dim, ctx.act, _stream()))
        return dx, rets[0], rets[1], None


class SigmoidCrossEntropy(torch.autograd.Function):

    @staticmethod
    def forward(ctx, x, t, count):
        _need_cuda(x)
        x = _f32(x)
        t = t.to(torch.int32).contiguous()
        if count is None:
            count = float(max(int((t != -1).sum().item()), 1))
        loss = torch.zeros((), device=x.device, dtype=torch.float32)
        dx = torch.empty_like(x)
        K.check(K.lib.bmp_sigmoid_ce(_p(x), _p(t), _p(loss), _p(dx), x.numel(), float(count), _stream()))
        ctx.save_for_backward(dx)
        return loss

    @staticmethod
    def backward(ctx, g):
        return ctx.saved_tensors[0] * g, None, None


def sigmoid_cross_entropy(x, t, count=None):
    return SigmoidCrossEntropy.apply(x, t, count)
```

include/gcnbmp.h:

```cpp
#ifndef GCNBMP_H_
#define GCNBMP_H_

#include <stdint.h>
#include <stddef.h>

#ifdef __cplusplus
extern "C" {
#endif

#define BMP_OK       0
#define BMP_EINVAL  -1
#define BMP_ESHAPE  -2
#define BMP_EARCH   -3
#define BMP_ECUDA   -4

#define BMP_MAX_STEPS   16
#define BMP_MAX_ATOMS   64
#define BMP_X3_MAX_ATOMS 256
#define BMP_MAX_HIDDEN 256

enum { BMP_ACT_IDENTITY = 0, BMP_ACT_TANH = 1, BMP_ACT_RELU = 2, BMP_ACT_SIGMOID = 3 };
enum { BMP_READOUT_R1 = 1, BMP_READOUT_R2 = 2, BMP_READOUT_SUM = 3 };
enum { BMP_COATTN_FINE = 0, BMP_COATTN_POOL = 1 };
enum { BMP_MODE_F32 = 0,
       BMP_MODE_BF16 = 1 };

typedef struct {
    const float *W_r, *b_Wr, *U_r, *b_Ur;
    const float *W_z, *b_Wz, *U_z, *b_Uz;
    const float *W,   *b_W,  *U,   *b_U;
} bmp_gru_t;

typedef struct {
    float *W_r, *b_Wr, *U_r, *b_Ur;
    float *W_z, *b_Wz, *U_z, *b_Uz;
    float *W,   *b_W,  *U,   *b_U;
} bmp_gru_grad_t;

typedef struct {
    int mb, n_atoms, hidden, n_edge, n_steps, n_atom_types, mode;
    const int32_t *atoms;
    const float   *h_in;
    const float   *embed_W;
    const float   *adj;
    const float   *state_in;
    const float   *msg_W[BMP_MAX_STEPS];
    const float   *msg_b[BMP_MAX_STEPS];
    bmp_gru_t      gru[BMP_MAX_STEPS];
    int            stateful[BMP_MAX_STEPS];
    float *h_out;
    float *h0_out;
    float *Hs, *Ms, *Gs, *RSs;
    void  *tc_workspace;
    size_t tc_workspace_bytes;
    void  *stash2;
    int    tc_images_ready;
    int    adj_u8;
    const int32_t *mol_index;
} bmp_ggnn_fwd_t;

int bmp_ggnn_forward(const bmp_ggnn_fwd_t *a, void *stream);
size_t bmp_ggnn_tc_workspace_bytes(int hidden, int n_steps);
size_t bmp_ggnn_x3_workspace_bytes(int mb, int n_atoms, int hidden, int n_edge, int n_steps, int inference);
size_t bmp_ggnn_stash2_bytes(int mb, int hidden, int n_steps);

typedef struct {
    int mb, n_atoms, hidden, n_edge, n_steps, mode;
    const float *adj, *state_in;
    const float *msg_W[BMP_MAX_STEPS];
    bmp_gru_t    gru[BMP_MAX_STEPS];
    int          stateful[BMP_MAX_STEPS];
    const float *Hs, *Ms, *RSs;
    float *Gs, *Ps, *dHs;
    float *d_msg_W[BMP_MAX_STEPS], *d_msg_b[BMP_MAX_STEPS];
    bmp_gru_grad_t d_gru[BMP_MAX_STEPS];
    float *d_state_in;
    void  *tc_workspace;
    size_t tc_workspace_bytes;
    void  *stash2;
    int    tc_images_ready;
    int    adj_u8;
    const int32_t *mol_index;
} bmp_ggnn_bwd_t;

int bmp_ggnn_backward(const bmp_ggnn_bwd_t *a, void *stream);

int bmp_embed_backward(const int32_t *atoms, const float *dh, float *d_embed_W,
                       int rows, int hidden, int n_atom_types, void *stream);

typedef struct {
    int mb, n_atoms, n_edge, n_layers, n_atom_types, scale_adj;
    int act;
    int ch[BMP_MAX_STEPS + 1];
    const int32_t *atoms;  const float *h_in;  const float *embed_W;
    const float *adj;
    const float *self_W[BMP_MAX_STEPS], *self_b[BMP_MAX_STEPS];
    const float *edge_W[BMP_MAX_STEPS], *edge_b[BMP_MAX_STEPS];
    float *h_out;
    float *Hs;
    int    mode;
    void  *tc_workspace;
    size_t tc_workspace_bytes;
    void  *stash2;
    int    tc_images_ready;
    int    adj_u8;
} bmp_relgcn_fwd_t;

int bmp_relgcn_forward(const bmp_relgcn_fwd_t *a, void *stream);
size_t bmp_relgcn_tc_workspace_bytes(int channels, int n_layers);
int bmp_rescale_adj(const float *adj, float *adj_out, int mb, int n_edge, int n_atoms, void *stream);

typedef struct {
    int mb, n_atoms, n_edge, n_layers, scale_adj, act;
    int ch[BMP_MAX_STEPS + 1];
    const float *adj;
    const float *self_W[BMP_MAX_STEPS], *edge_W[BMP_MAX_STEPS];
    const float *Hs;
    const float *d_h_out;
    float *Ds, *Ps, *d_h0;
    float *d_self_W[BMP_MAX_STEPS], *d_self_b[BMP_MAX_STEPS];
    float *d_edge_W[BMP_MAX_STEPS], *d_edge_b[BMP_MAX_STEPS];
    int    mode;
    void  *tc_workspace;
    size_t tc_workspace_bytes;
    void  *stash2;
    int    tc_images_ready;
    int    adj_u8;
} bmp_relgcn_bwd_t;

int bmp_relgcn_backward(const bmp_relgcn_bwd_t *a, void *stream);

typedef struct {
    int mb, n_atoms, hidden, out_dim, variant, act, act_agg;
    const float *h, *h0, *is_real_node;
    const float *W_i, *b_i, *W_j, *b_j;
    float *g;
    int    mode;
    void  *tc_workspace;
    size_t tc_workspace_bytes;
    int    tc_images_ready;
} bmp_readout_fwd_t;

int bmp_readout_forward(const bmp_readout_fwd_t *a, void *stream);
size_t bmp_readout_tc_workspace_bytes(int hidden, int out_dim);
size_t bmp_readout_x3_workspace_bytes(int mb, int n_atoms, int hidden, int out_dim, int variant, int has_h0);

typedef struct {
    int mb, n_atoms, hidden, out_dim, variant, act, act_agg;
    const float *h, *h0, *is_real_node;
    const float *W_i, *b_i, *W_j, *b_j;
    const float *g, *dg;
    float *DU, *DV, *dh, *dh0;
    float *d_W_i, *d_b_i, *d_W_j, *d_b_j;
    int    mode;
    void  *tc_workspace;
    size_t tc_workspace_bytes;
    int    tc_images_ready;
} bmp_readout_bwd_t;

int bmp_readout_backward(const bmp_readout_bwd_t *a, void *stream);

typedef struct {
    int mb, n1, n2, hidden, out_dim, head, variant, act;
    const float *atoms_1, *atoms_2;
    const float *W, *V1, *V2, *b, *lt_1, *lt_2, *wa_1, *wa_2, *W_j, *b_j;
    float *compact_1, *compact_2;
    int    mode;
    void  *tc_workspace;
    size_t tc_workspace_bytes;
    int    tc_images_ready;
} bmp_coattn_fwd_t;

int bmp_coattn_forward(const bmp_coattn_fwd_t *a, void *stream);

typedef struct {
    int mb, n1, n2, hidden, out_dim, head, variant, act;
    const float *atoms_1, *atoms_2;
    const float *W, *V1, *V2, *b, *lt_1, *lt_2, *wa_1, *wa_2, *W_j, *b_j;
    const float *d_compact_1, *d_compact_2;
    float *R, *P1, *P2, *DL1, *DL2;
    float *d_atoms_1, *d_atoms_2;
    float *d_W, *d_V1, *d_V2, *d_b, *d_lt_1, *d_lt_2, *d_wa_1, *d_wa_2, *d_W_j, *d_b_j;
    int    mode;
    void  *tc_workspace;
    size_t tc_workspace_bytes;
    int    tc_images_ready;
} bmp_coattn_bwd_t;

int bmp_coattn_backward(const bmp_coattn_bwd_t *a, void *stream);
size_t bmp_coattn_tc_workspace_bytes(int hidden);

int bmp_hole_corr_forward(const float *left, const float *right, float *out,
                          int mb, int dim, void *stream);
int bmp_hole_corr_backward(const float *left, const float *right, const float *d_out,
                           float *d_left, float *d_right, int mb, int dim, void *stream);

int bmp_linear_forward(const float *x, const float *W, const float *b, float *y,
                       int rows, int in_dim, int out_dim, int act, void *stream);
int bmp_linear_backward(const float *x, const float *W, const float *y, float *dy,
                        float *dx, float *dW, float *db,
                        int rows, int in_dim, int out_dim, int act, void *stream);

int bmp_wgrad(const float *A, int lda, const float *B, int ldb, float *C, int ldc,
              int64_t rows, int M, int N, void *stream);
int bmp_wgrad_tc(const float *A, int lda, const float *B, int ldb, float *C, int ldc,
                 int64_t rows, int M, int N, float *dbias, int bias_stride, void *stream);
int bmp_wgrad_tc3(const float *A, int lda, const float *B, int ldb, float *C, int ldc,
                 int64_t rows, int M, int N, float *dbias, int bias_stride, void *stream);
int bmp_colsum(const float *B, int ldb, float *out, int out_stride, int64_t rows, int N, void *stream);

int bmp_sigmoid_ce(const float *logits, const int32_t *labels, float *loss_sum,
                   float *d_logits, int n, float count, void *stream);

int bmp_adam_step(float *param, const float *grad, float *m, float *v, int n,
                  float alpha, float beta1, float beta2, float eps,
                  float weight_decay_rate, int step, void *stream);

typedef struct {
    int mb, n1, n2, hidden, out_dim, head, n_classes, n_steps, n_atom_types, mode;
    int coattn_variant, coattn_act;
    const int32_t *atoms_1, *atoms_2;
    const void    *adj_1, *adj_2;
    const int32_t *labels;
    float count;
    const float *embed_W;
    const float *msg_W[BMP_MAX_STEPS], *msg_b[BMP_MAX_STEPS];
    bmp_gru_t    gru[BMP_MAX_STEPS];
    int          stateful[BMP_MAX_STEPS];
    const float *W, *V1, *V2, *b, *lt_1, *lt_2, *wa_1, *wa_2, *W_j, *b_j;
    const float *out_W, *out_b;
    float *d_embed_W;
    float *d_msg_W[BMP_MAX_STEPS], *d_msg_b[BMP_MAX_STEPS];
    bmp_gru_grad_t d_gru[BMP_MAX_STEPS];
    float *d_W, *d_V1, *d_V2, *d_b, *d_lt_1, *d_lt_2, *d_wa_1, *d_wa_2, *d_W_j, *d_b_j;
    float *d_out_W, *d_out_b;
    float *logits, *loss;
    void  *workspace;
    size_t workspace_bytes;
    int    adj_u8;
} bmp_pair_t;

size_t bmp_pair_workspace_bytes(int mb, int n1, int n2, int hidden, int out_dim, int head, int n_classes, int n_steps, int mode);
int bmp_pair_forward_backward(const bmp_pair_t *a, void *stream);

enum { BMP_PAIR_SYM = 0, BMP_PAIR_PROD = 1, BMP_PAIR_CONCAT = 2 };
int bmp_pair_features_forward(const float *left, const float *right, float *out, int rows, int dim, int kind, void *stream);
int bmp_pair_features_backward(const float *left, const float *right, const float *d_out, float *d_left, float *d_right,
                               int rows, int dim, int kind, void *stream);

int bmp_bilinear_forward(const float *e1, const float *e2, const float *W, const float *V1, const float *V2, const float *b,
                         float *u, float *y, int rows, int left, int right, int out, void *stream);
int bmp_bilinear_backward(const float *e1, const float *e2, const float *W, const float *V1, const float *V2, const float *u,
                          const float *dy, float *du, float *de1, float *de2, float *dW, float *dV1, float *dV2, float *db,
                          int rows, int left, int right, int out, void *stream);

int bmp_atoms_bcast_add_act_forward(const float *x, const float *v, float *y, int mb, int n_atoms, int ch, int act, void *stream);
int bmp_atoms_bcast_add_act_backward(const float *y, const float *dy, float *dx, float *dv, int mb, int n_atoms, int ch, int act, void *stream);
int bmp_atoms_softmax_forward(const float *x, float *y, int mb, int n_atoms, int ch, void *stream);
int bmp_atoms_softmax_backward(const float *y, const float *dy, float *dx, int mb, int n_atoms, int ch, void *stream);
int bmp_atoms_pool_forward(const float *a, int a_ch, const float *z, float *out, int mb, int n_atoms, int ch, void *stream);
int bmp_atoms_pool_backward(const float *a, int a_ch, const float *z, const float *d_out, float *da, float *dz,
                            int mb, int n_atoms, int ch, void *stream);

int bmp_gin_aggregate(const float *adj, const float *h, float *out, int mb, int n_edge, int n_atoms, int hidden,
                      int transpose, void *stream);

int bmp_grad_hooks(float *grad, const float *param, int n, float clip_threshold, float l2_rate, float l1_rate,
                   float *norm_ws, void *stream);

const char *bmp_last_error(void);
int         bmp_version(void);
int         bmp_device_check(void);
uint64_t    bmp_launch_count(void);
void        bmp_reset_launch_count(void);

typedef struct {
    int mb, n1, n2, hidden, head;
    const float *atoms_1, *atoms_2;
    const float *max_pooling_W, *att_mean_W, *att_max_W;
    float *out_1, *out_2;
    const float *d_out_1, *d_out_2;
    float *d_atoms_1, *d_atoms_2;
    float *d_max_pooling_W, *d_att_mean_W, *d_att_max_W;
    void  *workspace;
    size_t workspace_bytes;
} bmp_bimpm_t;
size_t bmp_bimpm_workspace_bytes(int mb, int n1, int n2, int hidden, int head);
int bmp_bimpm_forward(const bmp_bimpm_t *a, void *stream);
int bmp_bimpm_backward(const bmp_bimpm_t *a, void *stream);

int bmp_embed_forward(const int32_t *atoms, const float *embed_W, float *out, int rows, int hidden, int n_atom_types, void *stream);
int bmp_nfp_gather(const float *adj, const float *src, float *dst, int mb, int n_atoms, int ch, int n_degree, int backward,
                   void *stream);

enum { BMP_PROF_GGNN_FWD = 0, BMP_PROF_GGNN_BWD = 1, BMP_PROF_WGRAD = 2, BMP_PROF_COATTN_FWD = 3, BMP_PROF_COATTN_BWD = 4,
       BMP_PROF_READOUT = 5, BMP_PROF_KINDS = 6 };
void bmp_profile_enable(int on);
int  bmp_profile_read(double *ms, long long *launches, int n_kinds);

#ifdef __cplusplus
}
#endif
#endif
```

Measured before the change: 414,500.

## Split W_j projection out of co-attention kernel into batched linear GEMMs

Moves the per-pair W_j projection (forward compact outputs and backward dP from d_compact) out of the persistent tensor-core co-attention kernel into separate batched linear kernels, with pooled vectors passed through new P/DP workspaces. Inside the kernel it also fuses the softmax normalisation into fewer passes, folds the attention score dot product into the tanh epilogue, parallelises the pooling reduction, and merges an extra MMA tile into the last weight tile. This removes per-pair scalar GEMV work and several barriers from the kernel. The cost is extra kernel launches and global round-trips for the pooled vectors.

After: 422,800 (median of 6 runs). +2.0%, better.

```diff
diff --git a/gcn-bmp_b200/csrc/coattn_tc.cu b/gcn-bmp_b200/csrc/coattn_tc.cu
--- a/gcn-bmp_b200/csrc/coattn_tc.cu
+++ b/gcn-bmp_b200/csrc/coattn_tc.cu
@@ -14,12 +14,12 @@
 #define CTS(i) do { if (a.dbg && blockIdx.x == 0 && tid == 0 && it == 1) a.dbg[i] = clock64(); } while (0)
 
 struct Args {
-    int mb, n1, n2, O, head, act, pool;
-    const float *atoms_1, *atoms_2, *b, *wa_1, *wa_2, *W_j, *b_j, *lt_2, *V2;
+    int mb, n1, n2, head, act, pool;
+    const float *atoms_1, *atoms_2, *b, *wa_1, *wa_2, *lt_2, *V2;
     const uint8_t *img1, *img2, *img1x;
-    float *c1, *c2;
-    const float *dc1, *dc2;
-    float *R, *P1, *P2, *DL1, *DL2, *d_a1, *d_a2;
+    float *P1, *P2;
+    const float *DP1, *DP2;
+    float *d_a1, *d_a2;
     float *d_W, *d_lt_1, *d_lt_2, *d_V1, *d_V2, *d_b, *d_wa_1, *d_wa_2;
     long long *dbg;
 };
@@ -43,7 +43,7 @@
     hd = hd <= 8 ? 8 : 16;
     int n = AT * CLD + 2 * AT * PLD + 4;
     n += 4 * hd * AT;
-    n += 4 * AT + 2 * H;
+    n += 4 * AT;
     n += 4 * AT + 16 * AT;
     if (bwd) n += 2 * H + 2 * hd * AT + 2 * 16 + 4;
     return (n + 3) & ~3;
@@ -63,6 +63,9 @@
 }
 __device__ __forceinline__ float bf16_at(const uint8_t *panels, int row, int col) {
     return __bfloat162float(*reinterpret_cast<const __nv_bfloat16 *>(panels + (col >> 6) * PANEL_BYTES + sw128(row, col & 63)));
+}
+__device__ __forceinline__ uint64_t desc_mn16(uint32_t saddr) {
+    return (uint64_t)((saddr >> 4) & 0x3FFF) | ((uint64_t)(2048 >> 4) << 16) | (64ull << 32) | (1ull << 46) | (2ull << 61);
 }
 __device__ __forceinline__ uint4 pack8(const float *v) {
     return make_uint4(pack_bf16(v[0], v[1]), pack_bf16(v[2], v[3]), pack_bf16(v[4], v[5]), pack_bf16(v[6], v[7]));
@@ -79,7 +82,7 @@
     const uint32_t s_xp = sbase + C::OFF_XP, s_qp = sbase + C::OFF_QP, s_w = sbase + C::OFF_W, s_sp = sbase + C::OFF_SP,
                    s_dp = sbase + C::OFF_DP;
     uint8_t *XP = smem + C::OFF_XP, *QP = smem + C::OFF_QP, *SP = smem + C::OFF_SP, *DP = smem + C::OFF_DP;
-    const int hd = a.head, N1 = a.n1, N2 = a.n2, O = a.O;
+    const int hd = a.head, N1 = a.n1, N2 = a.n2;
     const bool pool = a.pool != 0;
     float *fp = reinterpret_cast<float *>(smem + C::OFF_F);
     float *Cs = fp; fp += AT * CLD;
@@ -93,8 +96,6 @@
     float *attn2 = fp; fp += AT;
     float *v1 = fp; fp += AT;
     float *v2 = fp; fp += AT;
-    float *p1 = fp; fp += H;
-    float *p2 = fp; fp += H;
     float *st4 = fp; fp += 4 * AT;
     float *part = fp; fp += 16 * AT;
     float *dp1 = fp, *dp2 = fp + H, *dpre1 = fp + 2 * H, *dpre2 = dpre1 + HS * AT;
@@ -143,8 +144,8 @@
                 for (int kt = 0; kt < KP; ++kt) put(a.img1 + (size_t)kt * C::W1_TILE, C::W1_TILE);
                 if (BWD) {
                     for (int kt = 0; kt < KP; ++kt) put(a.img2 + (size_t)kt * C::WH_TILE, C::WH_TILE);
-                    for (int kt = 0; kt < KP; ++kt) put(a.img1 + (size_t)kt * C::W1_TILE, C::WH_TILE);
-                    put(a.img1x, C::WH_TILE);
+                    for (int kt = 0; kt < KP - 1; ++kt) put(a.img1 + (size_t)kt * C::W1_TILE, C::WH_TILE);
+                    put(a.img1x, C::W1_TILE);
                 }
             }
         }
@@ -153,12 +154,13 @@
             constexpr uint32_t ID_G1 = idesc2(H + 32, 0, 0), ID_H = idesc2(H, 0, 0), ID_64 = idesc2(64, 0, 0), ID_HMN = idesc2(H, 0, 1),
                                ID_WMN = idesc2(H, 1, 1), ID_X = idesc2(16, 1, 1);
             uint32_t stage = 0, phase = 0, it = 0;
-            auto mma_wtile = [&](uint32_t a_addr, uint32_t dcol, uint32_t id, bool first, int ksteps) {
+            auto mma_wtile = [&](uint32_t a_addr, uint32_t dcol, uint32_t id, bool first, int ksteps, bool ext = false) {
                 mbar_wait(BAR(B_FULL + stage), phase);
                 tc_fence_after();
                 const uint32_t b_addr = s_w + stage * C::W1_TILE;
                 for (int k = 0; k < ksteps; ++k)
                     tc_mma(tmem + dcol, desc_kmajor(a_addr + k * 32), desc_kmajor(b_addr + k * 32), id, (first && k == 0) ? 0u : 1u);
+                if (ext) tc_mma(tmem + dcol, desc_kmajor(s_qp), desc_mn16(b_addr + H * 128), ID_HMN, 1u);
                 tc_commit(BAR(B_EMPTY + stage));
                 if (++stage == STAGES) { stage = 0; phase ^= 1; }
             };
@@ -199,8 +201,7 @@
                     tc_commit(BAR(B_A2));
                     mbar_wait(BAR(B_RRDY), par);
                     tc_fence_after();
-                    for (int kp = 0; kp < KP; ++kp) mma_wtile(s_sp + kp * PANEL_BYTES, C::COL_A1, ID_H, kp == 0, 4);
-                    mma_wtile(s_qp, C::COL_A1, ID_H, false, 1);
+                    for (int kp = 0; kp < KP; ++kp) mma_wtile(s_sp + kp * PANEL_BYTES, C::COL_A1, ID_H, kp == 0, 4, kp == KP - 1);
 #pragma unroll
                     for (int k = 0; k < 4; ++k) {
                         tc_mma(tmem + C::COL_DW, desc_mnmajor(s_xp + k * 16 * 128), desc_mnmajor(s_sp + k * 16 * 128), ID_WMN, (acc || k) ? 1u : 0u);
@@ -257,6 +258,8 @@
                 }
             }
             warp_arrive(BAR(B_XRDY), lane);
+            if (BWD)
+                for (int e = tid; e < 2 * H; e += NE) dp1[e] = e < H ? __ldg(a.DP1 + (long)pair * H + e) : __ldg(a.DP2 + (long)pair * H + e - H);
             CTS(1);
             if (pair + (int)gridDim.x < a.mb) {
                 const long np = pair + gridDim.x;
@@ -346,7 +349,6 @@
                     if (lane == 0) attn1[j] = sm / (float)N2;
                 }
             } else {
-            float *m2 = st4, *is2 = st4 + AT, *m1 = st4 + 2 * AT, *is1 = st4 + 3 * AT;
             {
                 const int i = tid & 63, pt = tid >> 6;
                 float m = -INFINITY, s = 0.f;
@@ -361,54 +363,51 @@
                 }
                 part[pt * AT + i] = m;
                 part[8 * AT + pt * AT + i] = s;
-                {
-                    float x0[4], x1[4], mx[4], sm[4];
-#pragma unroll
-                    for (int k = 0; k < 4; ++k) {
-                        const int j = warp + EPW * k;
-                        x0[k] = (j < N1 && lane < N2) ? Cs[j * CLD + lane] : -INFINITY;
-                        x1[k] = (j < N1 && lane + 32 < N2) ? Cs[j * CLD + lane + 32] : -INFINITY;
-                        mx[k] = fmaxf(x0[k], x1[k]);
-                    }
-#pragma unroll
-                    for (int o = 16; o; o >>= 1)
-#pragma unroll
-                        for (int k = 0; k < 4; ++k) mx[k] = fmaxf(mx[k], __shfl_xor_sync(0xffffffffu, mx[k], o));
-#pragma unroll
-                    for (int k = 0; k < 4; ++k)
-                        sm[k] = (x0[k] > -INFINITY ? __expf(x0[k] - mx[k]) : 0.f) + (x1[k] > -INFINITY ? __expf(x1[k] - mx[k]) : 0.f);
-#pragma unroll
-                    for (int o = 16; o; o >>= 1)
-#pragma unroll
-                        for (int k = 0; k < 4; ++k) sm[k] += __shfl_xor_sync(0xffffffffu, sm[k], o);
-                    if (lane < 4) {
-                        const float mm = lane == 0 ? mx[0] : (lane == 1 ? mx[1] : (lane == 2 ? mx[2] : mx[3]));
-                        const float ss = lane == 0 ? sm[0] : (lane == 1 ? sm[1] : (lane == 2 ? sm[2] : sm[3]));
-                        m2[warp + EPW * lane] = mm;
-                        is2[warp + EPW * lane] = ss > 0.f ? 1.f / ss : 0.f;
-                    }
-                }
-            }
-            EPI_SYNC();
-            if (tid < AT) {
+                float e0[4], e1[4], mx[4], sm[4];
+#pragma unroll
+                for (int k = 0; k < 4; ++k) {
+                    const int j = warp + EPW * k;
+                    e0[k] = (j < N1 && lane < N2) ? Cs[j * CLD + lane] : -INFINITY;
+                    e1[k] = (j < N1 && lane + 32 < N2) ? Cs[j * CLD + lane + 32] : -INFINITY;
+                    mx[k] = fmaxf(e0[k], e1[k]);
+                }
+#pragma unroll
+                for (int o = 16; o; o >>= 1)
+#pragma unroll
+                    for (int k = 0; k < 4; ++k) mx[k] = fmaxf(mx[k], __shfl_xor_sync(0xffffffffu, mx[k], o));
+#pragma unroll
+                for (int k = 0; k < 4; ++k) {
+                    e0[k] = e0[k] > -INFINITY ? __expf(e0[k] - mx[k]) : 0.f;
+                    e1[k] = e1[k] > -INFINITY ? __expf(e1[k] - mx[k]) : 0.f;
+                    sm[k] = e0[k] + e1[k];
+                }
+#pragma unroll
+                for (int o = 16; o; o >>= 1)
+#pragma unroll
+                    for (int k = 0; k < 4; ++k) sm[k] += __shfl_xor_sync(0xffffffffu, sm[k], o);
+#pragma unroll
+                for (int k = 0; k < 4; ++k) {
+                    const int j = warp + EPW * k;
+                    const float is = sm[k] > 0.f ? 1.f / sm[k] : 0.f;
+                    L2p[j * PLD + lane] = e0[k] * is;
+                    L2p[j * PLD + lane + 32] = e1[k] * is;
+                }
+            }
+            EPI_SYNC();
+            {
+                const int i = tid & 63;
                 float m = -INFINITY, s = 0.f;
 #pragma unroll
-                for (int pt = 0; pt < 8; ++pt) m = fmaxf(m, part[pt * AT + tid]);
+                for (int pt = 0; pt < 8; ++pt) m = fmaxf(m, part[pt * AT + i]);
 #pragma unroll
                 for (int pt = 0; pt < 8; ++pt) {
-                    const float pm = part[pt * AT + tid];
-                    s += pm > -INFINITY ? part[8 * AT + pt * AT + tid] * __expf(pm - m) : 0.f;
-                }
-                m1[tid] = m;
-                is1[tid] = s > 0.f ? 1.f / s : 0.f;
-            }
-            EPI_SYNC();
-            for (int idx = tid; idx < AT * AT; idx += NE) {
-                const int j = idx >> 6, i = idx & 63;
-                const bool live = j < N1 && i < N2;
-                const float c = Cs[j * CLD + i];
-                L2p[j * PLD + i] = live ? __expf(c - m2[j]) * is2[j] : 0.f;
-                L1t[i * PLD + j] = live ? __expf(c - m1[i]) * is1[i] : 0.f;
+                    const float pm = part[pt * AT + i];
+                    s += pm > -INFINITY ? part[8 * AT + pt * AT + i] * __expf(pm - m) : 0.f;
+                }
+                const float is = s > 0.f ? 1.f / s : 0.f;
+#pragma unroll
+                for (int j = tid >> 6; j < AT; j += NE / 64)
+                    L1t[i * PLD + j] = (j < N1 && i < N2) ? __expf(Cs[j * CLD + i] - m) * is : 0.f;
             }
             EPI_SYNC();
             CTS(6);
@@ -434,24 +433,22 @@
                     acc[d] += __shfl_xor_sync(0xffffffffu, acc[d], 1);
                     acc[d] += __shfl_xor_sync(0xffffffffu, acc[d], 2);
                 }
-                const float *self = (which ? lt2 : lt1) + n * HS;
+                const float *self = (which ? lt2 : lt1) + n * HS, *wa = which ? a.wa_2 : a.wa_1;
                 float *Hk = (which ? H2 : H1) + n * HS;
+                float sc = 0.f;
 #pragma unroll
                 for (int d4 = 0; d4 < HQ; ++d4) {
+                    const int d = 4 * d4 + pt;
                     const float v = pt == 0 ? acc[4 * d4] : (pt == 1 ? acc[4 * d4 + 1] : (pt == 2 ? acc[4 * d4 + 2] : acc[4 * d4 + 3]));
-                    Hk[4 * d4 + pt] = tanh_fast(self[4 * d4 + pt] + v);
-                }
-            }
-            EPI_SYNC();
+                    const float h = tanh_fast(self[d] + v);
+                    if (BWD) Hk[d] = h;
+                    sc += d < hd ? __ldg(wa + d) * h : 0.f;
+                }
+                sc += __shfl_xor_sync(0xffffffffu, sc, 1);
+                sc += __shfl_xor_sync(0xffffffffu, sc, 2);
+                if (pt == 0) (which ? attn2 : attn1)[n] = sc;
+            }
             CTS(7);
-            if (tid < 2 * AT) {
-                const int n = tid & 63;
-                const float *Hk = (tid < AT ? H1 : H2) + n * HS, *wa = tid < AT ? a.wa_1 : a.wa_2;
-                float sc = 0.f;
-#pragma unroll
-                for (int d = 0; d < HP; ++d) sc += d < hd ? __ldg(wa + d) * Hk[d] : 0.f;
-                (tid < AT ? attn1 : attn2)[n] = sc;
-            }
             }
             EPI_SYNC();
             if (warp < 2) {
@@ -466,65 +463,22 @@
             }
             EPI_SYNC();
             CTS(8);
-            if (tid < 2 * H) {
-                const int which = tid >= H, h = which ? tid - H : tid;
+            if (tid < 4 * H) {
+                const int e = tid >> 1, half = tid & 1, which = e >= H, h = which ? e - H : e;
                 const float *at = which ? attn2 : attn1;
-                const int n = which ? N2 : N1;
-                float s = 0.f;
-                for (int r = 0; r < n; ++r) s += at[r] * bf16_at(XP, 64 * which + r, h);
-                (which ? p2 : p1)[h] = s;
-            }
-            EPI_SYNC();
+                float s[4] = {0.f, 0.f, 0.f, 0.f};
+#pragma unroll
+                for (int u = 0; u < AT / 2; ++u) {
+                    const int r = 2 * u + half;
+                    s[u & 3] = fmaf(at[r], bf16_at(XP, 64 * which + r, h), s[u & 3]);
+                }
+                float sum = (s[0] + s[1]) + (s[2] + s[3]);
+                sum += __shfl_xor_sync(0xffffffffu, sum, 1);
+                if (half == 0) (which ? a.P2 : a.P1)[(long)pair * H + h] = sum;
+            }
             CTS(9);
-            if (!BWD) {
-                for (int r = tid >> 2; r < 2 * O; r += NE / 4) {
-                    const int which = r >= O, o = which ? r - O : r, pt = tid & 3;
-                    const float *p = which ? p2 : p1;
-                    const float4 *w = reinterpret_cast<const float4 *>(a.W_j + (long)o * H);
-                    float4 ww[H / 16];
-#pragma unroll
-                    for (int u = 0; u < H / 16; ++u) ww[u] = __ldg(w + 4 * u + pt);
-                    float s0 = 0.f, s1 = 0.f;
-#pragma unroll
-                    for (int u = 0; u < H / 16; ++u) {
-                        const float4 pp = *reinterpret_cast<const float4 *>(p + 4 * (4 * u + pt));
-                        s0 = fmaf(ww[u].x, pp.x, fmaf(ww[u].y, pp.y, s0));
-                        s1 = fmaf(ww[u].z, pp.z, fmaf(ww[u].w, pp.w, s1));
-                    }
-                    float sum = s0 + s1;
-                    sum += __shfl_xor_sync(0xffffffffu, sum, 1);
-                    sum += __shfl_xor_sync(0xffffffffu, sum, 2);
-                    if (pt == 0) (which ? a.c2 : a.c1)[(long)pair * O + o] = sum + a.b_j[o];
-                }
-                CTS(10);
-                continue;
-            }
+            if (!BWD) continue;
             float *t1 = st4, *t2 = st4 + AT, *cs = st4 + 2 * AT, *rsum = st4 + 3 * AT;
-            {
-                const int oh = tid >> 8, e = tid & 255;
-                const int which = e >= H, h = which ? e - H : e;
-                float s0 = 0.f, s1 = 0.f, s2 = 0.f, s3 = 0.f;
-                if (e < 2 * H) {
-                    if (oh == 0) (which ? a.P2 : a.P1)[(long)pair * H + h] = (which ? p2 : p1)[h];
-                    const float *dc = (which ? a.dc2 : a.dc1) + (long)pair * O;
-                    const int ob = ((O + 1) / 2 + 7) & ~7, o_end = oh ? O : (ob < O ? ob : O);
-                    int o = oh ? (ob < O ? ob : O) : 0;
-                    for (; o + 8 <= o_end; o += 8) {
-                        float w[8];
-#pragma unroll
-                        for (int x = 0; x < 8; ++x) w[x] = __ldg(a.W_j + (long)(o + x) * H + h);
-                        const float4 d0 = __ldg(reinterpret_cast<const float4 *>(dc + o)), d1 = __ldg(reinterpret_cast<const float4 *>(dc + o) + 1);
-                        s0 = fmaf(w[0], d0.x, s0); s1 = fmaf(w[1], d0.y, s1); s2 = fmaf(w[2], d0.z, s2); s3 = fmaf(w[3], d0.w, s3);
-                        s0 = fmaf(w[4], d1.x, s0); s1 = fmaf(w[5], d1.y, s1); s2 = fmaf(w[6], d1.z, s2); s3 = fmaf(w[7], d1.w, s3);
-                    }
-                    for (; o < o_end; ++o) s0 = fmaf(__ldg(a.W_j + (long)o * H + h), __ldg(dc + o), s0);
-                }
-                if (oh == 1 && e < 2 * H) part[e] = (s0 + s1) + (s2 + s3);
-                EPI_SYNC();
-                if (oh == 0 && e < 2 * H) (which ? dp2 : dp1)[h] = (s0 + s1) + (s2 + s3) + part[e];
-            }
-            EPI_SYNC();
-            CTS(10);
             {
                 const int which = tid >> 8, n = (tid >> 2) & 63, hp = tid & 3;
                 const float *dp = which ? dp2 : dp1;
@@ -553,7 +507,7 @@
                 da[lane + 32] = lane + 32 < n ? at[lane + 32] * (da[lane + 32] - dot) : 0.f;
             }
             EPI_SYNC();
-            CTS(11);
+            CTS(10);
             if (pool) {
                 for (int idx = tid; idx < 2 * AT * HP; idx += NE) (idx < AT * HP ? H1 : H2 - AT * HP)[idx] = 0.f;
                 for (int idx = tid; idx < AT * AT; idx += NE) {
@@ -583,33 +537,7 @@
                 if (lane == 0) (which ? gwa2 : gwa1)[d] += sw;
             }
             EPI_SYNC();
-            CTS(12);
-            {
-                const int out = tid >> 2, pt = tid & 3, which = out >= AT, n = out & 63;
-                const float *Lw = which ? L2p : L1t;
-                const float *other = which ? dpre2 : dpre1;
-                float own[HP];
-#pragma unroll
-                for (int d4 = 0; d4 < HQ; ++d4) {
-                    const float4 r4 = *reinterpret_cast<const float4 *>((which ? lt1 : lt2) + n * HS + 4 * d4);
-                    own[4 * d4] = r4.x; own[4 * d4 + 1] = r4.y; own[4 * d4 + 2] = r4.z; own[4 * d4 + 3] = r4.w;
-                }
-                float u = 0.f;
-#pragma unroll 4
-                for (int mm = 0; mm < 16; ++mm) {
-                    const int m = 4 * mm + pt;
-                    float dl = 0.f;
-#pragma unroll
-                    for (int d4 = 0; d4 < HQ; ++d4) {
-                        const float4 r4 = *reinterpret_cast<const float4 *>(other + m * HS + 4 * d4);
-                        dl = fmaf(r4.x, own[4 * d4], fmaf(r4.y, own[4 * d4 + 1], fmaf(r4.z, own[4 * d4 + 2], fmaf(r4.w, own[4 * d4 + 3], dl))));
-                    }
-                    u = fmaf(Lw[n * PLD + m], dl, u);
-                }
-                u += __shfl_xor_sync(0xffffffffu, u, 1);
-                u += __shfl_xor_sync(0xffffffffu, u, 2);
-                if (pt == 0) part[out] = u;
-            }
+            CTS(11);
             {
                 const int which = tid >> 8, n = (tid >> 2) & 63, pt = tid & 3;
                 const float *Lw = which ? L1t : L2p, *other = which ? dpre1 : dpre2;
@@ -632,16 +560,21 @@
                     acc[d] += __shfl_xor_sync(0xffffffffu, acc[d], 1);
                     acc[d] += __shfl_xor_sync(0xffffffffu, acc[d], 2);
                 }
-                const float *self = (which ? dpre2 : dpre1) + n * HS;
+                const float *self = (which ? dpre2 : dpre1) + n * HS, *own = (which ? lt2 : lt1) + n * HS;
                 float *dst = (which ? H2 : H1) + n * HS;
+                float u = 0.f;
 #pragma unroll
                 for (int d4 = 0; d4 < HQ; ++d4) {
                     const float v = pt == 0 ? acc[4 * d4] : (pt == 1 ? acc[4 * d4 + 1] : (pt == 2 ? acc[4 * d4 + 2] : acc[4 * d4 + 3]));
                     dst[4 * d4 + pt] = self[4 * d4 + pt] + v;
-                }
-            }
-            EPI_SYNC();
-            CTS(13);
+                    u = fmaf(own[4 * d4 + pt], v, u);
+                }
+                u += __shfl_xor_sync(0xffffffffu, u, 1);
+                u += __shfl_xor_sync(0xffffffffu, u, 2);
+                if (pt == 0) part[(which ? 0 : AT) + n] = u;
+            }
+            EPI_SYNC();
+            CTS(12);
             {
                 const int i = tid & 63;
                 float l2[HP], p2[HP];
@@ -668,7 +601,7 @@
                 }
             }
             EPI_SYNC();
-            CTS(14);
+            CTS(13);
             }
             if (tid < AT) {
                 float s = 0.f;
@@ -680,7 +613,7 @@
                 if (lane == 0) cs[j] = s;
             }
             EPI_SYNC();
-            CTS(15);
+            CTS(14);
             if (warp == EPW - 1) {
                 const float s = warp_sum(rsum[lane] + rsum[lane + 32]);
                 if (lane == 0) gb[0] += s;
@@ -712,11 +645,11 @@
                 *reinterpret_cast<uint4 *>(dst + sw128(r, 8)) = pack8(v + 8);
             }
             warp_arrive(BAR(B_DRDY), lane);
-            CTS(16);
+            CTS(15);
             mbar_wait(BAR(B_R), par);
             mbar_wait(BAR(B_A2), par);
             tc_fence_after();
-            CTS(17);
+            CTS(16);
             float *stg = reinterpret_cast<float *>(DP + warp * 2048);
             if (cg * 32 < H) {
                 uint32_t v[32];
@@ -751,10 +684,10 @@
                 }
             }
             warp_arrive(BAR(B_RRDY), lane);
-            CTS(18);
+            CTS(17);
             mbar_wait(BAR(B_A1), par);
             tc_fence_after();
-            CTS(19);
+            CTS(18);
             if (q < 2 && cg * 32 < H) {
                 uint32_t v[32];
                 tc_ld32(t_lane + C::COL_A1 + cg * 32, v);
@@ -774,8 +707,7 @@
                         return j < N1 ? a.d_a1 + (r1 + j) * H + cg * 32 + 16 * h2 : nullptr;
                     });
             }
-            CTS(20);
-            CTS(21);
+            CTS(19);
             tc_fence_before();
         }
         if (BWD && it > 0) {
@@ -825,7 +757,7 @@
 };
 __global__ void pack_coattn_kernel(const PackArgs p) {
     const int H = p.H, KP = H / 64, hd = p.head;
-    const long n1 = (long)KP * (H + 32) * 64, n2 = (long)KP * H * 64, n3 = (long)H * 64;
+    const long n1 = (long)KP * (H + 32) * 64, n2 = (long)KP * H * 64, n3 = (long)(H + 32) * 64;
     for (long idx = (long)blockIdx.x * blockDim.x + threadIdx.x; idx < n1 + n2 + n3; idx += (long)gridDim.x * blockDim.x) {
         float w = 0.f;
         uint8_t *dst;
@@ -849,8 +781,11 @@
         } else {
             const long r = idx - n1 - n2;
             kk = r & 63; n = (int)(r >> 6);
-            if (kk < hd) w = p.lt_1[(long)kk * H + n];
-            else if (kk == 15) w = p.V1[n];
+            if (n < H) w = p.W[(long)n * H + (KP - 1) * 64 + kk];
+            else {
+                const int e = (n - H) & 15, nn = ((n - H) >> 4) * 64 + kk;
+                if (nn < H) w = e < hd ? p.lt_1[(long)e * H + nn] : (e == 15 ? p.V1[nn] : 0.f);
+            }
             dst = p.img1x;
         }
         const uint32_t off = (uint32_t)n * 128u + ((((uint32_t)(kk >> 3) ^ ((uint32_t)n & 7u)) << 4) | (((uint32_t)kk & 7u) << 1));
@@ -858,7 +793,7 @@
     }
 }
 
-static size_t img_bytes(int H) { return (size_t)(H / 64) * (H + 32) * 128 + (size_t)(H / 64) * H * 128 + (size_t)H * 128; }
+static size_t img_bytes(int H) { return (size_t)(H / 64) * (H + 32) * 128 + (size_t)(H / 64) * H * 128 + (size_t)(H + 32) * 128; }
 
 }
 }
@@ -901,10 +836,9 @@
     return head <= 8 ? launch_ctc_hp<H, BWD, 8>(k, head, st) : launch_ctc_hp<H, BWD, 16>(k, head, st);
 }
 
-static int ctc_prepare(ctc::Args &k, int mb, int n1, int n2, int H, int O, int head, int act, const float *a1, const float *a2,
+static int ctc_prepare(ctc::Args &k, int mb, int n1, int n2, int H, int head, int act, const float *a1, const float *a2,
                        const float *W, const float *V1, const float *V2, const float *b, const float *lt1, const float *lt2,
-                       const float *wa1, const float *wa2, const float *Wj, const float *bj, void *ws, size_t ws_bytes, bool images_ready,
-                       cudaStream_t st) {
+                       const float *wa1, const float *wa2, void *ws, size_t ws_bytes, bool images_ready, cudaStream_t st) {
     if (!ws || ws_bytes < bmp_coattn_tc_workspace_bytes(H)) {
         set_error("BMP_MODE_BF16 co-attention: tc_workspace of >= %zu bytes required", bmp_coattn_tc_workspace_bytes(H));
         return BMP_EINVAL;
@@ -922,8 +856,8 @@
         if (rc) return rc;
     }
     k = ctc::Args{};
-    k.mb = mb; k.n1 = n1; k.n2 = n2; k.O = O; k.head = head; k.act = act;
-    k.atoms_1 = a1; k.atoms_2 = a2; k.b = b; k.wa_1 = wa1; k.wa_2 = wa2; k.W_j = Wj; k.b_j = bj; k.lt_2 = lt2; k.V2 = V2;
+    k.mb = mb; k.n1 = n1; k.n2 = n2; k.head = head; k.act = act;
+    k.atoms_1 = a1; k.atoms_2 = a2; k.b = b; k.wa_1 = wa1; k.wa_2 = wa2; k.lt_2 = lt2; k.V2 = V2;
     k.img1 = p.img1; k.img2 = p.img2; k.img1x = p.img1x;
     k.dbg = g_ctc_dbg;
     return BMP_OK;
@@ -931,24 +865,31 @@
 
 int bmp_coattn_forward_tc(const bmp_coattn_fwd_t *a, void *stream) {
     cudaStream_t st = (cudaStream_t)stream;
+    if (!a->P1 || !a->P2) { set_error("BMP_MODE_BF16 co-attention: (mb, hidden) workspaces P1, P2 required"); return BMP_EINVAL; }
     ctc::Args k;
     const int head = a->variant == BMP_COATTN_POOL ? 0 : a->head;
-    int rc = ctc_prepare(k, a->mb, a->n1, a->n2, a->hidden, a->out_dim, head, a->act, a->atoms_1, a->atoms_2, a->W, a->V1, a->V2, a->b,
-                         a->lt_1, a->lt_2, a->wa_1, a->wa_2, a->W_j, a->b_j, a->tc_workspace, a->tc_workspace_bytes, a->tc_images_ready != 0, st);
+    int rc = ctc_prepare(k, a->mb, a->n1, a->n2, a->hidden, head, a->act, a->atoms_1, a->atoms_2, a->W, a->V1, a->V2, a->b,
+                         a->lt_1, a->lt_2, a->wa_1, a->wa_2, a->tc_workspace, a->tc_workspace_bytes, a->tc_images_ready != 0, st);
     if (rc) return rc;
-    k.c1 = a->compact_1; k.c2 = a->compact_2;
+    k.P1 = a->P1; k.P2 = a->P2;
     k.pool = a->variant == BMP_COATTN_POOL;
-    return a->hidden == 64 ? launch_ctc<64, false>(k, head, st) : launch_ctc<128, false>(k, head, st);
+    rc = a->hidden == 64 ? launch_ctc<64, false>(k, head, st) : launch_ctc<128, false>(k, head, st);
+    if (rc) return rc;
+    if ((rc = bmp_linear_forward(a->P1, a->W_j, a->b_j, a->compact_1, a->mb, a->hidden, a->out_dim, BMP_ACT_IDENTITY, stream))) return rc;
+    return bmp_linear_forward(a->P2, a->W_j, a->b_j, a->compact_2, a->mb, a->hidden, a->out_dim, BMP_ACT_IDENTITY, stream);
 }
 
 int bmp_coattn_backward_tc(const bmp_coattn_bwd_t *a, void *stream) {
     cudaStream_t st = (cudaStream_t)stream;
+    if (!a->DP1 || !a->DP2) { set_error("BMP_MODE_BF16 co-attention: (mb, hidden) workspaces DP1, DP2 required"); return BMP_EINVAL; }
     ctc::Args k;
     const int head = a->variant == BMP_COATTN_POOL ? 0 : a->head;
-    int rc = ctc_prepare(k, a->mb, a->n1, a->n2, a->hidden, a->out_dim, head, a->act, a->atoms_1, a->atoms_2, a->W, a->V1, a->V2, a->b,
-                         a->lt_1, a->lt_2, a->wa_1, a->wa_2, a->W_j, a->b_j, a->tc_workspace, a->tc_workspace_bytes, a->tc_images_ready != 0, st);
+    int rc = ctc_prepare(k, a->mb, a->n1, a->n2, a->hidden, head, a->act, a->atoms_1, a->atoms_2, a->W, a->V1, a->V2, a->b,
+                         a->lt_1, a->lt_2, a->wa_1, a->wa_2, a->tc_workspace, a->tc_workspace_bytes, a->tc_images_ready != 0, st);
     if (rc) return rc;
-    k.dc1 = a->d_compact_1; k.dc2 = a->d_compact_2; k.R = a->R; k.P1 = a->P1; k.P2 = a->P2; k.DL1 = a->DL1; k.DL2 = a->DL2;
+    if ((rc = linear_dx(a->d_compact_1, a->W_j, a->DP1, a->mb, a->hidden, a->out_dim, st))) return rc;
+    if ((rc = linear_dx(a->d_compact_2, a->W_j, a->DP2, a->mb, a->hidden, a->out_dim, st))) return rc;
+    k.DP1 = a->DP1; k.DP2 = a->DP2; k.P1 = a->P1; k.P2 = a->P2;
     k.d_a1 = a->d_atoms_1; k.d_a2 = a->d_atoms_2;
     k.d_W = a->d_W; k.d_lt_1 = a->d_lt_1; k.d_lt_2 = a->d_lt_2;
     k.d_V1 = a->d_V1; k.d_V2 = a->d_V2; k.d_b = a->d_b; k.d_wa_1 = a->d_wa_1; k.d_wa_2 = a->d_wa_2;
diff --git a/gcn-bmp_b200/csrc/common.cuh b/gcn-bmp_b200/csrc/common.cuh
--- a/gcn-bmp_b200/csrc/common.cuh
+++ b/gcn-bmp_b200/csrc/common.cuh
@@ -17,6 +17,7 @@
 void count_launch(int n = 1);
 int check_launch(const char *what);
 bool aligned16(std::initializer_list<const void *> ps);
+int linear_dx(const float *dy, const float *W, float *dx, int rows, int in_dim, int out_dim, cudaStream_t st);
 struct ProfScope {
     int kind;
     cudaStream_t st;
diff --git a/gcn-bmp_b200/csrc/gemm.cu b/gcn-bmp_b200/csrc/gemm.cu
--- a/gcn-bmp_b200/csrc/gemm.cu
+++ b/gcn-bmp_b200/csrc/gemm.cu
@@ -185,6 +185,13 @@
     dy[i] *= d;
 }
 
+int linear_dx(const float *dy, const float *W, float *dx, int rows, int in_dim, int out_dim, cudaStream_t st) {
+    dim3 grid((rows + 63) / 64, (in_dim + 63) / 64);
+    linear_kernel<1><<<grid, NTHREADS, 0, st>>>(dy, W, nullptr, dx, rows, in_dim, out_dim, 0);
+    count_launch();
+    return check_launch("linear_kernel<1>");
+}
+
 static int sm_count() {
     static int sms = 0;
     if (!sms) {
@@ -263,12 +270,7 @@
         count_launch();
         if ((rc = check_launch("act_bwd_kernel"))) return rc;
     }
-    if (dx) {
-        dim3 grid((rows + 63) / 64, (in_dim + 63) / 64);
-        linear_kernel<1><<<grid, NTHREADS, 0, st>>>(dy, W, nullptr, dx, rows, in_dim, out_dim, 0);
-        count_launch();
-        if ((rc = check_launch("linear_kernel<1>"))) return rc;
-    }
+    if (dx && (rc = linear_dx(dy, W, dx, rows, in_dim, out_dim, st))) return rc;
     if (dW) {
         if ((rc = bmp_wgrad(dy, out_dim, x, in_dim, dW, in_dim, rows, out_dim, in_dim, stream))) return rc;
     }
diff --git a/gcn-bmp_b200/csrc/pair.cu b/gcn-bmp_b200/csrc/pair.cu
--- a/gcn-bmp_b200/csrc/pair.cu
+++ b/gcn-bmp_b200/csrc/pair.cu
@@ -30,7 +30,7 @@
     Enc e[2];
     void *x3_ws, *tc_fwd, *tc_bwd, *co_ws;
     size_t x3_bytes, tc_bytes, co_bytes;
-    float *c1, *c2, *dc1, *dc2, *P1, *P2, *corr, *dcorr, *dlogits;
+    float *c1, *c2, *dc1, *dc2, *P1, *P2, *DP1, *DP2, *corr, *dcorr, *dlogits;
     size_t total;
 };
 
@@ -72,6 +72,7 @@
     pl.c1 = c.take<float>((size_t)mb * O); pl.c2 = c.take<float>((size_t)mb * O);
     pl.dc1 = c.take<float>((size_t)mb * O); pl.dc2 = c.take<float>((size_t)mb * O);
     pl.P1 = c.take<float>((size_t)mb * H); pl.P2 = c.take<float>((size_t)mb * H);
+    if (bf16) { pl.DP1 = c.take<float>((size_t)mb * H); pl.DP2 = c.take<float>((size_t)mb * H); }
     pl.corr = c.take<float>((size_t)mb * O); pl.dcorr = c.take<float>((size_t)mb * O);
     pl.dlogits = c.take<float>((size_t)mb * K);
     pl.total = c.used;
@@ -141,7 +142,7 @@
     cf.W = a->W; cf.V1 = a->V1; cf.V2 = a->V2; cf.b = a->b; cf.lt_1 = a->lt_1; cf.lt_2 = a->lt_2; cf.wa_1 = a->wa_1; cf.wa_2 = a->wa_2;
     cf.W_j = a->W_j; cf.b_j = a->b_j;
     cf.compact_1 = pl.c1; cf.compact_2 = pl.c2;
-    cf.mode = a->mode; cf.tc_workspace = pl.co_ws; cf.tc_workspace_bytes = pl.co_bytes;
+    cf.mode = a->mode; cf.tc_workspace = pl.co_ws; cf.tc_workspace_bytes = pl.co_bytes; cf.P1 = pl.P1; cf.P2 = pl.P2;
     if ((rc = bmp_coattn_forward(&cf, stream))) return rc;
     if ((rc = bmp_hole_corr_forward(pl.c1, pl.c2, pl.corr, mb, O, stream))) return rc;
     if ((rc = bmp_linear_forward(pl.corr, a->out_W, a->out_b, a->logits, mb, O, K, BMP_ACT_IDENTITY, stream))) return rc;
@@ -166,6 +167,7 @@
     cb.d_W = a->d_W; cb.d_V1 = a->d_V1; cb.d_V2 = a->d_V2; cb.d_b = a->d_b; cb.d_lt_1 = a->d_lt_1; cb.d_lt_2 = a->d_lt_2;
     cb.d_wa_1 = a->d_wa_1; cb.d_wa_2 = a->d_wa_2; cb.d_W_j = a->d_W_j; cb.d_b_j = a->d_b_j;
     cb.mode = a->mode; cb.tc_workspace = pl.co_ws; cb.tc_workspace_bytes = pl.co_bytes; cb.tc_images_ready = 1;
+    cb.DP1 = pl.DP1; cb.DP2 = pl.DP2;
     if ((rc = bmp_coattn_backward(&cb, stream))) return rc;
     for (int s = 0; s < 2; ++s) {
         Enc &e = pl.e[s];
diff --git a/gcn-bmp_b200/gcnbmp/_capi.py b/gcn-bmp_b200/gcnbmp/_capi.py
--- a/gcn-bmp_b200/gcnbmp/_capi.py
+++ b/gcn-bmp_b200/gcnbmp/_capi.py
@@ -90,7 +90,8 @@
 class CoattnFwd(C.Structure):
     _fields_ = [(n, C.c_int) for n in ("mb", "n1", "n2", "hidden", "out_dim", "head", "variant", "act")] + [
         (n, fp) for n in ("atoms_1", "atoms_2") + _CO_PARAMS + ("compact_1", "compact_2")] + [
-        ("mode", C.c_int), ("tc_workspace", fp), ("tc_workspace_bytes", C.c_size_t), ("tc_images_ready", C.c_int)]
+        ("mode", C.c_int), ("tc_workspace", fp), ("tc_workspace_bytes", C.c_size_t), ("tc_images_ready", C.c_int),
+        ("P1", fp), ("P2", fp)]
 
 
 class CoattnBwd(C.Structure):
@@ -98,7 +99,8 @@
         (n, fp) for n in ("atoms_1", "atoms_2") + _CO_PARAMS + ("d_compact_1", "d_compact_2", "R", "P1", "P2",
                                                              "DL1", "DL2", "d_atoms_1", "d_atoms_2")
         + tuple("d_" + p for p in _CO_PARAMS)] + [
-        ("mode", C.c_int), ("tc_workspace", fp), ("tc_workspace_bytes", C.c_size_t), ("tc_images_ready", C.c_int)]
+        ("mode", C.c_int), ("tc_workspace", fp), ("tc_workspace_bytes", C.c_size_t), ("tc_images_ready", C.c_int),
+        ("DP1", fp), ("DP2", fp)]
 
 
 def _load():
diff --git a/gcn-bmp_b200/gcnbmp/functional.py b/gcn-bmp_b200/gcnbmp/functional.py
--- a/gcn-bmp_b200/gcnbmp/functional.py
+++ b/gcn-bmp_b200/gcnbmp/functional.py
@@ -507,6 +507,9 @@
         a.compact_1, a.compact_2 = _p(c1), _p(c2)
         a.mode = mode
         ws = _coattn_workspace(a, mode, H, atoms_1.device, ps)
+        if ws is not None:
+            P = torch.empty((2, mb, H), device=atoms_1.device, dtype=torch.float32)
+            a.P1, a.P2 = _p(P[0]), _p(P[1])
         K.check(K.lib.bmp_coattn_forward(C.byref(a), _stream()))
         ctx.save_for_backward(atoms_1, atoms_2, *ps)
         ctx.meta = (variant, act, head, mode)
@@ -539,6 +542,9 @@
         a.d_atoms_1, a.d_atoms_2 = _p(da1), _p(da2)
         a.mode = mode
         ws = _coattn_workspace(a, mode, H, dev, ps)
+        if ws is not None:
+            DP = e(2, mb, H)
+            a.DP1, a.DP2 = _p(DP[0]), _p(DP[1])
         K.check(K.lib.bmp_coattn_backward(C.byref(a), _stream()))
         return (da1, da2, None, None) + tuple(rets) + (None,)
 
diff --git a/include/gcnbmp.h b/include/gcnbmp.h
--- a/include/gcnbmp.h
+++ b/include/gcnbmp.h
@@ -169,6 +169,7 @@
     void  *tc_workspace;
     size_t tc_workspace_bytes;
     int    tc_images_ready;
+    float *P1, *P2;
 } bmp_coattn_fwd_t;
 
 int bmp_coattn_forward(const bmp_coattn_fwd_t *a, void *stream);
@@ -185,6 +186,7 @@
     void  *tc_workspace;
     size_t tc_workspace_bytes;
     int    tc_images_ready;
+    float *DP1, *DP2;
 } bmp_coattn_bwd_t;
 
 int bmp_coattn_backward(const bmp_coattn_bwd_t *a, void *stream);
```
